# zyj0021200/simpleImageCaptionZoo

Measured on AMD Instinct MI355X. Metric: captions/sec (SCST step), BUTDDetection COCO14-size vocab, higher is better.
Workload: dtype f32

## Files before the change

### include/icz.h

```cpp
#ifndef ICZ_H_
#define ICZ_H_
#include <stddef.h>
#include <stdint.h>

#ifdef __cplusplus
extern "C" {
#endif

typedef enum {
    ICZ_OK = 0,
    ICZ_ERR_INVALID = -1,
    ICZ_ERR_HIP = -2,
    ICZ_ERR_STATE = -3,
    ICZ_ERR_NOMEM = -4
} icz_status;

const char* icz_last_error(void);
const char* icz_version(void);

typedef struct icz_butd icz_butd_t;

typedef struct {
    int32_t R;
    int32_t D;
    int32_t H;
    int32_t E;
    int32_t A;
    int32_t V;
    int32_t max_rows;
    int32_t max_len;
} icz_butd_dims;

typedef struct {
    float* embed_weight;
    float *td_w_ih, *td_w_hh, *td_b_ih, *td_b_hh;
    float *lm_w_ih, *lm_w_hh, *lm_b_ih, *lm_b_hh;
    float *enc_att_v, *enc_att_g, *enc_att_b;
    float *dec_att_v, *dec_att_g, *dec_att_b;
    float *affine_v, *affine_g, *affine_b;
    float *predict_v, *predict_g, *predict_b;
} icz_butd_params;

int icz_butd_create(const icz_butd_dims* dims, icz_butd_t** out);
int icz_butd_destroy(icz_butd_t* h);
int icz_butd_bind_params(icz_butd_t* h, const icz_butd_params* params);
int icz_butd_set_option(icz_butd_t* h, const char* name, int32_t value);
int icz_butd_set_mask_sum_global(icz_butd_t* h, const float* mask_sum_global_dev, void* stream);
typedef void (*icz_grad_ready_cb)(void* user, int32_t stage);
int icz_butd_set_grad_callback(icz_butd_t* h, icz_grad_ready_cb cb, void* user);
int icz_butd_refresh_weights(icz_butd_t* h, void* stream);

int icz_butd_greedy(icz_butd_t* h, const float* feats, int32_t B, int32_t max_len, int64_t* ids_out,
                    float* alphas_out, void* stream);

typedef struct {
    uint64_t seed;
    const float* uniforms;
    const uint8_t* emb_mask;
    const uint8_t* att_mask;
    const uint8_t* out_mask;
} icz_rng;

int icz_butd_sample(icz_butd_t* h, const float* feats, int32_t B, int32_t max_len, const icz_rng* rng,
                    int64_t* seq_out, float* logprobs_out, void* stream);

int icz_butd_scst_rollouts(icz_butd_t* h, const float* feats, int32_t B, int32_t max_len, const icz_rng* rng,
                           int64_t* greedy_ids_out, int64_t* seq_out, float* logprobs_out, void* stream);
int icz_butd_sample_n(icz_butd_t* h, const float* feats, int32_t B, int32_t K, int32_t max_len, const icz_rng* rng,
                      int64_t* seq_out, float* logprobs_out, void* stream);

int icz_butd_sample_backward(icz_butd_t* h, const float* reward, const icz_butd_params* grads, float* loss_out,
                             float* mask_sum_out, float mask_sum_global, void* stream);
int icz_butd_sample_backward_dlogp(icz_butd_t* h, const float* dlogp, const icz_butd_params* grads, void* stream);
int icz_butd_sample_mask_sum(icz_butd_t* h, float* mask_sum_out, void* stream);

int icz_butd_xe_forward(icz_butd_t* h, const float* feats, const int64_t* captions, int32_t B, int32_t L,
                        const int32_t* lengths_host, const icz_rng* rng, int32_t train,
                        float* packed_logits_out, void* stream);
int icz_butd_xe_backward(icz_butd_t* h, float smoothing, const icz_butd_params* grads, float* loss_out,
                         float n_tokens_global, void* stream);

int icz_butd_set_scheduled_sampling(icz_butd_t* h, float ss_prob, const float* gate_uniforms, const float* draw_uniforms);

int icz_butd_saved_alphas(icz_butd_t* h, float* alphas_out, void* stream);

int icz_butd_xe_backward_dlogits(icz_butd_t* h, const float* dpacked, const icz_butd_params* grads, void* stream);

int icz_butd_beam_search(icz_butd_t* h, const float* feats, int32_t n_img, int32_t beam, int32_t max_steps,
                         float* seqs_out, int32_t* lens_out, void* stream);

typedef struct {
    int32_t n_best;
    int32_t block_ngram;
    int32_t lp_kind;
    float lp_alpha;
} icz_beam_opts;

int icz_butd_beam_search_opts(icz_butd_t* h, const float* feats, int32_t n_img, int32_t beam, int32_t max_steps,
                              const icz_beam_opts* opts, float* seqs_out, int32_t* lens_out, float* scores_out, void* stream);

typedef struct {
    int32_t groups;
    float diversity;
} icz_beam_diversity;

int icz_butd_beam_search_diverse(icz_butd_t* h, const float* feats, int32_t n_img, int32_t beam, int32_t max_steps,
                                 const icz_beam_opts* opts, const icz_beam_diversity* div, float* seqs_out, int32_t* lens_out,
                                 float* scores_out, void* stream);

int icz_butd_step(icz_butd_t* h, const float* feats, int32_t B, const int64_t* it, float* h1, float* c1,
                  float* h2, float* c2, float* ctx_out, float* alpha_out, float* logits_out, void* stream);

typedef struct icz_nic icz_nic_t;
typedef struct { int32_t E, H, V, max_rows, max_len; } icz_nic_dims;
typedef struct {
    float* embed_weight;
    float *w_ih, *w_hh, *b_ih, *b_hh;
    float *predict_v, *predict_g, *predict_b;
} icz_nic_params;
int icz_nic_create(const icz_nic_dims* dims, icz_nic_t** out);
int icz_nic_destroy(icz_nic_t* h);
int icz_nic_bind_params(icz_nic_t* h, const icz_nic_params* params);
int icz_nic_refresh_weights(icz_nic_t* h, void* stream);
int icz_nic_greedy(icz_nic_t* h, const float* features, int32_t B, int32_t max_len, int64_t* ids_out, void* stream);
int icz_nic_sample(icz_nic_t* h, const float* features, int32_t B, int32_t max_len, const icz_rng* rng, int64_t* seq_out,
                   float* logprobs_out, void* stream);
int icz_nic_sample_backward(icz_nic_t* h, const float* reward, const icz_nic_params* grads, float* dfeatures_out, float* loss_out,
                            float* mask_sum_out, float mask_sum_global, void* stream);
int icz_nic_xe_forward(icz_nic_t* h, const float* features, const int64_t* captions, int32_t B, int32_t L, const int32_t* lengths_host,
                       const icz_rng* rng, int32_t train, float* packed_logits_out, void* stream);
int icz_nic_xe_backward(icz_nic_t* h, float smoothing, const icz_nic_params* grads, float* dfeatures_out, float* loss_out,
                        float n_tokens_global, void* stream);
int icz_nic_set_norm_global(icz_nic_t* h, const float* norm_dev, void* stream);
int icz_nic_set_option(icz_nic_t* h, const char* name, int32_t value);
int icz_nic_set_scheduled_sampling(icz_nic_t* h, float ss_prob, const float* gate_uniforms, const float* draw_uniforms);
int icz_nic_beam_search(icz_nic_t* h, const float* features, int32_t n_img, int32_t beam, int32_t max_steps, float* seqs_out,
                        int32_t* lens_out, void* stream);
int icz_nic_beam_search_opts(icz_nic_t* h, const float* features, int32_t n_img, int32_t beam, int32_t max_steps,
                             const icz_beam_opts* opts, float* seqs_out, int32_t* lens_out, float* scores_out, void* stream);
int icz_nic_beam_search_diverse(icz_nic_t* h, const float* features, int32_t n_img, int32_t beam, int32_t max_steps,
                                const icz_beam_opts* opts, const icz_beam_diversity* div, float* seqs_out, int32_t* lens_out,
                                float* scores_out, void* stream);

typedef struct icz_aoa icz_aoa_t;
typedef struct { int32_t R, D, Hd, E, V, NH, max_rows, max_len; } icz_aoa_dims;
typedef struct {
    float *q_w, *q_b, *k_w, *k_b, *v_w, *v_b, *aoa_w, *aoa_b, *ln_g, *ln_b;
} icz_aoa_block;
typedef struct {
    float *proj_w, *proj_b;
    icz_aoa_block layer[6];
    float *ref_ln_g, *ref_ln_b;
    float *lstm_w_ih, *lstm_w_hh, *lstm_b_ih, *lstm_b_hh;
    icz_aoa_block dec;
    float* embed_weight;
    float *predict_v, *predict_g, *predict_b;
} icz_aoa_params;
typedef struct {
    uint64_t seed;
    const float* uniforms;
    const uint8_t *proj_mask, *ref_att_mask, *ref_aoa_mask, *ref_sc_mask, *emb_mask, *ctx_mask, *att_mask, *out_mask;
} icz_aoa_rng;
int icz_aoa_create(const icz_aoa_dims* dims, icz_aoa_t** out);
int icz_aoa_destroy(icz_aoa_t* h);
int icz_aoa_bind_params(icz_aoa_t* h, const icz_aoa_params* params);
int icz_aoa_refresh_weights(icz_aoa_t* h, void* stream);
int icz_aoa_set_regions(icz_aoa_t* h, int32_t regions, const int32_t* counts_dev, const int32_t* counts_host, int32_t n_img);
int icz_aoa_set_option(icz_aoa_t* h, const char* name, int32_t value);
int icz_aoa_refine(icz_aoa_t* h, const float* feats, int32_t B, float* refined_out, void* stream);
int icz_aoa_greedy(icz_aoa_t* h, const float* feats, int32_t B, int32_t max_len, int64_t* ids_out, void* stream);
int icz_aoa_beam_search(icz_aoa_t* h, const float* feats, int32_t n_img, int32_t beam, int32_t max_steps, float* seqs_out,
                        int32_t* lens_out, void* stream);
int icz_aoa_beam_search_opts(icz_aoa_t* h, const float* feats, int32_t n_img, int32_t beam, int32_t max_steps,
                             const icz_beam_opts* opts, float* seqs_out, int32_t* lens_out, float* scores_out, void* stream);
int icz_aoa_beam_search_diverse(icz_aoa_t* h, const float* feats, int32_t n_img, int32_t beam, int32_t max_steps,
                                const icz_beam_opts* opts, const icz_beam_diversity* div, float* seqs_out, int32_t* lens_out,
                                float* scores_out, void* stream);
int icz_aoa_sample(icz_aoa_t* h, const float* feats, int32_t B, int32_t max_len, const icz_aoa_rng* rng, int64_t* seq_out,
                   float* logprobs_out, void* stream);
int icz_aoa_scst_rollouts(icz_aoa_t* h, const float* feats, int32_t B, int32_t max_len, const icz_aoa_rng* rng, int64_t* ids_out,
                          int64_t* seq_out, float* logprobs_out, void* stream);
int icz_aoa_sample_backward(icz_aoa_t* h, const float* reward, const icz_aoa_params* grads, float* loss_out, float* mask_sum_out,
                            float mask_sum_global, void* stream);
int icz_aoa_xe_forward(icz_aoa_t* h, const float* feats, const int64_t* captions, int32_t B, int32_t L, const int32_t* lengths_host,
                       const icz_aoa_rng* rng, int32_t train, float* packed_logits_out, void* stream);
int icz_aoa_xe_backward(icz_aoa_t* h, float smoothing, const icz_aoa_params* grads, float* loss_out, float n_tokens_global,
                        void* stream);
int icz_aoa_set_norm_global(icz_aoa_t* h, const float* norm_dev, void* stream);
int icz_aoa_set_grad_callback(icz_aoa_t* h, icz_grad_ready_cb cb, void* user);
int icz_aoa_saved_alphas(icz_aoa_t* h, float* alphas_out, void* stream);
int icz_aoa_set_scheduled_sampling(icz_aoa_t* h, float ss_prob, const float* gate_uniforms, const float* draw_uniforms);

typedef struct icz_ensemble icz_ensemble_t;
int icz_ensemble_create(const int32_t* kinds, void* const* members, const float* weights, int32_t M, icz_ensemble_t** out);
int icz_ensemble_destroy(icz_ensemble_t* h);
int icz_ensemble_greedy(icz_ensemble_t* h, const float* const* feats, int32_t B, int32_t max_len, int64_t* ids_out, void* stream);
int icz_ensemble_beam_search_diverse(icz_ensemble_t* h, const float* const* feats, int32_t n_img, int32_t beam, int32_t max_steps,
                                     const icz_beam_opts* opts, const icz_beam_diversity* div, float* seqs_out, int32_t* lens_out,
                                     float* scores_out, void* stream);
int icz_ensemble_logprob(int32_t M, const float* const* logits, const float* const* bias, const int32_t* nsplit, const int32_t* ld,
                         const float* weights, int32_t rows, int32_t V, float* lp_out, int32_t ldo, int64_t* argmax_out, void* stream);

typedef struct {
    float temperature;
    int32_t top_k;
    float top_p;
} icz_sample_opts;
int icz_sample_decode_check(const icz_sample_opts* opts, int32_t n_img, int32_t n, int32_t V, int32_t max_rows);
int icz_butd_sample_decode(icz_butd_t* h, const float* feats, int32_t n_img, int32_t n, int32_t max_len, const icz_sample_opts* opts,
                           uint64_t seed, const float* uniforms, int64_t* ids_out, float* logp_out, float* score_out, void* stream);
int icz_aoa_sample_decode(icz_aoa_t* h, const float* feats, int32_t n_img, int32_t n, int32_t max_len, const icz_sample_opts* opts,
                          uint64_t seed, const float* uniforms, int64_t* ids_out, float* logp_out, float* score_out, void* stream);
int icz_nic_sample_decode(icz_nic_t* h, const float* features, int32_t n_img, int32_t n, int32_t max_len, const icz_sample_opts* opts,
                          uint64_t seed, const float* uniforms, int64_t* ids_out, float* logp_out, float* score_out, void* stream);
int icz_sample_filter_draw(const float* logits, const float* bias, int32_t nsplit, int32_t ld, int32_t rows, int32_t V,
                           const icz_sample_opts* opts, const float* uniforms, int64_t* tok_out, float* logp_out, uint8_t* keep_out,
                           void* stream);

int icz_ensemble_sample_decode(icz_ensemble_t* h, const float* const* feats, int32_t n_img, int32_t n, int32_t max_len,
                               const icz_sample_opts* opts, uint64_t seed, const float* uniforms, int64_t* ids_out, float* logp_out,
                               float* score_out, void* stream);
int icz_ensemble_sample_filter_draw(int32_t M, const float* const* logits, const float* const* bias, const int32_t* nsplit,
                                    const int32_t* ld, const float* weights, int32_t rows, int32_t V, const icz_sample_opts* opts,
                                    const float* uniforms, int64_t* tok_out, float* logp_out, uint8_t* keep_out, void* stream);

int icz_adam_clamp_step(float* param, const float* grad, float* exp_avg, float* exp_avg_sq, int64_t n,
                        float lr, float clip, int32_t step, void* stream);
int icz_adam_clamp_multi(int32_t count, float* const* params, const float* const* grads, float* const* exp_avg,
                         float* const* exp_avg_sq, const int64_t* numel, float lr, float clip, int32_t step, void* stream);

typedef struct icz_ciderd icz_ciderd_t;

int icz_ciderd_create(const int32_t* df_keys, const double* df_idf, int64_t cap, double default_idf,
                      const double* penalty, icz_ciderd_t** out);
int icz_ciderd_destroy(icz_ciderd_t* h);

int icz_ciderd_reward(icz_ciderd_t* h, const int64_t* gen, const int64_t* greedy, int32_t B, int32_t T,
                      const int32_t* img_ref_ptr, const int32_t* ref_ent_ptr, const int32_t* ent_key,
                      const int32_t* ent_order, const double* ent_w, const double* ref_norm,
                      const int32_t* ref_len, float* reward_out, double* scores_out, void* stream);
int icz_ciderd_cook_host(const int32_t* df_keys_host, const double* df_idf_host, int64_t cap, double default_idf,
                         const int32_t* tokens, const int32_t* ref_tok_ptr, int32_t n_refs, int64_t max_ent,
                         int32_t* ent_key_out, int32_t* ent_order_out, double* ent_w_out, int32_t* ref_ent_ptr_out,
                         double* ref_norm_out, int32_t* ref_len_out, int64_t* n_ent_out);
typedef struct icz_ciderd_vocab icz_ciderd_vocab_t;
int icz_ciderd_vocab_create(const char* words, const int64_t* word_off, const int32_t* word_id, int32_t n_words, int32_t V,
                            icz_ciderd_vocab_t** out);
int icz_ciderd_vocab_destroy(icz_ciderd_vocab_t* v);
int icz_ciderd_vocab_oov_id(icz_ciderd_vocab_t* v, const char* word, int32_t len, int32_t* id_out);
int icz_ciderd_cook_text(icz_ciderd_vocab_t* vocab, const int32_t* df_keys_host, const double* df_idf_host, int64_t cap, double default_idf,
                         const char* text, int64_t text_len, int32_t n_refs, int64_t max_ent,
                         int32_t* ent_key_out, int32_t* ent_order_out, double* ent_w_out, int32_t* ref_ent_ptr_out,
                         double* ref_norm_out, int32_t* ref_len_out, int64_t* n_ent_out);
int icz_ciderd_reward_indexed(icz_ciderd_t* h, const int64_t* gen, const int64_t* greedy, int32_t B, int32_t T,
                              const int32_t* img_slot, const int32_t* img_ref_ptr, const int32_t* ref_ent_ptr,
                              const int32_t* ent_key, const int32_t* ent_order, const double* ent_w, const double* ref_norm,
                              const int32_t* ref_len, float* reward_out, double* scores_out, void* stream);
int icz_ciderd_reward_loo(icz_ciderd_t* h, const int64_t* gen, int32_t B, int32_t K, int32_t T, const int32_t* img_slot,
                          const int32_t* img_ref_ptr, const int32_t* ref_ent_ptr, const int32_t* ent_key, const int32_t* ent_order,
                          const double* ent_w, const double* ref_norm, const int32_t* ref_len, float* reward_out, double* scores_out,
                          void* stream);

int icz_ciderd_cook_device(icz_ciderd_t* h, const int32_t* tok, const int32_t* ptr, int32_t n_cand, int32_t* ent_key_out,
                           int32_t* ent_order_out, double* ent_w_out, int32_t* ent_ptr_out, double* norm_out, int32_t* len_out, void* stream);
size_t icz_ciderd_pairwise_workspace_bytes(int32_t n_img, int32_t K);
int icz_ciderd_pairwise(icz_ciderd_t* h, const int32_t* tok, const int32_t* ptr, int32_t n_img, int32_t K, double* pair_out,
                        double* consensus_out, int32_t* best_out, void* workspace, size_t workspace_bytes, void* stream);
int icz_ciderd_scores_csr(icz_ciderd_t* h, const int32_t* tok, const int32_t* ptr, int32_t n_img, int32_t K, const int32_t* img_slot,
                          const int32_t* img_ref_ptr, const int32_t* ref_ent_ptr, const int32_t* ent_key, const int32_t* ent_order,
                          const double* ent_w, const double* ref_norm, const int32_t* ref_len, double* scores_out, void* stream);
int icz_ngram_diversity(const int32_t* tok, const int32_t* ptr, int32_t n_img, int32_t K, int32_t* counts_out, void* stream);

int icz_bleu_stats(const int32_t* hyp_tok, const int32_t* hyp_ptr, const int32_t* ref_tok, const int32_t* ref_ptr,
                   const int32_t* img_ref_ptr, int32_t n_img, int32_t* stats_out, void* stream);
int icz_rouge_lcs(const int32_t* hyp_tok, const int32_t* hyp_ptr, const int32_t* ref_tok, const int32_t* ref_ptr,
                  const int32_t* img_ref_ptr, int32_t n_img, int32_t* lcs_out, void* stream);

int icz_gemm_f32(int32_t layout, const float* X, int32_t ldx, const float* W, int32_t ldw, const float* bias,
                 float* C, int32_t ldc, int32_t M, int32_t N, int32_t K, int32_t nsplit, float* workspace,
                 size_t workspace_floats, void* stream);
size_t icz_gemm_workspace_floats(int32_t M, int32_t N);
int icz_gemm_set_big_cfg(int32_t cfg);
int icz_gemm_big_cfg_for(int32_t layout, int32_t M, int32_t N, int32_t K, int32_t nsplit);
int icz_gemm_tn_grouped(const float* dY, int32_t ldy, int32_t M, int32_t K, int32_t ngroups, const float* const* X, const int32_t* ldx,
                        const int32_t* cols, float* const* out, const int32_t* ldo, const int32_t* rows_live, void* stream);
int icz_gemm_tn_split_pick(int32_t M, int32_t N, int32_t K);
int icz_gemm_tn_split(const float* dY, int32_t ldy, int32_t M, const float* X, int32_t ldx, int32_t N, int32_t K, float* out, int32_t ldo,
                      float* workspace, size_t workspace_floats, const int32_t* rows_live, void* stream);
int icz_gemm_route_for(int32_t layout, int32_t M, int32_t N, int32_t nseg, const int32_t* K, int32_t nsplit);
int icz_gemm_tn_grouped_fits(int32_t M, int32_t K, int32_t ngroups, const int32_t* cols);
int icz_prof_begin(void);
int icz_prof_select(int32_t which);
int icz_prof_pair_overhead(void* stream, int32_t n, double* avg_us);
int icz_prof_end(double* avg_us, double* bytes_per_launch, double* flops_per_launch, long long* launches);
int icz_kprof_begin(void);
int icz_kprof_end(int32_t group, double* avg_us, long long* pairs);
int icz_prof_stream_rate(const void* buf, size_t bytes, int32_t reps, void* stream, double* gbs);

#ifdef __cplusplus
}
#endif
#endif
```

### simpleimagecaptionzoo_amd/_lib.py

```python
import ctypes as C
import os

_HERE = os.path.dirname(os.path.abspath(__file__))
LIB_PATH = os.path.join(_HERE, "libicz.so")


class IczError(RuntimeError):
    pass


GRAD_READY_CB = C.CFUNCTYPE(None, C.c_void_p, C.c_int32)


class ButdDims(C.Structure):
    _fields_ = [(n, C.c_int32) for n in ("R", "D", "H", "E", "A", "V", "max_rows", "max_len")]


BUTD_PARAM_FIELDS = (
    "embed_weight",
    "td_w_ih", "td_w_hh", "td_b_ih", "td_b_hh",
    "lm_w_ih", "lm_w_hh", "lm_b_ih", "lm_b_hh",
    "enc_att_v", "enc_att_g", "enc_att_b",
    "dec_att_v", "dec_att_g", "dec_att_b",
    "affine_v", "affine_g", "affine_b",
# ... 45 lines not shown
class AoaRng(C.Structure):
    _fields_ = [("seed", C.c_uint64), ("uniforms", C.c_void_p)] + [(n, C.c_void_p) for n in (
        "proj_mask", "ref_att_mask", "ref_aoa_mask", "ref_sc_mask", "emb_mask", "ctx_mask", "att_mask", "out_mask")]


class NicParams(C.Structure):
    _fields_ = [(n, C.c_void_p) for n in NIC_PARAM_FIELDS]


class ButdParams(C.Structure):
    _fields_ = [(n, C.c_void_p) for n in BUTD_PARAM_FIELDS]


class Rng(C.Structure):
    _fields_ = [("seed", C.c_uint64), ("uniforms", C.c_void_p), ("emb_mask", C.c_void_p),
                ("att_mask", C.c_void_p), ("out_mask", C.c_void_p)]


class BeamOpts(C.Structure):
    _fields_ = [("n_best", C.c_int32), ("block_ngram", C.c_int32), ("lp_kind", C.c_int32), ("lp_alpha", C.c_float)]


class BeamDiversity(C.Structure):
    _fields_ = [("groups", C.c_int32), ("diversity", C.c_float)]


class SampleOpts(C.Structure):
    _fields_ = [("temperature", C.c_float), ("top_k", C.c_int32), ("top_p", C.c_float)]


_lib = None


def lib():
    global _lib
    if _lib is not None:
        return _lib
    if not os.path.exists(LIB_PATH):
        raise IczError("libicz.so not found at %s -- the HIP extension is required (no fallback); run "
                       "__graft_entry__.build()" % LIB_PATH)
    import torch
    L = C.CDLL(LIB_PATH)
    vp, i32, i64, f32 = C.c_void_p, C.c_int32, C.c_int64, C.c_float
    sig = {
        "icz_last_error": (C.c_char_p, []),
        "icz_version": (C.c_char_p, []),
        "icz_butd_create": (C.c_int, [C.POINTER(ButdDims), C.POINTER(vp)]),
        "icz_butd_destroy": (C.c_int, [vp]),
        "icz_butd_bind_params": (C.c_int, [vp, C.POINTER(ButdParams)]),
        "icz_butd_set_option": (C.c_int, [vp, C.c_char_p, i32]),
        "icz_butd_set_grad_callback": (C.c_int, [vp, GRAD_READY_CB, vp]),
        "icz_aoa_set_grad_callback": (C.c_int, [vp, GRAD_READY_CB, vp]),
        "icz_butd_set_mask_sum_global": (C.c_int, [vp, vp, vp]),
        "icz_butd_refresh_weights": (C.c_int, [vp, vp]),
        "icz_butd_greedy": (C.c_int, [vp, vp, i32, i32, vp, vp, vp]),
        "icz_butd_step": (C.c_int, [vp, vp, i32, vp, vp, vp, vp, vp, vp, vp, vp, vp]),
        "icz_butd_sample": (C.c_int, [vp, vp, i32, i32, C.POINTER(Rng), vp, vp, vp]),
        "icz_butd_scst_rollouts": (C.c_int, [vp, vp, i32, i32, C.POINTER(Rng), vp, vp, vp, vp]),
        "icz_butd_sample_n": (C.c_int, [vp, vp, i32, i32, i32, C.POINTER(Rng), vp, vp, vp]),
        "icz_butd_sample_backward": (C.c_int, [vp, vp, C.POINTER(ButdParams), vp, vp, f32, vp]),
        "icz_butd_sample_backward_dlogp": (C.c_int, [vp, vp, C.POINTER(ButdParams), vp]),
        "icz_butd_xe_backward_dlogits": (C.c_int, [vp, vp, C.POINTER(ButdParams), vp]),
        "icz_butd_beam_search": (C.c_int, [vp, vp, i32, i32, i32, vp, vp, vp]),
        "icz_butd_beam_search_opts": (C.c_int, [vp, vp, i32, i32, i32, C.POINTER(BeamOpts), vp, vp, vp, vp]),
        "icz_butd_beam_search_diverse": (C.c_int, [vp, vp, i32, i32, i32, C.POINTER(BeamOpts), C.POINTER(BeamDiversity), vp, vp, vp, vp]),
        "icz_butd_sample_mask_sum": (C.c_int, [vp, vp, vp]),
        "icz_butd_xe_forward": (C.c_int, [vp, vp, vp, i32, i32, C.POINTER(i32), C.POINTER(Rng), i32, vp, vp]),
        "icz_butd_xe_backward": (C.c_int, [vp, f32, C.POINTER(ButdParams), vp, f32, vp]),
        "icz_butd_set_scheduled_sampling": (C.c_int, [vp, f32, vp, vp]),
        "icz_nic_set_scheduled_sampling": (C.c_int, [vp, f32, vp, vp]),
        "icz_aoa_set_scheduled_sampling": (C.c_int, [vp, f32, vp, vp]),
        "icz_adam_clamp_step": (C.c_int, [vp, vp, vp, vp, i64, f32, f32, i32, vp]),
        "icz_nic_create": (C.c_int, [C.POINTER(NicDims), C.POINTER(vp)]),
        "icz_nic_destroy": (C.c_int, [vp]),
        "icz_nic_bind_params": (C.c_int, [vp, C.POINTER(NicParams)]),
        "icz_nic_refresh_weights": (C.c_int, [vp, vp]),
        "icz_nic_greedy": (C.c_int, [vp, vp, i32, i32, vp, vp]),
        "icz_nic_sample": (C.c_int, [vp, vp, i32, i32, C.POINTER(Rng), vp, vp, vp]),
        "icz_nic_sample_backward": (C.c_int, [vp, vp, C.POINTER(NicParams), vp, vp, vp, f32, vp]),
        "icz_nic_xe_forward": (C.c_int, [vp, vp, vp, i32, i32, C.POINTER(i32), C.POINTER(Rng), i32, vp, vp]),
        "icz_nic_xe_backward": (C.c_int, [vp, f32, C.POINTER(NicParams), vp, vp, f32, vp]),
        "icz_butd_saved_alphas": (C.c_int, [vp, vp, vp]),
        "icz_aoa_saved_alphas": (C.c_int, [vp, vp, vp]),
        "icz_nic_set_norm_global": (C.c_int, [vp, vp, vp]),
        "icz_aoa_set_norm_global": (C.c_int, [vp, vp, vp]),
        "icz_nic_beam_search": (C.c_int, [vp, vp, i32, i32, i32, vp, vp, vp]),
        "icz_nic_beam_search_opts": (C.c_int, [vp, vp, i32, i32, i32, C.POINTER(BeamOpts), vp, vp, vp, vp]),
        "icz_nic_beam_search_diverse": (C.c_int, [vp, vp, i32, i32, i32, C.POINTER(BeamOpts), C.POINTER(BeamDiversity), vp, vp, vp, vp]),
        "icz_aoa_create": (C.c_int, [C.POINTER(AoaDims), C.POINTER(vp)]),
        "icz_aoa_destroy": (C.c_int, [vp]),
        "icz_aoa_bind_params": (C.c_int, [vp, C.POINTER(AoaParams)]),
        "icz_aoa_refresh_weights": (C.c_int, [vp, vp]),
        "icz_aoa_set_regions": (C.c_int, [vp, i32, vp, vp, i32]),
        "icz_aoa_set_option": (C.c_int, [vp, C.c_char_p, i32]),
        "icz_nic_set_option": (C.c_int, [vp, C.c_char_p, i32]),
        "icz_aoa_refine": (C.c_int, [vp, vp, i32, vp, vp]),
        "icz_aoa_greedy": (C.c_int, [vp, vp, i32, i32, vp, vp]),
        "icz_aoa_beam_search": (C.c_int, [vp, vp, i32, i32, i32, vp, vp, vp]),
        "icz_aoa_beam_search_opts": (C.c_int, [vp, vp, i32, i32, i32, C.POINTER(BeamOpts), vp, vp, vp, vp]),
        "icz_aoa_beam_search_diverse": (C.c_int, [vp, vp, i32, i32, i32, C.POINTER(BeamOpts), C.POINTER(BeamDiversity), vp, vp, vp, vp]),
        "icz_ensemble_create": (C.c_int, [C.POINTER(i32), C.POINTER(vp), C.POINTER(f32), i32, C.POINTER(vp)]),
        "icz_ensemble_destroy": (C.c_int, [vp]),
        "icz_ensemble_greedy": (C.c_int, [vp, C.POINTER(vp), i32, i32, vp, vp]),
        "icz_ensemble_beam_search_diverse": (C.c_int, [vp, C.POINTER(vp), i32, i32, i32, C.POINTER(BeamOpts), C.POINTER(BeamDiversity), vp, vp,
                                                       vp, vp]),
        "icz_ensemble_logprob": (C.c_int, [i32, C.POINTER(vp), C.POINTER(vp), C.POINTER(i32), C.POINTER(i32), C.POINTER(f32), i32, i32, vp, i32,
                                           vp, vp]),
        "icz_ensemble_sample_decode": (C.c_int, [vp, C.POINTER(vp), i32, i32, i32, C.POINTER(SampleOpts), C.c_uint64, vp, vp, vp, vp, vp]),
        "icz_ensemble_sample_filter_draw": (C.c_int, [i32, C.POINTER(vp), C.POINTER(vp), C.POINTER(i32), C.POINTER(i32), C.POINTER(f32), i32, i32,
                                                      C.POINTER(SampleOpts), vp, vp, vp, vp, vp]),
        "icz_sample_decode_check": (C.c_int, [C.POINTER(SampleOpts), i32, i32, i32, i32]),
        "icz_butd_sample_decode": (C.c_int, [vp, vp, i32, i32, i32, C.POINTER(SampleOpts), C.c_uint64, vp, vp, vp, vp, vp]),
        "icz_aoa_sample_decode": (C.c_int, [vp, vp, i32, i32, i32, C.POINTER(SampleOpts), C.c_uint64, vp, vp, vp, vp, vp]),
        "icz_nic_sample_decode": (C.c_int, [vp, vp, i32, i32, i32, C.POINTER(SampleOpts), C.c_uint64, vp, vp, vp, vp, vp]),
        "icz_sample_filter_draw": (C.c_int, [vp, vp, i32, i32, i32, i32, C.POINTER(SampleOpts), vp, vp, vp, vp, vp]),
        "icz_aoa_sample": (C.c_int, [vp, vp, i32, i32, C.POINTER(AoaRng), vp, vp, vp]),
        "icz_aoa_scst_rollouts": (C.c_int, [vp, vp, i32, i32, C.POINTER(AoaRng), vp, vp, vp, vp]),
        "icz_aoa_sample_backward": (C.c_int, [vp, vp, C.POINTER(AoaParams), vp, vp, f32, vp]),
        "icz_aoa_xe_forward": (C.c_int, [vp, vp, vp, i32, i32, C.POINTER(i32), C.POINTER(AoaRng), i32, vp, vp]),
        "icz_aoa_xe_backward": (C.c_int, [vp, f32, C.POINTER(AoaParams), vp, f32, vp]),
        "icz_ciderd_create": (C.c_int, [vp, vp, i64, C.c_double, vp, C.POINTER(vp)]),
        "icz_ciderd_destroy": (C.c_int, [vp]),
        "icz_ciderd_reward": (C.c_int, [vp, vp, vp, i32, i32, vp, vp, vp, vp, vp, vp, vp, vp, vp, vp]),
        "icz_ciderd_cook_host": (C.c_int, [vp, vp, i64, C.c_double, vp, vp, i32, i64, vp, vp, vp, vp, vp, vp, C.POINTER(i64)]),
        "icz_ciderd_vocab_create": (C.c_int, [C.c_char_p, vp, vp, i32, i32, C.POINTER(vp)]),
        "icz_ciderd_vocab_destroy": (C.c_int, [vp]),
        "icz_ciderd_vocab_oov_id": (C.c_int, [vp, C.c_char_p, i32, C.POINTER(i32)]),
        "icz_ciderd_cook_text": (C.c_int, [vp, vp, vp, i64, C.c_double, C.c_char_p, i64, i32, i64, vp, vp, vp, vp, vp, vp, C.POINTER(i64)]),
        "icz_ciderd_reward_indexed": (C.c_int, [vp, vp, vp, i32, i32, vp, vp, vp, vp, vp, vp, vp, vp, vp, vp, vp]),
        "icz_ciderd_reward_loo": (C.c_int, [vp, vp, i32, i32, i32, vp, vp, vp, vp, vp, vp, vp, vp, vp, vp, vp]),
        "icz_ciderd_cook_device": (C.c_int, [vp, vp, vp, i32, vp, vp, vp, vp, vp, vp, vp]),
        "icz_ciderd_pairwise_workspace_bytes": (C.c_size_t, [i32, i32]),
        "icz_ciderd_pairwise": (C.c_int, [vp, vp, vp, i32, i32, vp, vp, vp, vp, C.c_size_t, vp]),
        "icz_ciderd_scores_csr": (C.c_int, [vp, vp, vp, i32, i32, vp, vp, vp, vp, vp, vp, vp, vp, vp, vp]),
        "icz_ngram_diversity": (C.c_int, [vp, vp, i32, i32, vp, vp]),
        "icz_bleu_stats": (C.c_int, [vp, vp, vp, vp, vp, i32, vp, vp]),
        "icz_rouge_lcs": (C.c_int, [vp, vp, vp, vp, vp, i32, vp, vp]),
        "icz_prof_begin": (C.c_int, []),
        "icz_prof_select": (C.c_int, [i32]),
        "icz_prof_pair_overhead": (C.c_int, [vp, i32, C.POINTER(C.c_double)]),
        "icz_prof_end": (C.c_int, [C.POINTER(C.c_double), C.POINTER(C.c_double), C.POINTER(C.c_double), C.POINTER(C.c_longlong)]),
        "icz_kprof_begin": (C.c_int, []),
        "icz_kprof_end": (C.c_int, [i32, C.POINTER(C.c_double), C.POINTER(C.c_longlong)]),
        "icz_prof_stream_rate": (C.c_int, [vp, C.c_size_t, i32, vp, C.POINTER(C.c_double)]),
        "icz_adam_clamp_multi": (C.c_int, [i32, C.POINTER(vp), C.POINTER(vp), C.POINTER(vp), C.POINTER(vp), C.POINTER(i64), f32, f32, i32, vp]),
        "icz_gemm_f32": (C.c_int, [i32, vp, i32, vp, i32, vp, vp, i32, i32, i32, i32, i32, vp, C.c_size_t, vp]),
        "icz_gemm_workspace_floats": (C.c_size_t, [i32, i32]),
        "icz_gemm_set_big_cfg": (C.c_int, [i32]),
        "icz_gemm_big_cfg_for": (C.c_int, [i32, i32, i32, i32, i32]),
        "icz_gemm_tn_grouped": (C.c_int, [vp, i32, i32, i32, i32, vp, vp, vp, vp, vp, vp, vp]),
        "icz_gemm_tn_split_pick": (C.c_int, [i32, i32, i32]),
        "icz_gemm_tn_split": (C.c_int, [vp, i32, i32, vp, i32, i32, i32, vp, i32, vp, C.c_size_t, vp, vp]),
        "icz_gemm_route_for": (C.c_int, [i32, i32, i32, i32, vp, i32]),
        "icz_gemm_tn_grouped_fits": (C.c_int, [i32, i32, i32, vp]),
    }
    for name, (res, args) in sig.items():
        try:
            fn = getattr(L, name)
        except AttributeError as e:
            raise IczError("libicz.so lacks symbol %s (stale build?)" % name) from e
        fn.restype, fn.argtypes = res, args
    _lib = L
    return L


def check(status):
    if status != 0:
        raise IczError("libicz status %d: %s" % (status, lib().icz_last_error().decode()))


def ptr(t):
    return None if t is None else C.c_void_p(t.data_ptr())


def stream_ptr():
    import torch
    return C.c_void_p(torch.cuda.current_stream().cuda_stream)
```

### simpleimagecaptionzoo_amd/butd.py

```python
import ctypes as C

import torch

from . import _lib
from ._lib import BUTD_PARAM_KEYS, ButdDims, ButdParams, Rng, check, lib, ptr, stream_ptr
from .handle import GraphDecoderHandle


def make_rng(seed=0, uniforms=None, emb_mask=None, att_mask=None, out_mask=None):
    r = Rng()
    r.seed = int(seed) & 0xFFFFFFFFFFFFFFFF
    keep = []
    for name, t, dt in (("uniforms", uniforms, torch.float32), ("emb_mask", emb_mask, torch.uint8),
                        ("att_mask", att_mask, torch.uint8), ("out_mask", out_mask, torch.uint8)):
        if t is not None:
            if t.dtype != dt or not t.is_cuda or not t.is_contiguous():
                raise _lib.IczError("%s must be a contiguous %s CUDA tensor" % (name, dt))
            setattr(r, name, t.data_ptr())
            keep.append(t)
    r._keep = keep
    return r


class ButdHandle(GraphDecoderHandle):

    family, kind = "butd", 0
    _Params, _param_keys = ButdParams, BUTD_PARAM_KEYS
    _make_rng = staticmethod(make_rng)
    _own_entries = ("step", "sample_n", "sample_mask_sum", "saved_alphas", "sample_backward_dlogp", "xe_backward_dlogits")
    _entry_names = {"set_norm_global": "set_mask_sum_global"}
    _sample_bufs = True

    def __init__(self, R, D, H, E, A, V, max_rows, max_len=20, device="cuda:0"):
        self._create(ButdDims(R, D, H, E, A, V, max_rows, max_len), device)

    def enable_graphs(self, on=True):
        super().enable_graphs(on)

    def set_concurrent(self, on=True):
        self.set_option("concurrent", 1 if on else 0)

    def _feats(self, feats):
        if feats.dtype != torch.float32 or not feats.is_cuda:
            raise _lib.IczError("feats must be an fp32 CUDA tensor")
        if feats.dim() != 3 or feats.shape[1] != self.R or feats.shape[2] != self.D:
            raise _lib.IczError("feats must be (B,%d,%d), got %s" % (self.R, self.D, tuple(feats.shape)))
        return feats.contiguous()

    def greedy(self, feats, max_len=20, want_alphas=False):
        feats = self._feats(feats)
        B = feats.shape[0]
        ids = self._buf("greedy_ids", (B, max_len), torch.int64)
        alphas = self._buf("greedy_alphas", (B, max_len, self.R), torch.float32) if want_alphas else None
        check(self._e.greedy(self._h, ptr(feats), B, max_len, ptr(ids), ptr(alphas), stream_ptr()))
        return (ids, alphas) if want_alphas else ids

    def sample_n(self, feats, n, max_len=20, rng=None):
        feats = self._feats(feats)
        B, n = feats.shape[0], int(n)
        if not 2 <= n <= 8:
            raise _lib.IczError("sample_n: n=%d samples per image outside 2..8" % n)
        if B * n > self.max_rows:
            raise _lib.IczError("sample_n: %d images x %d samples exceed the handle's row capacity %d" % (B, n, self.max_rows))
        rng = rng or make_rng(0)
        seq = self._buf("sample_n_seq", (B * n, max_len), torch.int64)
        lp = self._buf("sample_n_lp", (B * n, max_len), torch.float32)
        check(self._e.sample_n(self._h, ptr(feats), B, n, max_len, C.byref(rng), ptr(seq), ptr(lp), stream_ptr()))
        self._live = (feats, rng, seq, lp)
        return seq, lp

    def sample_mask_sum(self):
        out = torch.zeros(1, device=self.device)
        check(self._e.sample_mask_sum(self._h, ptr(out), stream_ptr()))
        return out

    def sample_backward_dlogp(self, dlogp, grads):
        dlogp = dlogp.to(device=self.device, dtype=torch.float32).contiguous()
        gs = self._grad_struct(grads)
        check(self._e.sample_backward_dlogp(self._h, ptr(dlogp), C.byref(gs), stream_ptr()))

    def saved_alphas(self, B, T):
        out = torch.empty(B, T, self.R, device=self.device)
        check(self._e.saved_alphas(self._h, ptr(out), stream_ptr()))
        return out

    def xe_backward_dlogits(self, dpacked, grads):
        dpacked = dpacked.to(device=self.device, dtype=torch.float32).contiguous()
        gs = self._grad_struct(grads)
        check(self._e.xe_backward_dlogits(self._h, ptr(dpacked), C.byref(gs), stream_ptr()))

    def step(self, feats, it, h1, c1, h2, c2):
        feats = self._feats(feats)
        B = feats.shape[0]
        dev = feats.device
        ctx = torch.empty(B, self.D, device=dev)
        alpha = torch.empty(B, self.R, device=dev)
        logits = torch.empty(B, self.V, device=dev)
        check(self._e.step(self._h, ptr(feats), B, ptr(it), ptr(h1), ptr(c1), ptr(h2), ptr(c2), ptr(ctx), ptr(alpha), ptr(logits),
                           stream_ptr()))
        return ctx, alpha, logits


def gemm(layout, X, W, bias=None, nsplit=0):
    code = {"nt": 0, "nn": 1, "tn": 2}[layout]
    if layout == "nt":
        M, K = X.shape
        N = W.shape[0]
    elif layout == "nn":
        M, K = X.shape
        N = W.shape[1]
    else:
        K, M = X.shape
        N = W.shape[1]
    out = torch.empty(M, N, device=X.device, dtype=torch.float32)
    ws = torch.empty(max(lib().icz_gemm_workspace_floats(M, N), max(nsplit, 1) * M * N), device=X.device,
                     dtype=torch.float32)
    check(lib().icz_gemm_f32(code, ptr(X), X.stride(0), ptr(W), W.stride(0), ptr(bias), ptr(out), N, M, N, K,
                             nsplit, ptr(ws), ws.numel(), stream_ptr()))
    return out


def gemm_set_big_cfg(cfg):
    check(lib().icz_gemm_set_big_cfg(int(cfg)))


def gemm_tn_grouped(dY, Xs, outs=None, rows_live=None):
    K, M = dY.shape
    n = len(Xs)
    if outs is None:
        outs = [torch.empty(M, x.shape[1], device=dY.device, dtype=torch.float32) for x in Xs]
    xp = (C.c_void_p * n)(*[x.data_ptr() for x in Xs])
    op = (C.c_void_p * n)(*[o.data_ptr() for o in outs])
    ldx = (C.c_int32 * n)(*[x.stride(0) for x in Xs])
    cols = (C.c_int32 * n)(*[x.shape[1] for x in Xs])
    ldo = (C.c_int32 * n)(*[o.stride(0) for o in outs])
    check(lib().icz_gemm_tn_grouped(ptr(dY), dY.stride(0), M, K, n, xp, ldx, cols, op, ldo, ptr(rows_live), stream_ptr()))
    return outs


def gemm_tn_split_pick(M, N, K):
    return int(lib().icz_gemm_tn_split_pick(int(M), int(N), int(K)))


def gemm_tn_split(dY, X, out=None, workspace=None, rows_live=None):
    K, M = dY.shape
    N = X.shape[1]
    if out is None:
        out = torch.empty(M, N, device=dY.device, dtype=torch.float32)
    if workspace is None:
        workspace = torch.empty(max(gemm_tn_split_pick(M, N, K), 1) * M * N, device=dY.device, dtype=torch.float32)
    check(lib().icz_gemm_tn_split(ptr(dY), dY.stride(0), M, ptr(X), X.stride(0), N, K, ptr(out), out.stride(0), ptr(workspace),
                                  workspace.numel(), ptr(rows_live), stream_ptr()))
    return out


GEMM_ROUTES = ("nt_fp32_mt1", "nt_fp32_mt2", "nt_fp32_mt4", "resident_4stage", "resident_512deep", "resident_128row", "x3_128tile",
               "large_tile", "nn_fp32", "tn_fp32_64", "tn_fp32_128")


def gemm_route_for(layout, M, N, Ks, nsplit=0):
    Ks = [int(k) for k in (Ks if isinstance(Ks, (list, tuple)) else [Ks])]
    arr = (C.c_int32 * len(Ks))(*Ks)
    r = int(lib().icz_gemm_route_for({"nt": 0, "nn": 1, "tn": 2}[layout], int(M), int(N), len(Ks), arr, int(nsplit)))
    return GEMM_ROUTES[r] if r >= 0 else None


def gemm_tn_grouped_fits(M, K, cols):
    arr = (C.c_int32 * len(cols))(*[int(c) for c in cols])
    return int(lib().icz_gemm_tn_grouped_fits(int(M), int(K), len(cols), arr)) == 1
```

### simpleimagecaptionzoo_amd/csrc/butd.hip

```cpp
#include <vector>

#include "butd_impl.h"

namespace icz {

int Butd::init(const icz_butd_dims& d) {
    dims = d;
    ICZ_REQUIRE(d.R > 0 && d.R <= 64, "butd: R=%d must be in 1..64 (36 boxes / 49 grid cells)", d.R);
    ICZ_REQUIRE(d.D % 4 == 0 && d.H % 4 == 0 && d.E % 4 == 0 && d.A % 4 == 0, "butd: D,H,E,A must be multiples of 4");
    ICZ_REQUIRE(d.V > 3 && d.max_rows > 0 && d.max_len > 0, "butd: bad V/max_rows/max_len");
    const size_t rows = d.max_rows, H = d.H, D = d.D, E = d.E, A = d.A, V = d.V, R = d.R;
    ICZ_TRY(alloc((void**)&w_enc, sizeof(float) * A * D));
    ICZ_TRY(alloc((void**)&w_dec, sizeof(float) * A * H));
    ICZ_TRY(alloc((void**)&w_aff, sizeof(float) * A));
    const size_t Vp = pad_vocab(d.V);
    ICZ_TRY(alloc((void**)&w_pred, sizeof(float) * Vp * H));
    ICZ_TRY(alloc((void**)&n_enc, sizeof(float) * A));
    ICZ_TRY(alloc((void**)&n_dec, sizeof(float) * A));
    ICZ_TRY(alloc((void**)&n_aff, sizeof(float) * 4));
    ICZ_TRY(alloc((void**)&n_pred, sizeof(float) * V));
    ICZ_TRY(alloc((void**)&mean, sizeof(float) * rows * D));
    ICZ_TRY(alloc((void**)&premean, sizeof(float) * rows * 4 * H));
    ICZ_TRY(alloc((void**)&enc_ctx, sizeof(float) * rows * R * A));
    for (int i = 0; i < 2; ++i) {
        ICZ_TRY(alloc((void**)&h1[i], sizeof(float) * rows * H));
        ICZ_TRY(alloc((void**)&c1[i], sizeof(float) * rows * H));
        ICZ_TRY(alloc((void**)&h2[i], sizeof(float) * rows * H));
        ICZ_TRY(alloc((void**)&c2[i], sizeof(float) * rows * H));
    }
    ICZ_TRY(alloc((void**)&emb, sizeof(float) * rows * E));
    ICZ_TRY(alloc((void**)&ctx, sizeof(float) * rows * D));
    ICZ_TRY(alloc((void**)&scores, sizeof(float) * rows * R));
    ICZ_TRY(alloc((void**)&alpha, sizeof(float) * rows * R));
    ICZ_TRY(alloc((void**)&h2drop, sizeof(float) * rows * H));
    ICZ_TRY(alloc((void**)&logits, sizeof(float) * rows * Vp));
    ICZ_TRY(alloc((void**)&amax_val, sizeof(float) * rows * ARGMAX_PARTS));
    ICZ_TRY(alloc((void**)&amax_idx, sizeof(int) * rows * ARGMAX_PARTS));
    ICZ_TRY(alloc((void**)&it, sizeof(int64_t) * rows));
    ICZ_TRY(alloc_scalars(mem));
    size_t nmax = 4 * H;
    if (A > nmax) nmax = A;
    if (V > nmax) nmax = V;
    ws_floats = (size_t)TARGET_WGS * 4096 * 2 + rows * nmax;
    {
        const size_t kmax = 2 * H + (E > D ? E : D), r128 = rows < 128 ? rows : 128;
        const size_t need = (kmax / 256 + 1) * r128 * 4 * H;
        if (need > ws_floats) ws_floats = need;
    }
    ICZ_TRY(alloc((void**)&ws, sizeof(float) * ws_floats));
    ICZ_TRY(mem.synced());
    if (const char* e = getenv("ICZ_EARLY_OUT")) early_out = atoi(e) != 0;
    if (const char* e = getenv("ICZ_MERGE_SMALL")) { const int n = atoi(e); if (n >= 0 && n <= 32) merge_small = n; }
    return ICZ_OK;
}

int Butd::refresh(hipStream_t st) {
    ICZ_REQUIRE(bound, "butd: parameters not bound");
    const int A = dims.A, D = dims.D, H = dims.H, V = dims.V;
    WeightNormTable wt = {};
    int nb = 0;
    auto add = [&](const float* v, const float* g, float* w, float* norm, int rows, int cols) {
        wt.j[wt.count++] = {v, g, w, norm, rows, cols, nb};
        nb += cdiv(rows, 4);
    };
    add(P.enc_att_v, P.enc_att_g, w_enc, n_enc, A, D);
    add(P.dec_att_v, P.dec_att_g, w_dec, n_dec, A, H);
    add(P.affine_v, P.affine_g, w_aff, n_aff, 1, A);
    add(P.predict_v, P.predict_g, w_pred, n_pred, V, H);
    hipLaunchKernelGGL(weight_norm_multi_kernel, dim3(nb), dim3(256), 0, st, wt);
    ICZ_CHECK_HIP(hipGetLastError());
    fresh = true;
    wt_fresh = false;
    return ICZ_OK;
}

bool Butd::wt_possible() const {
    GemmArgs g = {};
    g.nseg = 1;
    g.seg[0] = {w_enc, w_enc, 4 * dims.H, 4 * dims.H, 4 * dims.H, nullptr};
    g.M = 64; g.N = dims.D + dims.H;
    GemmArgs p = g, q = g;
    p.N = q.N = dims.H;
    p.nseg = 2; p.seg[1] = p.seg[0];
    return dims.H % 64 == 0 && dims.D % 64 == 0 && gemm_resident_x3_fits(g) && gemm_resident_x3_pair_fits(p, q);
}

int Butd::refresh_transposes(hipStream_t st) {
    ICZ_REQUIRE(bound && wt_lm_ih, "butd: no transposed weight buffers");
    const int H = dims.H, D = dims.D, E = dims.E;
    TransposeTable tt = {};
    int nb = 0;
    auto add = [&](const float* src, int ld, int cols, float* dst) {
        tt.j[tt.count++] = {src, ld, 4 * H, cols, dst, nb};
        nb += (4 * H / 64) * (cols / 64);
    };
    add(P.lm_w_ih, D + H, D + H, wt_lm_ih);
    add(P.lm_w_hh, H, H, wt_lm_hh);
    add(P.td_w_ih, H + D + E, H, wt_td_ih_h2);
    add(P.td_w_hh, H, H, wt_td_hh);
    hipLaunchKernelGGL(transpose_multi_kernel, dim3(nb), dim3(256), 0, st, tt);
    ICZ_CHECK_HIP(hipGetLastError());
    wt_fresh = true;
    return ICZ_OK;
}

int Butd::gemm_nt(GemmArgs& g, int* nsplit_out, hipStream_t st) {
    g.nsplit = gemm_fit_split(GEMM_NT, g, gemm_pick_split(g, TARGET_WGS), ws_floats);
    if (g.nsplit > 1) {
        ICZ_REQUIRE(gemm_slab_floats(g.M, g.N, g.nsplit) <= ws_floats, "butd: workspace too small for %dx%dx%d slabs", g.nsplit, g.M, g.N);
        g.out = ws;
        g.bias = nullptr;
    }
    *nsplit_out = g.nsplit;
    return gemm_f32(GEMM_NT, g, st);
}

int Butd::prologue(const float* feats, int n_img, hipStream_t st) {
    const int R = dims.R, D = dims.D, H = dims.H, E = dims.E, A = dims.A;
    ICZ_REQUIRE(fresh, "butd: call icz_butd_refresh_weights after binding/updating parameters");
    ICZ_REQUIRE(n_img > 0 && n_img <= dims.max_rows, "butd: %d images exceed capacity %d", n_img, dims.max_rows);
    hipLaunchKernelGGL(mean_feats_kernel, dim3(cdiv(D, 1024), n_img), dim3(256), 0, st, feats, mean, R, D);
    {
        GemmArgs g = {};
        g.nseg = 1;
        g.seg[0] = {mean, P.td_w_ih + H, D, H + D + E, D, nullptr};
        g.M = n_img; g.N = 4 * H; g.out = premean; g.ldo = 4 * H;
        int ns;
        ICZ_TRY(gemm_nt(g, &ns, st));
        if (ns > 1) {
            size_t MN = (size_t)n_img * 4 * H;
            hipLaunchKernelGGL(slab_reduce_kernel, dim3(cdiv((int)(MN / 4), 256)), dim3(256), 0, st, ws, ns, MN, 4 * H, (const float*)nullptr, premean);
        }
    }
    {
        GemmArgs g = {};
        g.nseg = 1;
        g.seg[0] = {feats, w_enc, D, D, D, nullptr};
        g.M = n_img * R; g.N = A; g.out = enc_ctx; g.ldo = A; g.bias = P.enc_att_b;
        int ns;
        const float* bias = g.bias;
        ICZ_TRY(gemm_nt(g, &ns, st));
        if (ns > 1) {
            size_t MN = (size_t)n_img * R * A;
            hipLaunchKernelGGL(slab_reduce_kernel, dim3(cdiv((int)(MN / 4), 256)), dim3(256), 0, st, ws, ns, MN, A, bias, enc_ctx);
        }
    }
    ICZ_CHECK_HIP(hipGetLastError());
    return ICZ_OK;
}

int Butd::step(const StepIO& s, hipStream_t st) {
    const int R = dims.R, D = dims.D, H = dims.H, E = dims.E, A = dims.A, V = dims.V;
    const int Vp = pad_vocab(V);
    const int rows = s.rows;
    float* const ws = s.ws_alt ? s.ws_alt : this->ws;
    float* const scores = s.scores_alt ? s.scores_alt : this->scores;
    DropCfg off = {0, nullptr, nullptr, 0, 0};
    if (!s.emb_ready)
        hipLaunchKernelGGL(embed_kernel, dim3(cdiv(E, 1024), rows), dim3(256), 0, st, P.embed_weight, s.it, s.emb_out ? s.emb_out : emb, rows, E, s.drop_emb);
    const float* embp = s.emb_out ? s.emb_out : emb;
    int ns;
    {
        GemmArgs g = {};
        g.nseg = 3;
        g.seg[0] = {s.h2_in, P.td_w_ih, H, H + D + E, H, nullptr};
        g.seg[1] = {embp, P.td_w_ih + H + D, E, H + D + E, E, nullptr};
        g.seg[2] = {s.h1_in, P.td_w_hh, H, H, H, nullptr};
        g.M = rows; g.N = 4 * H; g.out = ws; g.ldo = 4 * H;
        g.live = s.live;
        const size_t ws_cap = s.ws_alt ? (tb.xfloats < ws_floats ? tb.xfloats : ws_floats) : ws_floats;
        g.nsplit = gemm_fit_split(GEMM_NT, g, gemm_pick_split(g, STEP_WGS), ws_cap);
        ns = g.nsplit;
        ICZ_REQUIRE(gemm_slab_floats(rows, 4 * H, ns) <= ws_cap && (size_t)rows * 4 * H <= ws_cap, "butd: workspace too small");
        if (ns == 1) { g.out = ws; }
        ICZ_TRY(gemm_f32(GEMM_NT, g, st));
        LstmPointArgs a = {ws, ns, premean, s.img_of_row, P.td_b_ih, P.td_b_hh, s.c1_in, s.h1_out, s.c1_out, s.gates_td_out, nullptr, rows, H, s.live};
        kprof_mark(KP_LSTM_POINT, true, st);
        launch_lstm_point(a, off, st);
        kprof_mark(KP_LSTM_POINT, false, st);
    }
    {
        kprof_mark(KP_ATTENTION, true, st);
        GemmArgs g = {};
        g.nseg = 1;
        g.seg[0] = {s.h1_out, w_dec, H, H, H, nullptr};
        g.M = rows; g.N = A; g.out = ws; g.ldo = A;
        g.live = s.live;
        g.nsplit = gemm_pick_split(g, STEP_WGS);
        ns = g.nsplit;
        ICZ_TRY(gemm_f32(GEMM_NT, g, st));
        AttScoreArgs a = {enc_ctx, s.img_of_row, ws, ns, P.dec_att_b, w_aff, P.affine_b, s.dec_ctx_out, scores, rows, R, A, s.live};
        const int G = s.rows_per_img;
        const bool grouped = G > 1 && G <= ATT_CTX_MAX_G && rows % G == 0 && sizeof(float) * A * G <= 60 * 1024;
        if (grouped && s.drop_att.mode == 0 && !s.live)
            hipLaunchKernelGGL(att_scores_group_kernel, dim3(rows / G, ATT_PARTS), dim3(256), sizeof(float) * A * G, st, a, G);
        else if (grouped)
            hipLaunchKernelGGL(att_scores_group_train_kernel, dim3(rows / G, ATT_PARTS), dim3(256), sizeof(float) * A * G, st, a, s.drop_att, G);
        else
            hipLaunchKernelGGL(att_scores_kernel, dim3(rows, ATT_PARTS), dim3(256), sizeof(float) * A, st, a, s.drop_att);
        if (G > 1 && G <= ATT_CTX_MAX_G && rows % G == 0 && !s.alpha_out2)
            hipLaunchKernelGGL(att_ctx_group_kernel, dim3(rows / G, cdiv(D, 512)), dim3(256), 0, st, s.feats, (const float*)scores,
                               s.alpha_out ? s.alpha_out : alpha, s.ctx_out ? s.ctx_out : ctx, R, D, G, s.live);
        else
            hipLaunchKernelGGL(att_ctx_kernel, dim3(rows, cdiv(D, 512)), dim3(256), 0, st, s.feats, s.img_of_row, (const float*)scores,
                               s.alpha_out ? s.alpha_out : alpha, s.alpha_out2, s.alpha2_stride, s.ctx_out ? s.ctx_out : ctx, R, D, s.live);
        kprof_mark(KP_ATTENTION, false, st);
    }
    const float* ctxp = s.ctx_out ? s.ctx_out : ctx;
    {
        GemmArgs g = {};
        g.nseg = 3;
        g.seg[0] = {ctxp, P.lm_w_ih, D, D + H, D, nullptr};
        g.seg[1] = {s.h1_out, P.lm_w_ih + D, H, D + H, H, nullptr};
        g.seg[2] = {s.h2_in, P.lm_w_hh, H, H, H, nullptr};
        g.M = rows; g.N = 4 * H; g.out = ws; g.ldo = 4 * H;
        g.live = s.live;
        const size_t ws_cap = s.ws_alt ? (tb.xfloats < ws_floats ? tb.xfloats : ws_floats) : ws_floats;
        g.nsplit = gemm_fit_split(GEMM_NT, g, gemm_pick_split(g, STEP_WGS), ws_cap);
        ns = g.nsplit;
        ICZ_REQUIRE(gemm_slab_floats(rows, 4 * H, ns) <= ws_cap && (size_t)rows * 4 * H <= ws_cap, "butd: workspace too small");
        ICZ_TRY(gemm_f32(GEMM_NT, g, st));
        LstmPointArgs a = {ws, ns, nullptr, nullptr, P.lm_b_ih, P.lm_b_hh, s.c2_in, s.h2_out, s.c2_out, s.gates_lm_out,
                           s.h2drop_out ? s.h2drop_out : h2drop, rows, H, s.live};
        launch_lstm_point(a, s.drop_out, st);
    }
    if (!s.skip_predict) {
        const size_t ws_cap = s.ws_alt ? (tb.xfloats < ws_floats ? tb.xfloats : ws_floats) : ws_floats;
        ICZ_TRY(gemm_predict(s.h2drop_out ? s.h2drop_out : h2drop, H, w_pred, P.predict_b, rows, V, Vp, s.logits_out ? s.logits_out : logits,
                             s.logits_ld ? s.logits_ld : Vp, ws, ws_cap, s.pred_nsplit, st, s.live));
    }
    ICZ_CHECK_HIP(hipGetLastError());
    return ICZ_OK;
}

int Butd::zero_state(int rows, int which, hipStream_t st) {
    ZeroList z = {{h1[which], c1[which], h2[which], c2[which]}, 4};
    const size_t n = (size_t)rows * dims.H;
    hipLaunchKernelGGL(zero_bufs_kernel, dim3(cdiv((int)(n / 4), 256)), dim3(256), 0, st, z, n);
    return ICZ_OK;
}

int Butd::greedy(const float* feats, int B, int max_len, int64_t* ids_out, float* alphas_out, hipStream_t st) {
    ICZ_REQUIRE(feats && ids_out && B > 0 && B <= dims.max_rows && max_len > 0, "butd greedy: bad arguments");
    ICZ_REQUIRE(fresh, "butd: call icz_butd_refresh_weights after binding/updating parameters");
    if (!use_graphs) return greedy_impl(feats, B, max_len, ids_out, alphas_out, st);
    const std::vector<uintptr_t> key = {1, (uintptr_t)feats, (uintptr_t)B, (uintptr_t)max_len, (uintptr_t)ids_out, (uintptr_t)alphas_out, opt_bits()};
    return gc.run(key, st, [&](hipStream_t s) { return greedy_impl(feats, B, max_len, ids_out, alphas_out, s); });
}

int Butd::greedy_impl(const float* feats, int B, int max_len, int64_t* ids_out, float* alphas_out, hipStream_t st) {
    ICZ_TRY(prologue(feats, B, st));
    return greedy_chain(feats, B, max_len, ids_out, alphas_out, st);
}

int Butd::greedy_chain(const float* feats, int B, int max_len, int64_t* ids_out, float* alphas_out, hipStream_t st, bool scst) {
    ICZ_TRY(zero_state(B, 0, st));
    int* const gn = (scst && early_out && gnunf && tb.T >= max_len && tb.B >= B) ? gnunf : nullptr;
    hipLaunchKernelGGL(greedy_init_kernel, dim3(cdiv(B > max_len ? B : max_len, 256)), dim3(256), 0, st, it, B, gn, max_len);
    int cur = 0;
    const int Vp = pad_vocab(dims.V);
    bool track = false;
    for (int t = 0; t < max_len; ++t) {
        StepIO s = {};
        s.rows = B; s.feats = feats; s.it = it;
        s.emb_ready = t > 0;
        s.h1_in = h1[cur]; s.c1_in = c1[cur]; s.h2_in = h2[cur]; s.c2_in = c2[cur];
        s.h1_out = h1[cur ^ 1]; s.c1_out = c1[cur ^ 1]; s.h2_out = h2[cur ^ 1]; s.c2_out = c2[cur ^ 1];
        if (alphas_out) { s.alpha_out2 = alphas_out + (size_t)t * dims.R; s.alpha2_stride = max_len * dims.R; }
        int pns = 1;
        s.pred_nsplit = &pns;
        if (track && t > 0) s.live = gn + (t - 1);
        ICZ_TRY(step(s, st));
        if (t == 0) track = gn && pns > 1;
        kprof_mark(KP_GREEDY_SELECT, true, st);
        launch_greedy_select(logits_view(ws, P.predict_b, logits, B, Vp, pns), emb_slot(), B, dims.V, amax_val, amax_idx, it, ids_out, max_len, t,
                             track ? gunf : nullptr, track ? gn : nullptr, st);
        kprof_mark(KP_GREEDY_SELECT, false, st);
        cur ^= 1;
    }
    ICZ_CHECK_HIP(hipGetLastError());
    return ICZ_OK;
}

int Butd::prologue(const float* feats, int n_img, int k, const int32_t*, hipStream_t st) {
    ICZ_TRY(prologue(feats, n_img, st));
    seam_feats = feats;
    return zero_state(n_img * k, 0, st);
}

int Butd::step(int rows, const int64_t* it_, const int32_t* img_of_row, int rows_per_img, int cur, bool slabs, LogitsView* out,
               hipStream_t st) {
    StepIO s = {};
    s.rows = rows; s.feats = seam_feats; s.img_of_row = img_of_row; s.it = it_;
    s.rows_per_img = rows_per_img;
    s.emb_ready = seam_emb_ready; s.live = seam_live;
    s.h1_in = h1[cur]; s.c1_in = c1[cur]; s.h2_in = h2[cur]; s.c2_in = c2[cur];
    s.h1_out = h1[cur ^ 1]; s.c1_out = c1[cur ^ 1]; s.h2_out = h2[cur ^ 1]; s.c2_out = c2[cur ^ 1];
    int pns = 1;
    if (slabs) s.pred_nsplit = &pns;
    ICZ_TRY(step(s, st));
    if (out) *out = logits_view(ws, P.predict_b, logits, rows, pad_vocab(dims.V), pns);
    return ICZ_OK;
}

void Butd::gather(const int32_t* src_row, int rows, int fan, hipStream_t st) {
    hipLaunchKernelGGL(beam_gather_kernel, dim3(cdiv(dims.H, 1024), rows), dim3(256), 0, st, src_row, dims.H, h1[1], c1[1], h2[1], c2[1],
                       h1[0], c1[0], h2[0], c2[0], fan);
}

DecodeMember* butd_member(void* handle) { return static_cast<DecodeMember*>(reinterpret_cast<Butd*>(handle)); }

}

using namespace icz;

extern "C" {

int icz_butd_create(const icz_butd_dims* dims, icz_butd_t** out) { return abi_create<Butd>("icz_butd_create", dims, out); }

int icz_butd_destroy(icz_butd_t* h) {
    delete reinterpret_cast<Butd*>(h);
    return ICZ_OK;
}

int icz_butd_bind_params(icz_butd_t* h, const icz_butd_params* p) {
    ICZ_REQUIRE(h && p, "icz_butd_bind_params: null argument");
    ICZ_TRY(check_param_table("icz_butd_bind_params", p, sizeof(*p), (1u << 16) | (1u << 17)));
    Butd* b = reinterpret_cast<Butd*>(h);
    if (b->bound && memcmp(&b->P, p, sizeof(*p)) != 0) {
        ICZ_CHECK_HIP(hipDeviceSynchronize());
        b->gc.clear();
    }
    b->P = *p;
    b->bound = true;
    b->fresh = false;
    return ICZ_OK;
}

int icz_butd_set_option(icz_butd_t* h, const char* name, int32_t value) {
    ICZ_REQUIRE(h && name, "icz_butd_set_option: null argument");
    Butd* b = reinterpret_cast<Butd*>(h);
    if (strcmp(name, "graphs") == 0) { b->use_graphs = value != 0; return ICZ_OK; }
    if (strcmp(name, "concurrent") == 0) { b->concurrent = value != 0; return ICZ_OK; }
    if (strcmp(name, "early_out") == 0) { b->early_out = value != 0; return ICZ_OK; }
    if (strcmp(name, "small_nt") == 0) { b->small_nt = value != 0; return ICZ_OK; }
    if (strcmp(name, "group_att") == 0) { b->group_att = value != 0; return ICZ_OK; }
    if (strcmp(name, "merge_small") == 0) {
        ICZ_REQUIRE(value >= 0 && value <= 32, "icz_butd_set_option: merge_small %d outside 0..32", value);
        b->merge_small = value;
        return ICZ_OK;
    }
    set_error("icz_butd_set_option: unknown option '%s'", name);
    return ICZ_ERR_INVALID;
}

int icz_butd_set_mask_sum_global(icz_butd_t* h, const float* mask_sum_global_dev, void* stream) {
    return set_norm_global("icz_butd_set_mask_sum_global", reinterpret_cast<Butd*>(h), mask_sum_global_dev, stream);
}

int icz_butd_set_grad_callback(icz_butd_t* h, icz_grad_ready_cb cb, void* user) {
    ICZ_REQUIRE(h, "null handle");
    Butd* b = reinterpret_cast<Butd*>(h);
    b->grad_cb = cb; b->grad_cb_user = user;
    return ICZ_OK;
}

int icz_butd_refresh_weights(icz_butd_t* h, void* stream) {
    ICZ_REQUIRE(h, "null handle");
    return reinterpret_cast<Butd*>(h)->refresh((hipStream_t)stream);
}

int icz_butd_greedy(icz_butd_t* h, const float* feats, int32_t B, int32_t max_len, int64_t* ids_out,
                    float* alphas_out, void* stream) {
    ICZ_REQUIRE(h, "null handle");
    return reinterpret_cast<Butd*>(h)->greedy(feats, B, max_len, ids_out, alphas_out, (hipStream_t)stream);
}

int icz_butd_step(icz_butd_t* h, const float* feats, int32_t B, const int64_t* it, float* h1, float* c1,
                  float* h2, float* c2, float* ctx_out, float* alpha_out, float* logits_out, void* stream) {
    ICZ_REQUIRE(h && feats && it && h1 && c1 && h2 && c2 && logits_out, "icz_butd_step: null argument");
    Butd* b = reinterpret_cast<Butd*>(h);
    hipStream_t st = (hipStream_t)stream;
    ICZ_REQUIRE(B > 0 && B <= b->dims.max_rows, "icz_butd_step: B out of range");
    ICZ_TRY(b->prologue(feats, B, st));
    StepIO s = {};
    s.rows = B; s.feats = feats; s.it = it;
    s.h1_in = h1; s.c1_in = c1; s.h2_in = h2; s.c2_in = c2;
    s.h1_out = b->h1[0]; s.c1_out = b->c1[0]; s.h2_out = b->h2[0]; s.c2_out = b->c2[0];
    s.ctx_out = ctx_out; s.alpha_out = alpha_out; s.logits_out = logits_out; s.logits_ld = b->dims.V;
    ICZ_TRY(b->step(s, st));
    const size_t n = sizeof(float) * B * b->dims.H;
    ICZ_CHECK_HIP(hipMemcpyAsync(h1, b->h1[0], n, hipMemcpyDeviceToDevice, st));
    ICZ_CHECK_HIP(hipMemcpyAsync(c1, b->c1[0], n, hipMemcpyDeviceToDevice, st));
    ICZ_CHECK_HIP(hipMemcpyAsync(h2, b->h2[0], n, hipMemcpyDeviceToDevice, st));
    ICZ_CHECK_HIP(hipMemcpyAsync(c2, b->c2[0], n, hipMemcpyDeviceToDevice, st));
    return ICZ_OK;
}

}
```

### simpleimagecaptionzoo_amd/csrc/butd_impl.h

```cpp
#pragma once
#include <vector>
#include <stdint.h>

#include "decoder_core.h"

namespace icz {

struct StepIO {
    int rows;
    const float* feats;
    const int32_t* img_of_row;
    int rows_per_img;
    const int64_t* it;
    bool emb_ready;
    const float *h1_in, *c1_in, *h2_in, *c2_in;
    float *h1_out, *c1_out, *h2_out, *c2_out;
    float* emb_out;
    float* gates_td_out;
    float* gates_lm_out;
    float* dec_ctx_out;
    float* alpha_out;
    float* alpha_out2; int alpha2_stride;
    float* ctx_out;
    float* h2drop_out;
    float* logits_out;
    int logits_ld;
    int* pred_nsplit;
    float* ws_alt;
    float* scores_alt;
    DropCfg drop_emb, drop_att, drop_out;
    bool skip_predict;
    const int* live;
};

struct TrainBuf {
    int B = 0, T = 0;
    int64_t* tok = nullptr;
    float *emb = nullptr, *h1 = nullptr, *c1 = nullptr, *h2 = nullptr, *c2 = nullptr;
    float *gtd = nullptr, *glm = nullptr, *dec = nullptr, *alpha = nullptr, *ctx = nullptr, *h2d = nullptr, *logit = nullptr;
    int* nany = nullptr;
    int32_t* img2 = nullptr;
    int32_t* imgk = nullptr;
    float* dEncImg = nullptr;
    float *dGtd = nullptr, *dGlm = nullptr, *dDec = nullptr, *dEmb = nullptr, *dH2d = nullptr, *dEnc = nullptr;
    float *dwaff = nullptr, *dalpha = nullptr, *dS = nullptr, *dGsum = nullptr;
    float *dc1[2] = {nullptr, nullptr}, *dc2[2] = {nullptr, nullptr};
    float* X[4] = {nullptr, nullptr, nullptr, nullptr}; size_t xfloats = 0;
    float *dWp = nullptr, *dWenc = nullptr, *dWdec = nullptr, *dWaff = nullptr, *scalars = nullptr;
    float* wslab[2] = {nullptr, nullptr}; size_t wslab_floats[2] = {0, 0};
};

struct Butd : CaptionHead, DecodeMember {
    static constexpr int TARGET_WGS = 512;
    static constexpr int ATT_PARTS = 4;
    static constexpr int STEP_WGS = 256;
    icz_butd_dims dims;
    icz_butd_params P;
    bool bound = false, fresh = false;
    DeviceBuffers mem;

    float *w_enc = nullptr, *w_dec = nullptr, *w_aff = nullptr, *w_pred = nullptr;
    float *n_enc = nullptr, *n_dec = nullptr, *n_aff = nullptr, *n_pred = nullptr;
    float *mean = nullptr, *premean = nullptr, *enc_ctx = nullptr;
    float *h1[2], *c1[2], *h2[2], *c2[2];
    float *emb = nullptr, *ctx = nullptr, *scores = nullptr, *alpha = nullptr, *h2drop = nullptr, *logits = nullptr;
    int64_t* it = nullptr;
    float* amax_val = nullptr; int* amax_idx = nullptr;
    float* ws = nullptr;
    size_t ws_floats = 0;
    float *wt_lm_ih = nullptr, *wt_lm_hh = nullptr, *wt_td_ih_h2 = nullptr, *wt_td_hh = nullptr;
    bool wt_fresh = false;
    bool wt_possible() const;
    int refresh_transposes(hipStream_t st);

    int alloc(void** p, size_t bytes) { return mem.alloc(p, bytes); }
    int init(const icz_butd_dims& d);
    int refresh(hipStream_t st);
    int gemm_nt(GemmArgs& g, int* nsplit_out, hipStream_t st);
    int prologue(const float* feats, int n_img, hipStream_t st);
    int step(const StepIO& s, hipStream_t st);
    int zero_state(int rows, int which, hipStream_t st);
    int greedy(const float* feats, int B, int max_len, int64_t* ids_out, float* alphas_out, hipStream_t st);

    GraphCache gc{24};
    bool use_graphs = false;
    bool concurrent = true;
    uintptr_t opt_bits() const {
        return (concurrent ? 1 : 0) + (early_out ? 2 : 0) + 4 * merge_small + (small_nt ? 256 : 0) + (group_att ? 512 : 0);
    }
    int greedy_impl(const float* feats, int B, int max_len, int64_t* ids_out, float* alphas_out, hipStream_t st);
    int sample_impl(const float* feats, int B, int T, int64_t* seq_out, float* logp_out, hipStream_t st);
    int greedy_chain(const float* feats, int B, int max_len, int64_t* ids_out, float* alphas_out, hipStream_t st, bool scst = false);
    int sample_chain(const float* feats, int B, int T, int64_t* seq_out, float* logp_out, hipStream_t st, int row0 = 0, int64_t* ids_out = nullptr);
    int rollouts(const float* feats, int B, int T, const icz_rng* r, int64_t* ids_out, int64_t* seq_out, float* logp_out, hipStream_t st);
    int rollouts_impl(const float* feats, int B, int T, int64_t* ids_out, int64_t* seq_out, float* logp_out, hipStream_t st);
    SideStream side;
    SideStream low;
    icz_grad_ready_cb grad_cb = nullptr; void* grad_cb_user = nullptr;
    int sample_backward_impl(const float* reward, const icz_butd_params& G, float* loss_out, float* mask_sum_out, hipStream_t st,
                             int phases = 0xF, bool fire_cb = true);
    bool bptt_joined = false;
    int merge_small = 8;
    int cur_rows = 0, cur_row0 = 0;
    bool early_out = true;
    bool bptt_early_out = false;
    bool small_nt = true;
    int cur_K = 1, cur_nimg = 0;
    bool group_att = false;

    const float* seam_feats = nullptr;
    int vocab() const override { return dims.V; }
    int row_capacity() const override { return dims.max_rows; }
    bool refreshed() const override { return fresh; }
    bool compact_step() const override { return true; }
    EmbSlot emb_slot() const override { return {P.embed_weight, emb, dims.E, 1}; }
    DeviceBuffers& buffers() override { return mem; }
    int prologue(const float* feats, int n_img, int k, const int32_t* img_of_row, hipStream_t st) override;
    int step(int rows, const int64_t* it, const int32_t* img_of_row, int rows_per_img, int cur, bool slabs, LogitsView* out,
             hipStream_t st) override;
    void gather(const int32_t* src_row, int rows, int fan, hipStream_t st) override;

    TrainBuf tb;
    icz_rng rng = {};
    const float* cur_feats = nullptr;
    int ensure_train(int B, int T);
    int train_step(const float* feats, int rows, int Bs, int t, bool train, hipStream_t st, bool emb_ready = false, int* pred_nsplit = nullptr,
                   bool skip_predict = false, const int* live = nullptr, int row0 = 0);
    int sample(const float* feats, int B, int T, const icz_rng* r, int64_t* seq_out, float* logp_out, hipStream_t st);
    int sample_n(const float* feats, int B, int K, int T, const icz_rng* r, int64_t* seq_out, float* logp_out, hipStream_t st);
    int sample_n_impl(const float* feats, int B, int K, int T, int64_t* seq_out, float* logp_out, hipStream_t st);
    int sample_mask_sum(float* out, hipStream_t st);
    int sample_backward(const float* reward, const icz_butd_params* G, float* loss_out, float* mask_sum_out,
                        float mask_sum_global, hipStream_t st);
    int xe_forward(const float* feats, const int64_t* captions, int B, int L, const int32_t* lengths, const icz_rng* r,
                   int train, float* packed_out, hipStream_t st);
    int sample_backward_dlogp(const float* dlogp, const icz_butd_params* G, hipStream_t st);
    int xe_backward_dlogits(const float* dpacked, const icz_butd_params* G, hipStream_t st);
    int xe_backward(float smoothing, const icz_butd_params* G, float* loss_out, float n_tokens_global, hipStream_t st);
    int gemm_auto(GemmLayout layout, GemmArgs& g, float* slab, size_t slab_floats, int* ns_out, hipStream_t st);
    int wgrad(const float* dY, int ldy, int M, const float* X, int ldx, int N, int K, float* out, int ldo, hipStream_t st, const int* rows_live = nullptr);
    int bptt_prelude(hipStream_t st);
    int colsum(const float* X, int K, int N, int ldx, float* out, hipStream_t st);
    int bptt(const icz_butd_params& G, hipStream_t st, int phases = 0xF, bool fire_cb = true);
};

}
```

### simpleimagecaptionzoo_amd/csrc/butd_kernels.h

```cpp
#pragma once
#include <stdlib.h>

#include "icz_common.h"
#include "rng.h"

namespace icz {
namespace {

__global__ __launch_bounds__(256) void weight_norm_kernel(const float* __restrict__ v, const float* __restrict__ g,
                                                          float* __restrict__ w, float* __restrict__ norm,
                                                          int rows, int cols) {
    const int lane = threadIdx.x & 63;
    const int row = blockIdx.x * 4 + (threadIdx.x >> 6);
    if (row >= rows) return;
    const float* vr = v + (size_t)row * cols;
    float ss = 0.f;
    for (int c = lane * 4; c < cols; c += 256) {
        f32x4 x = *reinterpret_cast<const f32x4*>(vr + c);
        ss += x[0] * x[0] + x[1] * x[1] + x[2] * x[2] + x[3] * x[3];
    }
    ss = wave_sum(ss);
    const float nrm = sqrtf(ss);
    const float s = g[row] / nrm;
    float* wr = w + (size_t)row * cols;
// ... 1043 lines not shown
        if (w < wave) wave_off += t;
        total += t;
    }
    const double target = (double)u * total;
    int cand = 0x7fffffff;
    {
        const double prev = __shfl_up(inc, 1, 64);
        double run = wave_off + (lane ? prev : 0.0);
        if (run <= target && wave_off + inc > target) {
            cand = v1 - 1;
            for (int v = v0; v < v1 - 1; ++v) {
                run += (double)expf((srow[v] - mx) - lse);
                if (run > target) { cand = v; break; }
            }
        }
    }
#pragma unroll
    for (int o = 32; o > 0; o >>= 1) cand = min(cand, __shfl_xor(cand, o, 64));
    if (lane == 0) smi[wave] = cand;
    __syncthreads();
    int tok = 0;
    {
        int d = smi[0];
#pragma unroll
        for (int w = 1; w < NW; ++w) d = min(d, smi[w]);
        if (d > a.V - 1) d = a.V - 1;
        const bool unf = was_unf && (d != 2);
        tok = unf ? d : 0;
        if (tid == 0) {
            a.unfinished[sr] = unf ? 1 : 0;
            a.seq_out[(size_t)sr * a.T + a.t] = tok;
            a.logp_out[(size_t)sr * a.T + a.t] = (srow[d] - mx) - lse;
            a.it_next[row] = tok;
            a.draw_out[row] = d;
            a.lse_out[row] = mx + lse;
            if (unf) {
                atomicAdd(&a.n_unfinished[a.t], 1);
                if (MG) atomicAdd(&a.n_any[a.t], 1);
            }
        }
    }
    if (a.emb_next)
        for (int e = tid * 4; e < a.E; e += 4 * SEL_THREADS) {
            f32x4 x = *reinterpret_cast<const f32x4*>(a.emb_table + (size_t)tok * a.E + e);
            const uint32_t k = a.emb_drop.mode ? a.emb_drop.keep4((uint64_t)sr * a.E + e) : 0xFu;
#pragma unroll
            for (int j = 0; j < 4; ++j) x[j] = ((k >> j) & 1u) ? fmaxf(x[j], 0.f) * sc : 0.f;
            *reinterpret_cast<f32x4*>(a.emb_next + (size_t)row * a.E + e) = x;
        }
}
inline void launch_sample_select(hipStream_t st, int rows, const SampleSelArgs& a) {
    if (a.row0 > 0) hipLaunchKernelGGL(sample_select_kernel<true>, dim3(rows), dim3(SEL_THREADS), sizeof(float) * a.V, st, a);
    else hipLaunchKernelGGL(sample_select_kernel<false>, dim3(rows), dim3(SEL_THREADS), sizeof(float) * a.V, st, a);
}

__global__ __launch_bounds__(256) void reinforce_loss_kernel(const float* __restrict__ logp, const int64_t* __restrict__ seq,
                                                             const float* __restrict__ reward, int B, int T,
                                                             const float* __restrict__ mask_sum_global_p, float* __restrict__ coef,
                                                             float* __restrict__ loss_out, float* __restrict__ mask_sum_out) {
    __shared__ float smf[4];
    const int tid = threadIdx.x;
    float ms = 0.f, ls = 0.f;
    for (int i = tid; i < B * T; i += 256) {
        const int t = i % T;
        const float m = (t == 0) ? 1.f : (seq[i - 1] > 0 ? 1.f : 0.f);
        ms += m;
        ls += -logp[i] * reward[i] * m;
    }
    ms = block_sum_256(ms, smf);
    ls = block_sum_256(ls, smf);
    const float msg = mask_sum_global_p ? mask_sum_global_p[0] : 0.f;
    const float denom = msg > 0.f ? msg : ms;
    for (int i = tid; i < B * T; i += 256) {
        const int t = i % T;
        const float m = (t == 0) ? 1.f : (seq[i - 1] > 0 ? 1.f : 0.f);
        coef[i] = -reward[i] * m / denom;
    }
    if (tid == 0) {
        if (loss_out) loss_out[0] = ls / denom;
        if (mask_sum_out) mask_sum_out[0] = ms;
    }
}

__global__ __launch_bounds__(256) void reinforce_dlogits_kernel(float* __restrict__ logits, int V, int ldl,
                                                                const int32_t* __restrict__ draw, const float* __restrict__ lse,
                                                                const float* __restrict__ coef, int B, int T, int Bs = 0, int row0 = 0) {
    const int row = blockIdx.y;
    const int v = blockIdx.x * 256 + threadIdx.x;
    if (v >= ldl) return;
    const int stride = Bs > 0 ? Bs : B;
    const int t = row / stride, b = row % stride - row0;
    float* l = logits + (size_t)row * ldl;
    const float c = b >= 0 ? coef[(size_t)b * T + t] : 0.f;
    const int d = draw[row];
    float g = 0.f;
    if (v < V && d >= 0 && c != 0.f) g = c * ((v == d ? 1.f : 0.f) - expf(l[v] - lse[row]));
    l[v] = g;
}

constexpr int XE_MAX_T = 128;
struct XeRows { int n[XE_MAX_T]; };
__global__ __launch_bounds__(256) void xe_loss_dlogits_kernel(float* __restrict__ logits, int V, int ldl,
                                                              const int64_t* __restrict__ captions, int L, int B, XeRows rows,
                                                              float smoothing, float inv_n_host, const float* __restrict__ n_dev,
                                                              float* __restrict__ loss_rows) {
    __shared__ float smf[4];
    const int b = blockIdx.x, t = blockIdx.y, tid = threadIdx.x;
    if (b >= rows.n[t]) {
        float* z = logits + (size_t)(t * B + b) * ldl;
        for (int v = tid; v < ldl; v += 256) z[v] = 0.f;
        return;
    }
    const float inv_n = (n_dev && n_dev[0] > 0.f) ? 1.0f / n_dev[0] : inv_n_host;
    const int row = t * B + b;
    float* l = logits + (size_t)row * ldl;
    float mx = -INFINITY;
    for (int v = tid; v < V; v += 256) mx = fmaxf(mx, l[v]);
    mx = block_max_256(mx, smf);
    float se = 0.f;
    for (int v = tid; v < V; v += 256) se += expf(l[v] - mx);
    se = block_sum_256(se, smf);
    const float lse = mx + logf(se);
    const int tg = (int)captions[(size_t)b * L + t + 1];
    const float conf = 1.f - smoothing, low = smoothing / (float)(V - 1);
    const float lconf = conf > 0.f ? logf(conf) : 0.f, llow = low > 0.f ? logf(low) : 0.f;
    float ls = 0.f;
    for (int v = tid; v < ldl; v += 256) {
        float g = 0.f;
        if (v < V) {
            const float lp = l[v] - lse;
            const float tr = (v == tg) ? conf : low;
            if (tr > 0.f) ls += tr * (((v == tg) ? lconf : llow) - lp);
            g = (expf(lp) - tr) * inv_n;
        }
        l[v] = g;
    }
    ls = block_sum_256(ls, smf);
    if (tid == 0) loss_rows[row] = ls;
}

__global__ __launch_bounds__(256) void sum_scale_kernel(const float* __restrict__ x, int n, float scale_host, const float* __restrict__ n_dev,
                                                        float* __restrict__ out) {
    __shared__ float smf[4];
    const float scale = (n_dev && n_dev[0] > 0.f) ? 1.0f / n_dev[0] : scale_host;
    float s = 0.f;
    for (int i = threadIdx.x; i < n; i += 256) s += x[i];
    s = block_sum_256(s, smf);
    if (threadIdx.x == 0) out[0] = s * scale;
}

struct LstmBwdArgs {
    const float* dh_a; int ns_a;
    int lda_a;
    const float* dh_b; int ns_b; int lda_b;
    const float* dh_c; int ns_c; int lda_c;
    const float* dhdrop;
    const float* dc_in;
    const float* gates;
    const float* c_prev;
    const float* c_cur;
    float* dgates;
    float* dc_prev;
    int rows, H;
    int rows_a, rows_b, rows_c;
    int dc_in_rows;
    const int* live;
    const int* carry_live;
};
__global__ __launch_bounds__(256) void lstm_bwd_point_kernel(LstmBwdArgs a, DropCfg dc) {
    const int row = blockIdx.y;
    const int j = blockIdx.x * 256 + threadIdx.x;
    if (j >= a.H) return;
    const int H = a.H, G = 4 * H;
    const int lflag = live_flag(a.live), cflag = live_flag(a.carry_live);
    const float* g = a.gates + (size_t)row * G + j;
    const float gi = g[0], gf = g[H], gg = g[2 * H], go = g[3 * H];
    const float cc = a.c_cur[(size_t)row * H + j];
    const float cp = a.c_prev ? a.c_prev[(size_t)row * H + j] : 0.f;
    float dhd = 0.f;
    if (a.dhdrop) dhd = a.dhdrop[(size_t)row * H + j];
    if (flag_dead(lflag)) {
        float* o = a.dgates + (size_t)row * G + j;
        o[0] = 0.f; o[H] = 0.f; o[2 * H] = 0.f; o[3 * H] = 0.f;
        return;
    }
    const bool carry = cflag != 0;
    float dh = 0.f;
    if (a.dh_a && carry && row < a.rows_a) dh += sum_slabs1(a.dh_a, a.ns_a, (size_t)a.rows_a * a.lda_a, (size_t)row * a.lda_a + j);
    if (a.dh_b && row < a.rows_b) dh += sum_slabs1(a.dh_b, a.ns_b, (size_t)a.rows_b * a.lda_b, (size_t)row * a.lda_b + j);
    if (a.dh_c && row < a.rows_c) dh += sum_slabs1(a.dh_c, a.ns_c, (size_t)a.rows_c * a.lda_c, (size_t)row * a.lda_c + j);
    if (a.dhdrop) {
        float d = dhd;
        if (dc.mode) d = dc.keep((uint64_t)row * H + j) ? d * 2.0f : 0.f;
        dh += d;
    }
    const float dcin = (a.dc_in && carry && row < a.dc_in_rows) ? a.dc_in[(size_t)row * H + j] : 0.f;
    const float tc = tanhf(cc);
    const float dcv = dcin + dh * go * (1.f - tc * tc);
    float* o = a.dgates + (size_t)row * G + j;
    o[0] = dcv * gg * gi * (1.f - gi);
    o[H] = dcv * cp * gf * (1.f - gf);
    o[2 * H] = dcv * gi * (1.f - gg * gg);
    o[3 * H] = dh * tc * go * (1.f - go);
    a.dc_prev[(size_t)row * H + j] = dcv * gf;
}


constexpr int DALPHA_COLS = 512;
__global__ __launch_bounds__(256) void att_bwd_dalpha_kernel(const float* __restrict__ dctx, int ns, int ldc, int rows,
                                                             const float* __restrict__ feats, int R, int D,
                                                             float* __restrict__ dalpha_part, const int* __restrict__ live,
                                                             const int32_t* __restrict__ img_of_row) {
    __shared__ __attribute__((aligned(16))) float sd[DALPHA_COLS];
    const int lflag = live_flag(live);
    const int row = blockIdx.x, part = blockIdx.y, nparts = gridDim.y;
    const int tid = threadIdx.x, lane = tid & 63, wave = tid >> 6;
    const int c0 = part * DALPHA_COLS;
    const size_t ss = (size_t)rows * ldc;
    constexpr int NR = 5;
    const int ca = c0 + 4 * lane, cb = ca + 256;
    const bool va = ca < D, vb = cb < D;
    const float* frow = feats + (size_t)(img_of_row ? img_of_row[row] : row) * R * D;
    f32x4 xa[NR], xb[NR];
    auto load_pass = [&](int r0) {
#pragma unroll
        for (int u = 0; u < NR; ++u) {
            const int r = min(r0 + 4 * u, R - 1);
            xa[u] = *reinterpret_cast<const f32x4*>(frow + (size_t)r * D + (va ? ca : 0));
            xb[u] = *reinterpret_cast<const f32x4*>(frow + (size_t)r * D + (vb ? cb : 0));
        }
    };
    load_pass(wave);
    if (flag_dead(lflag)) return;
    if (tid < DALPHA_COLS / 4) {
        const int c = c0 + 4 * tid;
        f32x4 v = {0.f, 0.f, 0.f, 0.f};
        if (c < D) v = sum_slabs4(dctx, ns, ss, (size_t)row * ldc + c);
        *reinterpret_cast<f32x4*>(sd + 4 * tid) = v;
    }
    __syncthreads();
    const f32x4 ga = *reinterpret_cast<const f32x4*>(sd + 4 * lane), gb = *reinterpret_cast<const f32x4*>(sd + 256 + 4 * lane);
    for (int r0 = wave; r0 < R; r0 += 4 * NR) {
        if (r0 != wave) load_pass(r0);
#pragma unroll
        for (int u = 0; u < NR; ++u) {
            float acc = 0.f;
            if (va) acc += xa[u][0] * ga[0] + xa[u][1] * ga[1] + xa[u][2] * ga[2] + xa[u][3] * ga[3];
            if (vb) acc += xb[u][0] * gb[0] + xb[u][1] * gb[1] + xb[u][2] * gb[2] + xb[u][3] * gb[3];
            acc = wave_sum(acc);
            const int r = r0 + 4 * u;
            if (lane == 0 && r < R) dalpha_part[((size_t)row * nparts + part) * R + r] = acc;
        }
    }
}

struct AttBwdDdecArgs {
    const float* enc_ctx; const float* dec_ctx; const float* w_aff; const float* alpha; const float* dalpha;
    float* ddec; float* ds_out;
    int R, A, nparts;
    const int* live;
    const int32_t* img_of_row;
};
__global__ __launch_bounds__(256) void att_bwd_ddec_kernel(AttBwdDdecArgs a, DropCfg dc) {
    __shared__ float sds[64];
    __shared__ __attribute__((aligned(16))) float spart[3 * 64 * 4];
    const int row = blockIdx.x, tid = threadIdx.x, lane = tid & 63, wq = tid >> 6;
    const int lflag = live_flag(a.live);
    const int img = a.img_of_row ? a.img_of_row[row] : row;
    const float al = lane < a.R ? a.alpha[(size_t)row * a.R + lane] : 0.f;
    const float da0 = lane < a.R ? a.dalpha[(size_t)row * a.nparts * a.R + lane] : 0.f;
    if (flag_dead(lflag)) {
        if (blockIdx.y == 0 && tid < a.R) a.ds_out[(size_t)row * a.R + tid] = 0.f;
        const int c = blockIdx.y * 256 + tid;
        if (c < a.A) a.ddec[(size_t)row * a.A + c] = 0.f;
        return;
    }
    float da = da0;
    if (lane < a.R)
        for (int p = 1; p < a.nparts; ++p) da += a.dalpha[((size_t)row * a.nparts + p) * a.R + lane];
    const float dot = wave_sum(al * da);
    const float ds_l = al * (da - dot);
    if (tid < 64) {
        sds[tid] = ds_l;
        if (blockIdx.y == 0 && tid < a.R) a.ds_out[(size_t)row * a.R + tid] = ds_l;
    }
    __syncthreads();
    const int c = blockIdx.y * 256 + lane * 4;
    const bool valid = c < a.A;
    f32x4 acc = {0.f, 0.f, 0.f, 0.f};
    if (valid) {
        const f32x4 d = *reinterpret_cast<const f32x4*>(a.dec_ctx + (size_t)row * a.A + c);
        const f32x4 w = *reinterpret_cast<const f32x4*>(a.w_aff + c);
        const float sc = dc.mode ? 2.0f : 1.0f;
        constexpr int RB = 9;
        const bool shared_bits = dc.mode == 2 && (a.A & 255) == 0;
        for (int r0 = wq; r0 < a.R; r0 += 4 * RB) {
            f32x4 x[RB];
#pragma unroll
            for (int u = 0; u < RB; ++u) {
                const int r = min(r0 + 4 * u, a.R - 1);
                x[u] = *reinterpret_cast<const f32x4*>(a.enc_ctx + ((size_t)img * a.R + r) * a.A + c);
            }
            uint32_t kq[RB];
            if (shared_bits) {
                const int pu = min(lane >> 1, RB - 1), ph = lane & 1;
                const int pr = min(r0 + 4 * pu, a.R - 1);
                const uint64_t g = (((uint64_t)row * a.R + pr) * a.A + blockIdx.y * 256 + 128 * ph) >> 7;
                const uint64_t seed = *dc.seed_p;
                uint4_ ctr = {(uint32_t)g, (uint32_t)(g >> 32), dc.step, dc.stream};
                const uint4_ pw = philox4x32_10(ctr, (uint32_t)seed, (uint32_t)(seed >> 32));
#pragma unroll
                for (int u = 0; u < RB; ++u) {
                    const int src = 2 * u + (lane >> 5);
                    const uint32_t w0 = __shfl(pw.x, src), w1 = __shfl(pw.y, src), w2 = __shfl(pw.z, src), w3 = __shfl(pw.w, src);
                    const int wi = (lane >> 3) & 3;
                    const uint32_t ww = wi == 0 ? w0 : (wi == 1 ? w1 : (wi == 2 ? w2 : w3));
                    kq[u] = (ww >> ((4 * lane) & 31)) & 0xFu;
                }
            }
#pragma unroll
            for (int u = 0; u < RB; ++u) {
                const int r = r0 + 4 * u;
                if (r < a.R) {
                    const float ds = sds[r];
                    const uint32_t k = shared_bits ? kq[u] : (dc.mode ? dc.keep4(((uint64_t)row * a.R + r) * a.A + c) : 0xFu);
#pragma unroll
                    for (int j = 0; j < 4; ++j) {
                        const bool on = (x[u][j] + d[j] > 0.f) && ((k >> j) & 1u);
                        acc[j] += on ? ds * w[j] * sc : 0.f;
                    }
                }
            }
        }
    }
    if (wq > 0) *reinterpret_cast<f32x4*>(spart + ((wq - 1) * 64 + lane) * 4) = acc;
    __syncthreads();
    if (wq == 0 && valid) {
#pragma unroll
        for (int w = 0; w < 3; ++w) acc += *reinterpret_cast<const f32x4*>(spart + (w * 64 + lane) * 4);
        *reinterpret_cast<f32x4*>(a.ddec + (size_t)row * a.A + c) = acc;
    }
// ... 509 lines not shown
```

### simpleimagecaptionzoo_amd/csrc/butd_train.hip

```cpp
#include <math.h>

#include "butd_impl.h"

namespace icz {

static inline int round4(int x) { return pad_vocab(x); }

__global__ void sample_init_kernel(uint8_t* unf, int* nunf, int64_t* tok, int B, int T) {
    const int i = blockIdx.x * blockDim.x + threadIdx.x;
    if (i < B) { unf[i] = 1; tok[i] = 1; }
    if (i < T) nunf[i] = 0;
}

int Butd::ensure_train(int B, int T) {
    if (tb.B >= B && tb.T >= T) return ICZ_OK;
    ICZ_REQUIRE(B <= 2 * dims.max_rows, "butd: batch %d exceeds capacity %d", B, dims.max_rows);
    ICZ_REQUIRE(T <= XE_MAX_T, "butd: %d steps exceed the limit of %d", T, XE_MAX_T);
    if (tb.B > B) B = tb.B;
    if (tb.T > T) T = tb.T;
    if (dims.max_len > T) T = dims.max_len;
    if (!mem.training.empty()) {
        ICZ_TRY(mem.release_training(&gc));
        tb = TrainBuf();
        drop_loss_buffers();
    }
    if (!wt_lm_ih && wt_possible()) {
        const size_t G4 = 4 * (size_t)dims.H;
        ICZ_TRY(alloc((void**)&wt_lm_ih, sizeof(float) * G4 * (dims.D + dims.H)));
        ICZ_TRY(alloc((void**)&wt_lm_hh, sizeof(float) * G4 * dims.H));
        ICZ_TRY(alloc((void**)&wt_td_ih_h2, sizeof(float) * G4 * dims.H));
        ICZ_TRY(alloc((void**)&wt_td_hh, sizeof(float) * G4 * dims.H));
        wt_fresh = false;
    }
    DeviceBuffers::TrainingScope scope(mem);
    const size_t H = dims.H, D = dims.D, E = dims.E, A = dims.A, R = dims.R, V = dims.V;
    const size_t Vp = round4(dims.V);
    const size_t TB = (size_t)T * B;
    ICZ_TRY(alloc((void**)&tb.tok, sizeof(int64_t) * (TB + B)));
    ICZ_TRY(alloc((void**)&tb.emb, sizeof(float) * TB * E));
    ICZ_TRY(alloc((void**)&tb.h1, sizeof(float) * (TB + B) * H));
    ICZ_TRY(alloc((void**)&tb.c1, sizeof(float) * (TB + B) * H));
    ICZ_TRY(alloc((void**)&tb.h2, sizeof(float) * (TB + B) * H));
    ICZ_TRY(alloc((void**)&tb.c2, sizeof(float) * (TB + B) * H));
    ICZ_TRY(alloc((void**)&tb.gtd, sizeof(float) * TB * 4 * H));
    ICZ_TRY(alloc((void**)&tb.glm, sizeof(float) * TB * 4 * H));
    ICZ_TRY(alloc((void**)&tb.dec, sizeof(float) * TB * A));
    ICZ_TRY(alloc((void**)&tb.alpha, sizeof(float) * TB * R));
    ICZ_TRY(alloc((void**)&tb.ctx, sizeof(float) * TB * D));
    ICZ_TRY(alloc((void**)&tb.h2d, sizeof(float) * TB * H));
    ICZ_TRY(alloc((void**)&tb.logit, sizeof(float) * TB * Vp));
    ICZ_TRY(alloc_loss_buffers(mem, TB, B, T));
    ICZ_TRY(alloc((void**)&tb.nany, sizeof(int) * T));
    ICZ_TRY(alloc((void**)&tb.img2, sizeof(int32_t) * B));
    ICZ_TRY(alloc((void**)&tb.imgk, sizeof(int32_t) * B));
    ICZ_TRY(alloc((void**)&tb.dGtd, sizeof(float) * TB * 4 * H));
    ICZ_TRY(alloc((void**)&tb.dGlm, sizeof(float) * TB * 4 * H));
    ICZ_TRY(alloc((void**)&tb.dDec, sizeof(float) * TB * A));
    ICZ_TRY(alloc((void**)&tb.dEmb, sizeof(float) * TB * E));
    ICZ_TRY(alloc((void**)&tb.dH2d, sizeof(float) * TB * H));
    ICZ_TRY(alloc((void**)&tb.dEnc, sizeof(float) * (size_t)B * R * A));
    ICZ_TRY(alloc((void**)&tb.dEncImg, sizeof(float) * (size_t)(B / 2) * R * A));
    ICZ_TRY(alloc((void**)&tb.dwaff, sizeof(float) * (size_t)B * ATT_PARTS * A));
    ICZ_TRY(alloc((void**)&tb.dalpha, sizeof(float) * (size_t)B * R * cdiv((int)D, DALPHA_COLS)));
    ICZ_TRY(alloc((void**)&tb.dS, sizeof(float) * TB * R));
    ICZ_TRY(alloc((void**)&tb.dGsum, sizeof(float) * (size_t)(B + B / 2) * 4 * H));
    for (int i = 0; i < 2; ++i) {
        ICZ_TRY(alloc((void**)&tb.dc1[i], sizeof(float) * (size_t)B * H));
        ICZ_TRY(alloc((void**)&tb.dc2[i], sizeof(float) * (size_t)B * H));
    }
    tb.xfloats = (size_t)TARGET_WGS * 4096 * 2 + (size_t)B * (D + H);
    {
        const size_t kmax = 2 * H + (E > D ? E : D), r128 = B < 128 ? B : 128;
        const size_t need = (kmax / 256 + 1) * r128 * 4 * H;
        if (need > tb.xfloats) tb.xfloats = need;
    }
    for (int i = 0; i < 4; ++i) ICZ_TRY(alloc((void**)&tb.X[i], sizeof(float) * tb.xfloats));
    ICZ_TRY(alloc((void**)&tb.dWp, sizeof(float) * Vp * H));
    ICZ_TRY(alloc((void**)&tb.dWenc, sizeof(float) * A * D));
    ICZ_TRY(alloc((void**)&tb.dWdec, sizeof(float) * A * H));
    {
        auto slabs = [](size_t M, size_t N, size_t K) { return (size_t)gemm_tn_split_pick((int)M, (int)N, (int)K) * M * N; };
        const size_t side[3] = {slabs(A, H, TB), slabs(A, D, B * R), slabs(Vp, H, TB)}, own = slabs(4 * H, H, TB);
        const size_t direct[3] = {A * H, A * D, Vp * H};
        for (int i = 0; i < 3; ++i)
            if (side[i] > direct[i] && side[i] > tb.wslab_floats[1]) tb.wslab_floats[1] = side[i];
        tb.wslab_floats[0] = tb.wslab_floats[1];
        if (own > 4 * H * H && own > tb.wslab_floats[0]) tb.wslab_floats[0] = own;
        for (int i = 0; i < 2; ++i)
            if (tb.wslab_floats[i]) ICZ_TRY(alloc((void**)&tb.wslab[i], sizeof(float) * tb.wslab_floats[i]));
    }
    ICZ_TRY(alloc((void**)&tb.dWaff, sizeof(float) * A));
    ICZ_TRY(alloc((void**)&tb.scalars, sizeof(float) * 16));
    (void)V;
    ICZ_TRY(mem.synced());
    tb.B = B;
    tb.T = T;
    return ICZ_OK;
}

static DropCfg make_drop(const uint64_t* seed_p, bool train, const uint8_t* base, size_t per_step, uint32_t stream, int t, int row0 = 0) {
    DropCfg d = {0, nullptr, seed_p, stream, (uint32_t)t, row0};
    if (!train) return d;
    if (base) { d.mode = 1; d.mask = base + per_step * t; }
    else d.mode = 2;
    return d;
}

int Butd::train_step(const float* feats, int rows, int Bs, int t, bool train, hipStream_t st, bool emb_ready, int* pred_nsplit, bool skip_predict,
                     const int* live, int row0) {
    const size_t H = dims.H, D = dims.D, E = dims.E, A = dims.A, R = dims.R;
    const size_t Vp = round4(dims.V);
    const size_t slot = (size_t)t * Bs;
    StepIO s = {};
    s.emb_ready = emb_ready;
    s.rows = rows; s.feats = feats; s.it = tb.tok + slot;
    s.h1_in = tb.h1 + slot * H; s.c1_in = tb.c1 + slot * H; s.h2_in = tb.h2 + slot * H; s.c2_in = tb.c2 + slot * H;
    s.h1_out = tb.h1 + (slot + Bs) * H; s.c1_out = tb.c1 + (slot + Bs) * H;
    s.h2_out = tb.h2 + (slot + Bs) * H; s.c2_out = tb.c2 + (slot + Bs) * H;
    s.emb_out = tb.emb + slot * E;
    s.gates_td_out = tb.gtd + slot * 4 * H; s.gates_lm_out = tb.glm + slot * 4 * H;
    s.dec_ctx_out = tb.dec + slot * A; s.alpha_out = tb.alpha + slot * R; s.ctx_out = tb.ctx + slot * D;
    s.h2drop_out = tb.h2d + slot * H; s.logits_out = tb.logit + slot * Vp; s.logits_ld = (int)Vp;
    s.ws_alt = tb.X[0]; s.scores_alt = tb.dalpha;
    const size_t Bd = (size_t)(Bs - row0);
    s.drop_emb = make_drop(d_seed, train, rng.emb_mask, Bd * E, RNG_EMB, t, row0);
    s.drop_att = make_drop(d_seed, train, rng.att_mask, Bd * R * A, RNG_ATT, t, row0);
    s.drop_out = make_drop(d_seed, train, rng.out_mask, Bd * H, RNG_OUT, t, row0);
    if (row0 > 0) s.img_of_row = tb.img2;
    else if (cur_K > 1) {
        s.img_of_row = tb.imgk;
        s.rows_per_img = group_att ? cur_K : 1;
    }
    s.pred_nsplit = pred_nsplit;
    s.skip_predict = skip_predict;
    s.live = live;
    return step(s, st);
}

int Butd::sample(const float* feats, int B, int T, const icz_rng* r, int64_t* seq_out, float* logp_out, hipStream_t st) {
    ICZ_REQUIRE(feats && seq_out && logp_out && r, "butd sample: null argument");
    ICZ_REQUIRE(B > 0 && T > 0, "butd sample: bad B/T");
    ICZ_REQUIRE(fresh, "butd: call icz_butd_refresh_weights after binding/updating parameters");
    ICZ_TRY(ensure_train(B, T));
    rng = *r;
    hipLaunchKernelGGL(set_scalars_kernel, dim3(1), dim3(1), 0, st, d_seed, rng.seed, (float*)nullptr, 0.f);
    mode = 1; cur_B = B; cur_T = T; cur_train = true; cur_feats = feats;
    cur_rows = B; cur_row0 = 0; cur_K = 1; cur_nimg = B;
    rows_t.assign(T, B);
    cur_seq = seq_out; cur_logp = logp_out;
    const bool explicit_rng = rng.uniforms || rng.emb_mask || rng.att_mask || rng.out_mask;
    if (explicit_rng || !use_graphs) return sample_impl(feats, B, T, seq_out, logp_out, st);
    const std::vector<uintptr_t> key = {2, (uintptr_t)feats, (uintptr_t)B, (uintptr_t)T, (uintptr_t)seq_out, (uintptr_t)logp_out, opt_bits()};
    return gc.run(key, st, [&](hipStream_t s) { return sample_impl(feats, B, T, seq_out, logp_out, s); });
}

int Butd::sample_impl(const float* feats, int B, int T, int64_t* seq_out, float* logp_out, hipStream_t st) {
    ICZ_TRY(prologue(feats, B, st));
    return sample_chain(feats, B, T, seq_out, logp_out, st);
}

__global__ void imgk_init_kernel(int32_t* imgk, int rows, int K) {
    const int i = blockIdx.x * blockDim.x + threadIdx.x;
    if (i < rows) imgk[i] = i / K;
}

int Butd::sample_n(const float* feats, int B, int K, int T, const icz_rng* r, int64_t* seq_out, float* logp_out, hipStream_t st) {
    ICZ_REQUIRE(feats && seq_out && logp_out && r, "butd sample_n: null argument");
    ICZ_REQUIRE(K >= 2 && K <= ATT_CTX_MAX_G, "butd sample_n: K=%d samples per image outside 2..%d", K, ATT_CTX_MAX_G);
    ICZ_REQUIRE(B > 0 && T > 0, "butd sample_n: bad B/T");
    ICZ_REQUIRE((int64_t)B * K <= dims.max_rows, "butd sample_n: %d images x %d samples exceed the row capacity %d", B, K, dims.max_rows);
    ICZ_REQUIRE(fresh, "butd: call icz_butd_refresh_weights after binding/updating parameters");
    const int rows = B * K;
    ICZ_TRY(ensure_train(rows, T));
    rng = *r;
    hipLaunchKernelGGL(set_scalars_kernel, dim3(1), dim3(1), 0, st, d_seed, rng.seed, (float*)nullptr, 0.f);
    mode = 1; cur_B = rows; cur_T = T; cur_train = true; cur_feats = feats;
    cur_rows = rows; cur_row0 = 0; cur_K = K; cur_nimg = B;
    rows_t.assign(T, rows);
    cur_seq = seq_out; cur_logp = logp_out;
    const bool explicit_rng = rng.uniforms || rng.emb_mask || rng.att_mask || rng.out_mask;
    if (explicit_rng || !use_graphs) return sample_n_impl(feats, B, K, T, seq_out, logp_out, st);
    const std::vector<uintptr_t> key = {5, (uintptr_t)feats, (uintptr_t)B, (uintptr_t)K, (uintptr_t)T, (uintptr_t)seq_out, (uintptr_t)logp_out, opt_bits()};
    return gc.run(key, st, [&](hipStream_t s) { return sample_n_impl(feats, B, K, T, seq_out, logp_out, s); });
}

int Butd::sample_n_impl(const float* feats, int B, int K, int T, int64_t* seq_out, float* logp_out, hipStream_t st) {
    ICZ_TRY(prologue(feats, B, st));
    hipLaunchKernelGGL(imgk_init_kernel, dim3(cdiv(B * K, 256)), dim3(256), 0, st, tb.imgk, B * K, K);
    return sample_chain(feats, B * K, T, seq_out, logp_out, st);
}

int Butd::rollouts(const float* feats, int B, int T, const icz_rng* r, int64_t* ids_out, int64_t* seq_out, float* logp_out,
                   hipStream_t st) {
    ICZ_REQUIRE(feats && ids_out && seq_out && logp_out && r, "butd rollouts: null argument");
    ICZ_REQUIRE(B > 0 && T > 0 && B <= dims.max_rows, "butd rollouts: bad B/T");
    ICZ_REQUIRE(fresh, "butd: call icz_butd_refresh_weights after binding/updating parameters");
    const bool merged = B <= merge_small;
    ICZ_TRY(ensure_train(merged ? 2 * B : B, T));
    ICZ_TRY(side.ensure());
    rng = *r;
    hipLaunchKernelGGL(set_scalars_kernel, dim3(1), dim3(1), 0, st, d_seed, rng.seed, (float*)nullptr, 0.f);
    mode = 1; cur_B = B; cur_T = T; cur_train = true; cur_feats = feats;
    cur_rows = merged ? 2 * B : B; cur_row0 = merged ? B : 0; cur_K = 1; cur_nimg = B;
    rows_t.assign(T, B);
    cur_seq = seq_out; cur_logp = logp_out;
    const bool explicit_rng = rng.uniforms || rng.emb_mask || rng.att_mask || rng.out_mask;
    if (explicit_rng || !use_graphs) return rollouts_impl(feats, B, T, ids_out, seq_out, logp_out, st);
    const std::vector<uintptr_t> key = {4, (uintptr_t)feats, (uintptr_t)B, (uintptr_t)T, (uintptr_t)ids_out, (uintptr_t)seq_out, (uintptr_t)logp_out, opt_bits()};
    return gc.run(key, st, [&](hipStream_t s) { return rollouts_impl(feats, B, T, ids_out, seq_out, logp_out, s); });
}

int Butd::rollouts_impl(const float* feats, int B, int T, int64_t* ids_out, int64_t* seq_out, float* logp_out, hipStream_t st) {
    ICZ_TRY(prologue(feats, B, st));
    if (cur_row0 > 0) return sample_chain(feats, B, T, seq_out, logp_out, st, cur_row0, ids_out);
    if (!concurrent) {
        ICZ_TRY(greedy_chain(feats, B, T, ids_out, nullptr, st, true));
        return sample_chain(feats, B, T, seq_out, logp_out, st);
    }
    ICZ_CHECK_HIP(hipEventRecord(side.fork[0], st));
    ICZ_CHECK_HIP(hipStreamWaitEvent(side.st, side.fork[0], 0));
    const int ss = sample_chain(feats, B, T, seq_out, logp_out, st);
    const int sg = greedy_chain(feats, B, T, ids_out, nullptr, side.st, true);
    ICZ_CHECK_HIP(hipEventRecord(side.join[0], side.st));
    ICZ_CHECK_HIP(hipStreamWaitEvent(st, side.join[0], 0));
    return sg != ICZ_OK ? sg : ss;
}

__global__ void merged_init_kernel(int32_t* img2, int B, int* nany, int T, int64_t* tok_greedy) {
    const int i = blockIdx.x * blockDim.x + threadIdx.x;
// ... 62 lines not shown
    bptt_early_out = true;
    ICZ_TRY(bptt_prelude(st));
    const bool explicit_rng = rng.uniforms || rng.emb_mask || rng.att_mask || rng.out_mask;
    if (explicit_rng || !use_graphs) return sample_backward_impl(reward, *G, loss_out, mask_sum_out, st);
    std::vector<uintptr_t> key = {3, (uintptr_t)reward, (uintptr_t)loss_out, (uintptr_t)mask_sum_out, (uintptr_t)cur_B, (uintptr_t)cur_T,
                                  (uintptr_t)cur_feats, (uintptr_t)cur_seq, (uintptr_t)cur_logp,
                                  (uintptr_t)cur_rows, (uintptr_t)cur_row0,
                                  (uintptr_t)cur_K};
    const float* const* gp = reinterpret_cast<const float* const*>(G);
    for (size_t i = 0; i < sizeof(icz_butd_params) / sizeof(float*); ++i) key.push_back((uintptr_t)gp[i]);
    const icz_butd_params Gc = *G;
    if (!grad_cb) {
        key.push_back(opt_bits());
        return gc.run(key, st, [&](hipStream_t s) { return sample_backward_impl(reward, Gc, loss_out, mask_sum_out, s); });
    }
    for (int ph = 0; ph < 4; ++ph) {
        std::vector<uintptr_t> k2 = key;
        k2.push_back(0x100 + ph);
        k2.push_back(opt_bits());
        ICZ_TRY(gc.run(k2, st, [&](hipStream_t s) { return sample_backward_impl(reward, Gc, loss_out, mask_sum_out, s, 1 << ph, false); }));
        if (ph < 3) grad_cb(grad_cb_user, ph);
    }
    return ICZ_OK;
}

int Butd::sample_backward_impl(const float* reward, const icz_butd_params& G, float* loss_out, float* mask_sum_out, hipStream_t st,
                               int phases, bool fire_cb) {
    if (phases & 1) ICZ_TRY(reinforce(reward, tb.logit, dims.V, round4(dims.V), loss_out, mask_sum_out, st, cur_rows, cur_row0));
    return bptt(G, st, phases, fire_cb);
}

int Butd::xe_forward(const float* feats, const int64_t* captions, int B, int L, const int32_t* lengths, const icz_rng* r,
                     int train, float* packed_out, hipStream_t st) {
    ICZ_REQUIRE(feats && captions && lengths && B > 0 && L > 1, "butd xe_forward: bad arguments");
    int T = 0;
    ICZ_TRY(xe_steps("butd", lengths, B, L, &T));
    ICZ_TRY(ensure_train(B, T));
    if (r) rng = *r; else { rng = {}; }
    ICZ_REQUIRE(!train || r, "butd xe_forward: training mode needs an icz_rng");
    begin_xe(lengths, B, T, L, captions, train != 0, rng.seed, st);
    cur_feats = feats;
    cur_rows = B; cur_row0 = 0; cur_K = 1; cur_nimg = B;
    const size_t H = dims.H;
    const size_t Vp = round4(dims.V);
    ICZ_TRY(prologue(feats, B, st));
    ICZ_CHECK_HIP(hipMemsetAsync(tb.h1, 0, sizeof(float) * B * H, st));
    ICZ_CHECK_HIP(hipMemsetAsync(tb.c1, 0, sizeof(float) * B * H, st));
    ICZ_CHECK_HIP(hipMemsetAsync(tb.h2, 0, sizeof(float) * B * H, st));
    ICZ_CHECK_HIP(hipMemsetAsync(tb.c2, 0, sizeof(float) * B * H, st));
    ICZ_CHECK_HIP(hipMemsetAsync(tb.logit, 0, sizeof(float) * (size_t)T * B * Vp, st));
    captions_to_tok(tb.tok, st);
    const bool batched_predict = ss_prob <= 0.f && T * B >= 128;
    const bool batched_embed = ss_prob <= 0.f && T <= EMB_MAX_T && dims.E % 4 == 0;
    if (batched_embed) {
        EmbRows er = {};
        for (int t = 0; t < T; ++t) er.n[t] = rows_t[t];
        hipLaunchKernelGGL(embed_steps_kernel, dim3(cdiv(dims.E, 1024), T * B), dim3(256), 0, st, P.embed_weight, tb.tok, tb.emb, B, dims.E, er,
                           make_drop(d_seed, train != 0, rng.emb_mask, (size_t)B * dims.E, RNG_EMB, 0));
    }
    for (int t = 0; t < T; ++t) {
        if (t >= 2 && ss_prob > 0.f)
            ICZ_TRY(ss_select_launch(st, rows_t[t], tb.logit + (size_t)(t - 1) * B * Vp, (int)Vp, dims.V, t, B, ss_prob, ss_gate, ss_draw,
                                     d_seed, tb.tok + (size_t)t * B));
        ICZ_TRY(train_step(feats, rows_t[t], B, t, train != 0, st, batched_embed, nullptr, batched_predict));
    }
    if (batched_predict) {
        GemmArgs g = {};
        g.nseg = 1;
        g.seg[0] = {tb.h2d, w_pred, (int)H, (int)H, (int)H, nullptr};
        g.M = T * B; g.N = dims.V; g.out = tb.logit; g.ldo = (int)Vp; g.bias = P.predict_b; g.nsplit = 1;
        ICZ_TRY(gemm_f32(GEMM_NT, g, st));
    }
    if (packed_out) ICZ_TRY(gather_packed(tb.logit, dims.V, (int)Vp, packed_out, st));
    ICZ_CHECK_HIP(hipGetLastError());
    return ICZ_OK;
}

int Butd::xe_backward_dlogits(const float* dpacked, const icz_butd_params* G, hipStream_t st) {
    ICZ_TRY(require_mode(2, "butd"));
    ICZ_REQUIRE(dpacked && G, "butd xe_backward_dlogits: null argument");
    ICZ_TRY(scatter_packed(dpacked, dims.V, round4(dims.V), tb.logit, st));
    mode = 0;
    bptt_early_out = false;
    ICZ_TRY(bptt_prelude(st));
    return bptt(*G, st);
}

__global__ void transpose_coef_kernel(const float* __restrict__ dlogp, int n, float* __restrict__ coef) {
    int i = blockIdx.x * blockDim.x + threadIdx.x;
    if (i < n) coef[i] = dlogp[i];
}

int Butd::sample_backward_dlogp(const float* dlogp, const icz_butd_params* G, hipStream_t st) {
    ICZ_TRY(require_mode(1, "butd"));
    ICZ_REQUIRE(dlogp && G, "butd sample_backward_dlogp: null argument");
    const int B = cur_B, T = cur_T;
    const int Vp = round4(dims.V);
    ICZ_CHECK_HIP(hipMemcpyAsync(coef, dlogp, sizeof(float) * B * T, hipMemcpyDeviceToDevice, st));
    hipLaunchKernelGGL(reinforce_dlogits_kernel, dim3(cdiv(Vp, 256), T * cur_rows), dim3(256), 0, st, tb.logit, dims.V, Vp,
                       draw, lse, coef, B, T, cur_rows, cur_row0);
    ICZ_CHECK_HIP(hipGetLastError());
    mode = 0;
    bptt_early_out = true;
    ICZ_TRY(bptt_prelude(st));
    return bptt(*G, st);
}

int Butd::xe_backward(float smoothing, const icz_butd_params* G, float* loss_out, float n_tokens_global, hipStream_t st) {
    ICZ_TRY(require_mode(2, "butd"));
    ICZ_REQUIRE(G, "butd xe_backward: null grads");
    ICZ_TRY(xe_loss(smoothing, n_tokens_global, tb.logit, dims.V, round4(dims.V), loss_out, st));
    bptt_early_out = false;
    ICZ_TRY(bptt_prelude(st));
    return bptt(*G, st);
}

int Butd::gemm_auto(GemmLayout layout, GemmArgs& g, float* slab, size_t slab_floats, int* ns_out, hipStream_t st) {
    g.nsplit = g.M <= 64 ? gemm_pick_split(g, STEP_WGS, layout) : gemm_pick_split_balanced(g, layout, slab ? slab_floats : 0);
    if (g.nsplit > 1) {
        ICZ_REQUIRE(slab && gemm_slab_floats(g.M, g.N, g.nsplit) <= slab_floats, "butd: slab buffer too small (%d x %d x %d)", g.nsplit, g.M, g.N);
        g.out = slab; g.ldo = g.N; g.bias = nullptr; g.accumulate = 0;
    }
    if (ns_out) *ns_out = g.nsplit;
    return gemm_f32(layout, g, st);
}

int Butd::wgrad(const float* dY, int ldy, int M, const float* X, int ldx, int N, int K, float* out, int ldo, hipStream_t st, const int* rows_live) {
    float* const slab = tb.wslab[st == low.st ? 1 : 0];
    const size_t slab_floats = tb.wslab_floats[st == low.st ? 1 : 0];
    if (slab && ldo == N) {
        const int ns = gemm_tn_split_pick(M, N, K);
        if (ns > 1 && (size_t)ns * M * N <= slab_floats && ((size_t)M * N) % 4 == 0) {
            ICZ_TRY(gemm_tn_split(dY, ldy, M, X, ldx, N, K, ns, slab, rows_live, st));
            const size_t MN = (size_t)M * N;
            hipLaunchKernelGGL(slab_reduce_kernel, dim3(cdiv((int)(MN / 4), 256)), dim3(256), 0, st, (const float*)slab, ns, MN, N, (const float*)nullptr, out);
            ICZ_CHECK_HIP(hipGetLastError());
            return ICZ_OK;
        }
    }
    GemmArgs g = {};
    g.nseg = 1;
    g.rows_live = rows_live;
    g.seg[0] = {dY, X, ldy, ldx, K, nullptr};
    g.M = M; g.N = N; g.out = out; g.ldo = ldo; g.nsplit = 1;
    return gemm_f32(GEMM_TN, g, st);
}

int Butd::colsum(const float* X, int K, int N, int ldx, float* out, hipStream_t st) {
    hipLaunchKernelGGL(colsum_kernel, dim3(cdiv(N, 32)), dim3(256), 0, st, X, K, N, ldx, out);
    return ICZ_OK;
}

int Butd::bptt_prelude(hipStream_t st) {
    if (wt_lm_ih && !wt_fresh) ICZ_TRY(refresh_transposes(st));
    return ICZ_OK;
}

int Butd::bptt(const icz_butd_params& G, hipStream_t st, int phases, bool fire_cb) {
    const int B = cur_B, T = cur_T, Bs = cur_rows, roff = cur_row0;
    const int H = dims.H, D = dims.D, E = dims.E, A = dims.A, R = dims.R, V = dims.V;
    const int Vp = round4(V);
    const int TB = T * Bs;
    const float* feats = cur_feats;
    const size_t sH = (size_t)Bs * H;
    const int* const rl = (bptt_early_out && early_out) ? live_rows : nullptr;
    const int K = cur_K, n_img = K > 1 ? cur_nimg : B;
    const int32_t* const imgk = K > 1 ? tb.imgk : nullptr;

    ICZ_TRY(low.ensure(true));
    hipEvent_t ev_fork = low.fork[0], ev_join = low.join[0];
    if (phases & 1) {
    bptt_joined = false;
    auto side_branch = [&]() -> int {
        ICZ_CHECK_HIP(hipStreamWaitEvent(low.st, ev_fork, 0));
        hipStream_t sb = concurrent ? low.st : st;
        int s1 = wgrad(tb.logit, Vp, Vp, tb.h2d, H, H, TB, tb.dWp, H, sb, rl);
        hipLaunchKernelGGL(colsum_kernel, dim3(cdiv(V, 32)), dim3(256), 0, sb, tb.logit, TB, V, (int)Vp, G.predict_b);
        hipLaunchKernelGGL(weight_norm_bwd_kernel, dim3(cdiv(V, 4)), dim3(256), 0, sb, tb.dWp, H, P.predict_v, P.predict_g, n_pred,
                           G.predict_v, G.predict_g, V, H);
        ICZ_CHECK_HIP(hipEventRecord(ev_join, sb));
        if (s1 != ICZ_OK) { (void)hipStreamWaitEvent(st, ev_join, 0); return s1; }
        return ICZ_OK;
    };
    ICZ_CHECK_HIP(hipEventRecord(ev_fork, st));
    {
        GemmArgs g = {};
        g.nseg = 1;
        g.seg[0] = {tb.logit, w_pred, Vp, H, Vp, nullptr};
        g.M = TB; g.N = H; g.out = tb.dH2d; g.ldo = H; g.rows_live = rl;
        int ns;
        const int sg = gemm_auto(GEMM_NN, g, ws, ws_floats, &ns, st);
        if (sg != ICZ_OK) return sg;
        if (ns > 1) {
            size_t MN = (size_t)TB * H;
            hipLaunchKernelGGL(slab_reduce_kernel, dim3(cdiv((int)(MN / 4), 256)), dim3(256), 0, st, ws, ns, MN, H, (const float*)nullptr, tb.dH2d);
        }
    }
    ICZ_TRY(side_branch());
    const bool ragged = rows_t[T - 1] < B || roff > 0;
    if (ragged) {
        ICZ_CHECK_HIP(hipMemsetAsync(tb.dGtd, 0, sizeof(float) * (size_t)TB * 4 * H, st));
        ICZ_CHECK_HIP(hipMemsetAsync(tb.dGlm, 0, sizeof(float) * (size_t)TB * 4 * H, st));
        ICZ_CHECK_HIP(hipMemsetAsync(tb.dDec, 0, sizeof(float) * (size_t)TB * A, st));
        ICZ_CHECK_HIP(hipMemsetAsync(tb.dS, 0, sizeof(float) * (size_t)TB * R, st));
    }

    auto loop = [&]() -> int {
    int cur = 0;
    int ns1 = 1, ns2 = 1, ns3 = 1, ns4 = 1;
    int bnext = 0;
    for (int t = T - 1; t >= 0; --t) {
        const int bt = rows_t[t];
        const size_t slot = (size_t)t * Bs + roff;
        const int* const live = (bptt_early_out && early_out && t > 0) ? nunf + (t - 1) : nullptr;
        const int* const carry_live = (bptt_early_out && early_out && t + 1 < T) ? nunf + t : nullptr;
        DropCfg d_out = make_drop(d_seed, cur_train, rng.out_mask, (size_t)B * H, RNG_OUT, t);
        DropCfg d_att = make_drop(d_seed, cur_train, rng.att_mask, (size_t)B * R * A, RNG_ATT, t);
        DropCfg d_off = {0, nullptr, nullptr, 0, 0};
        {
            LstmBwdArgs a = {};
            a.dh_a = bnext ? tb.X[2] : nullptr; a.ns_a = ns3; a.lda_a = H; a.rows_a = bnext;
            a.dhdrop = tb.dH2d + slot * H;
            a.dc_in = bnext ? tb.dc2[cur] : nullptr; a.dc_in_rows = bnext;
            a.gates = tb.glm + slot * 4 * H;
            a.c_prev = tb.c2 + slot * H; a.c_cur = tb.c2 + slot * H + sH;
            a.dgates = tb.dGlm + slot * 4 * H; a.dc_prev = tb.dc2[cur ^ 1];
            a.rows = bt; a.H = H; a.live = live; a.carry_live = carry_live;
            hipLaunchKernelGGL(lstm_bwd_point_kernel, dim3(cdiv(H, 256), bt), dim3(256), 0, st, a, d_out);
        }
        const bool rdg = wt_lm_ih && wt_fresh && bt > 32 && bt <= 64 && gemm_slab_floats(bt, D + H, 4 * H / 256) <= tb.xfloats &&
                         gemm_slab_floats(bt, H, 2 * (4 * H / 256)) <= tb.xfloats;
        const bool tdg = small_nt && wt_lm_ih && wt_fresh && bt <= 32;
        if (rdg) {
            GemmArgs g = {};
            g.nseg = 1;
            g.seg[0] = {tb.dGlm + slot * 4 * H, wt_lm_ih, 4 * H, 4 * H, 4 * H, nullptr};
            g.M = bt; g.N = D + H; g.out = tb.X[0]; g.ldo = D + H; g.live = live;
            g.nsplit = ns1 = gemm_resident_x3_nsplit(g);
            ICZ_REQUIRE(gemm_slab_floats(bt, D + H, ns1) <= tb.xfloats, "butd: slab buffer too small for the dgrad slabs");
            ICZ_TRY(gemm_f32(GEMM_NT, g, st));
        } else if (tdg) {
            GemmArgs g = {};
            g.nseg = 1;
            g.seg[0] = {tb.dGlm + slot * 4 * H, wt_lm_ih, 4 * H, 4 * H, 4 * H, nullptr};
            g.M = bt; g.N = D + H; g.out = tb.X[0]; g.ldo = D + H; g.live = live;
            ICZ_TRY(gemm_auto(GEMM_NT, g, tb.X[0], tb.xfloats, &ns1, st));
        } else {
            GemmArgs g = {};
            g.nseg = 1;
            g.seg[0] = {tb.dGlm + slot * 4 * H, P.lm_w_ih, 4 * H, D + H, 4 * H, nullptr};
            g.M = bt; g.N = D + H; g.out = tb.X[0]; g.ldo = D + H; g.live = live;
            ICZ_TRY(gemm_auto(GEMM_NN, g, tb.X[0], tb.xfloats, &ns1, st));
        }
        {
            const int dparts = cdiv(D, DALPHA_COLS);
            hipLaunchKernelGGL(att_bwd_dalpha_kernel, dim3(bt, dparts), dim3(256), 0, st, tb.X[0], ns1, D + H, bt, feats, R, D, tb.dalpha, live, imgk);
            AttBwdDdecArgs da = {enc_ctx, tb.dec + slot * A, w_aff, tb.alpha + slot * R, tb.dalpha, tb.dDec + slot * A, tb.dS + slot * R, R, A, dparts, live, imgk};
            hipLaunchKernelGGL(att_bwd_ddec_kernel, dim3(bt, cdiv(A, 256)), dim3(256), 0, st, da, d_att);
            GemmArgs g = {};
            g.nseg = 1;
            g.seg[0] = {tb.dDec + slot * A, w_dec, A, H, A, nullptr};
            g.M = bt; g.N = H; g.out = tb.X[1]; g.ldo = H; g.live = live;
            ICZ_TRY(gemm_auto(GEMM_NN, g, tb.X[1], tb.xfloats, &ns2, st));
        }
        {
            LstmBwdArgs a = {};
            a.dh_a = bnext ? tb.X[3] : nullptr; a.ns_a = ns4; a.lda_a = H; a.rows_a = bnext;
            a.dh_b = tb.X[0] + D; a.ns_b = ns1; a.lda_b = D + H; a.rows_b = bt;
            a.dh_c = tb.X[1]; a.ns_c = ns2; a.lda_c = H; a.rows_c = bt;
            a.dc_in = bnext ? tb.dc1[cur] : nullptr; a.dc_in_rows = bnext;
            a.gates = tb.gtd + slot * 4 * H;
            a.c_prev = tb.c1 + slot * H; a.c_cur = tb.c1 + slot * H + sH;
            a.dgates = tb.dGtd + slot * 4 * H; a.dc_prev = tb.dc1[cur ^ 1];
            a.rows = bt; a.H = H; a.live = live; a.carry_live = carry_live;
            hipLaunchKernelGGL(lstm_bwd_point_kernel, dim3(cdiv(H, 256), bt), dim3(256), 0, st, a, d_off);
        }
        if (t > 0 && rdg) {
            GemmArgs g3 = {}, g4 = {};
            g3.nseg = 2;
            g3.seg[0] = {tb.dGlm + slot * 4 * H, wt_lm_hh, 4 * H, 4 * H, 4 * H, nullptr};
            g3.seg[1] = {tb.dGtd + slot * 4 * H, wt_td_ih_h2, 4 * H, 4 * H, 4 * H, nullptr};
            g3.M = bt; g3.N = H; g3.out = tb.X[2]; g3.ldo = H; g3.live = live;
            g4.nseg = 1; g4.live = live;
            g4.seg[0] = {tb.dGtd + slot * 4 * H, wt_td_hh, 4 * H, 4 * H, 4 * H, nullptr};
            g4.M = bt; g4.N = H; g4.out = tb.X[3]; g4.ldo = H;
            ns3 = gemm_resident_x3_nsplit(g3); ns4 = gemm_resident_x3_nsplit(g4);
            ICZ_REQUIRE(gemm_slab_floats(bt, H, ns3) <= tb.xfloats, "butd: slab buffer too small for the dgrad slabs");
            ICZ_TRY(gemm_resident_x3_pair(g3, g4, st));
        } else if (t > 0 && tdg) {
            {
                GemmArgs g = {};
                g.nseg = 2;
                g.seg[0] = {tb.dGlm + slot * 4 * H, wt_lm_hh, 4 * H, 4 * H, 4 * H, nullptr};
                g.seg[1] = {tb.dGtd + slot * 4 * H, wt_td_ih_h2, 4 * H, 4 * H, 4 * H, nullptr};
                g.M = bt; g.N = H; g.out = tb.X[2]; g.ldo = H; g.live = live;
                ICZ_TRY(gemm_auto(GEMM_NT, g, tb.X[2], tb.xfloats, &ns3, st));
            }
            {
                GemmArgs g = {};
                g.nseg = 1;
                g.seg[0] = {tb.dGtd + slot * 4 * H, wt_td_hh, 4 * H, 4 * H, 4 * H, nullptr};
                g.M = bt; g.N = H; g.out = tb.X[3]; g.ldo = H; g.live = live;
                ICZ_TRY(gemm_auto(GEMM_NT, g, tb.X[3], tb.xfloats, &ns4, st));
            }
        } else if (t > 0) {
            {
                GemmArgs g = {};
                g.nseg = 2;
                g.seg[0] = {tb.dGlm + slot * 4 * H, P.lm_w_hh, 4 * H, H, 4 * H, nullptr};
                g.seg[1] = {tb.dGtd + slot * 4 * H, P.td_w_ih, 4 * H, H + D + E, 4 * H, nullptr};
                g.M = bt; g.N = H; g.out = tb.X[2]; g.ldo = H; g.live = live;
                ICZ_TRY(gemm_auto(GEMM_NN, g, tb.X[2], tb.xfloats, &ns3, st));
            }
            {
                GemmArgs g = {};
                g.nseg = 1;
                g.seg[0] = {tb.dGtd + slot * 4 * H, P.td_w_hh, 4 * H, H, 4 * H, nullptr};
                g.M = bt; g.N = H; g.out = tb.X[3]; g.ldo = H; g.live = live;
                ICZ_TRY(gemm_auto(GEMM_NN, g, tb.X[3], tb.xfloats, &ns4, st));
            }
        }
        bnext = bt;
        cur ^= 1;
    }
    return ICZ_OK;
    };
    const int s_loop = loop();
    if (grad_cb || s_loop != ICZ_OK) {
        ICZ_CHECK_HIP(hipStreamWaitEvent(st, ev_join, 0));
        bptt_joined = true;
    }
    if (s_loop != ICZ_OK) return s_loop;
    }
    if ((phases & 1) && grad_cb && fire_cb) grad_cb(grad_cb_user, 0);
    const int ldtd = H + D + E, ldlm = D + H;
    const bool tail_side = phases == 0xF && !grad_cb && concurrent;
    if (tail_side) ICZ_CHECK_HIP(hipEventRecord(low.fork[1], st));
    bool tail_forked = false;
    hipStream_t const main_st = st;
    auto behind_loop = [&]() -> int {
    if (phases & 2) {
    {
        GemmArgs g = {};
        g.nseg = 1;
        g.seg[0] = {tb.dGtd, P.td_w_ih + H + D, 4 * H, H + D + E, 4 * H, nullptr};
        g.M = TB; g.N = E; g.out = tb.dEmb; g.ldo = E; g.rows_live = rl;
        int ns;
        ICZ_TRY(gemm_auto(GEMM_NN, g, ws, ws_floats, &ns, st));
        if (ns > 1) {
            size_t MN = (size_t)TB * E;
            hipLaunchKernelGGL(slab_reduce_kernel, dim3(cdiv((int)(MN / 4), 256)), dim3(256), 0, st, ws, ns, MN, E, (const float*)nullptr, tb.dEmb);
        }
        ICZ_CHECK_HIP(embed_grad_launch(st, tb.tok, TB, tb.dEmb, 1, (size_t)0, tb.emb, cur_train ? 2.0f : 1.0f, E, G.embed_weight, V, 1, rl));
    }
    const GemmColGroup td_groups[3] = {{tb.h2, H, H, G.td_w_ih, ldtd},
                                       {tb.emb, E, E, G.td_w_ih + H + D, ldtd},
                                       {tb.h1, H, H, G.td_w_hh, H}};
    const bool td_grouped = gemm_tn_grouped_fits(4 * H, TB, td_groups, 3);
    if (td_grouped) ICZ_TRY(gemm_tn_grouped(tb.dGtd, 4 * H, 4 * H, TB, td_groups, 3, rl, st));
    else ICZ_TRY(wgrad(tb.dGtd, 4 * H, 4 * H, tb.h2, H, H, TB, G.td_w_ih, ldtd, st, rl));
    hipLaunchKernelGGL(timesum_kernel, dim3(cdiv((int)((size_t)Bs * 4 * H / 4), 256)), dim3(256), 0, st, tb.dGtd, T, (size_t)Bs * 4 * H, tb.dGsum);
    if (K > 1) {
        float* const gimg = tb.dGsum + (size_t)Bs * 4 * H;
        const size_t N4 = (size_t)4 * H;
        hipLaunchKernelGGL(rowgroup_sum_kernel, dim3(cdiv((int)((size_t)n_img * N4 / 4), 256)), dim3(256), 0, st, (const float*)tb.dGsum, n_img, K, N4, gimg);
        ICZ_TRY(wgrad(gimg, 4 * H, 4 * H, mean, D, D, n_img, G.td_w_ih + H, ldtd, st));
    } else
        ICZ_TRY(wgrad(tb.dGsum + (size_t)roff * 4 * H, 4 * H, 4 * H, mean, D, D, B, G.td_w_ih + H, ldtd, st));
    if (!td_grouped) {
        ICZ_TRY(wgrad(tb.dGtd, 4 * H, 4 * H, tb.emb, E, E, TB, G.td_w_ih + H + D, ldtd, st, rl));
        ICZ_TRY(wgrad(tb.dGtd, 4 * H, 4 * H, tb.h1, H, H, TB, G.td_w_hh, H, st, rl));
    }
    }
    if ((phases & 2) && grad_cb && fire_cb) grad_cb(grad_cb_user, 1);
    if (phases & 4) {
    const GemmColGroup lm_groups[3] = {{tb.ctx, D, D, G.lm_w_ih, ldlm},
                                       {tb.h1 + sH, H, H, G.lm_w_ih + D, ldlm},
                                       {tb.h2, H, H, G.lm_w_hh, H}};
    if (gemm_tn_grouped_fits(4 * H, TB, lm_groups, 3)) {
        ICZ_TRY(gemm_tn_grouped(tb.dGlm, 4 * H, 4 * H, TB, lm_groups, 3, rl, st));
    } else {
        ICZ_TRY(wgrad(tb.dGlm, 4 * H, 4 * H, tb.ctx, D, D, TB, G.lm_w_ih, ldlm, st, rl));
        ICZ_TRY(wgrad(tb.dGlm, 4 * H, 4 * H, tb.h1 + sH, H, H, TB, G.lm_w_ih + D, ldlm, st, rl));
        ICZ_TRY(wgrad(tb.dGlm, 4 * H, 4 * H, tb.h2, H, H, TB, G.lm_w_hh, H, st, rl));
    }
    }
    if ((phases & 4) && grad_cb && fire_cb) grad_cb(grad_cb_user, 2);
    if (phases & 8) {
    if (tail_side) {
        ICZ_CHECK_HIP(hipStreamWaitEvent(low.st, low.fork[1], 0));
        tail_forked = true;
        st = low.st;
    }
    ICZ_TRY(wgrad(tb.dDec, A, A, tb.h1 + sH, H, H, TB, tb.dWdec, H, st));
    {
        AttBwdDencArgs ea = {enc_ctx, tb.dec + (size_t)roff * A, tb.dS + (size_t)roff * R, w_aff, tb.dEnc, tb.dwaff, B, R, A, T,
                             cur_train ? (rng.att_mask ? 1 : 2) : 0, rng.att_mask, (size_t)B * R * A, d_seed, (uint32_t)RNG_ATT, Bs, imgk};
        if (K > 1 && group_att) {
            ea.denc = tb.dEncImg;
            hipLaunchKernelGGL(att_bwd_denc_group_kernel<20>, dim3(n_img, ATT_PARTS), dim3(256), sizeof(float) * T * R, st, ea, K);
        } else {
            hipLaunchKernelGGL(att_bwd_denc_kernel<20>, dim3(B, ATT_PARTS), dim3(256), sizeof(float) * T * R, st, ea);
            if (K > 1) {
                const size_t N = (size_t)R * A;
                hipLaunchKernelGGL(rowgroup_sum_kernel, dim3(cdiv((int)((size_t)n_img * N / 4), 256)), dim3(256), 0, st, (const float*)tb.dEnc,
                                   n_img, K, N, tb.dEncImg);
            }
        }
    }
    const float* const denc = K > 1 ? tb.dEncImg : tb.dEnc;
    const int waff_rows = (K > 1 && group_att ? n_img : B) * ATT_PARTS;
    ICZ_TRY(wgrad(denc, A, A, feats, D, D, n_img * R, tb.dWenc, D, st));
    {
        ColsumTable ct = {};
        int nb = 0;
        auto add = [&](const float* X, int K, int N, int ldx, float* out, float* out2) {
            ct.j[ct.count++] = {X, K, N, ldx, out, out2, nb};
            nb += cdiv(N, 32);
        };
        add(tb.dGtd, TB, 4 * H, 4 * H, G.td_b_ih, G.td_b_hh);
        add(tb.dGlm, TB, 4 * H, 4 * H, G.lm_b_ih, G.lm_b_hh);
        add(tb.dDec, TB, A, A, G.dec_att_b, nullptr);
        add(denc, n_img * R, A, A, G.enc_att_b, nullptr);
        add(tb.dwaff, waff_rows, A, A, tb.dWaff, nullptr);
        add(tb.dwaff, 0, 1, 1, G.affine_b, nullptr);
        hipLaunchKernelGGL(colsum_multi_kernel, dim3(nb), dim3(256), 0, st, ct);
    }
    {
        WeightNormBwdTable wt = {};
        int nb = 0;
        auto add = [&](const float* dw, int lddw, const float* v, const float* g, const float* norm, float* dv, float* dg, int rows, int cols) {
            wt.j[wt.count++] = {dw, lddw, v, g, norm, dv, dg, rows, cols, nb};
            nb += cdiv(rows, 4);
        };
        add(tb.dWenc, D, P.enc_att_v, P.enc_att_g, n_enc, G.enc_att_v, G.enc_att_g, A, D);
        add(tb.dWdec, H, P.dec_att_v, P.dec_att_g, n_dec, G.dec_att_v, G.dec_att_g, A, H);
        add(tb.dWaff, A, P.affine_v, P.affine_g, n_aff, G.affine_v, G.affine_g, 1, A);
        hipLaunchKernelGGL(weight_norm_bwd_multi_kernel, dim3(nb), dim3(256), 0, st, wt);
    }
    }
    return ICZ_OK;
    };
    const int s_tail = behind_loop();
    st = main_st;
    if (tail_forked) {
        ICZ_CHECK_HIP(hipEventRecord(low.join[1], low.st));
        ICZ_CHECK_HIP(hipStreamWaitEvent(st, low.join[1], 0));
    }
    if (((phases & 8) || s_tail != ICZ_OK) && !bptt_joined) {
        ICZ_CHECK_HIP(hipStreamWaitEvent(st, ev_join, 0));
        bptt_joined = true;
    }
    if (s_tail != ICZ_OK) return s_tail;
    ICZ_CHECK_HIP(hipGetLastError());
    return ICZ_OK;
}

}

using namespace icz;
extern "C" {

int icz_butd_sample(icz_butd_t* h, const float* feats, int32_t B, int32_t max_len, const icz_rng* rng,
                    int64_t* seq_out, float* logprobs_out, void* stream) {
    ICZ_REQUIRE(h, "null handle");
    return reinterpret_cast<Butd*>(h)->sample(feats, B, max_len, rng, seq_out, logprobs_out, (hipStream_t)stream);
}
int icz_butd_sample_n(icz_butd_t* h, const float* feats, int32_t B, int32_t K, int32_t max_len, const icz_rng* rng,
                      int64_t* seq_out, float* logprobs_out, void* stream) {
    ICZ_REQUIRE(K >= 2 && K <= ATT_CTX_MAX_G, "icz_butd_sample_n: K=%d samples per image outside 2..%d", K, ATT_CTX_MAX_G);
    ICZ_REQUIRE(h, "icz_butd_sample_n: null handle");
    return reinterpret_cast<Butd*>(h)->sample_n(feats, B, K, max_len, rng, seq_out, logprobs_out, (hipStream_t)stream);
}
int icz_butd_scst_rollouts(icz_butd_t* h, const float* feats, int32_t B, int32_t max_len, const icz_rng* rng,
// ... 80 lines not shown
```

### simpleimagecaptionzoo_amd/csrc/gemm_f32.h

```cpp
#pragma once
#include "icz_common.h"

namespace icz {

constexpr int GEMM_MAX_SEG = 4;
constexpr int GEMM_BM = 64, GEMM_BN = 64, GEMM_BK = 64;

enum GemmLayout { GEMM_NT = 0, GEMM_NN = 1, GEMM_TN = 2 };

struct GemmSeg {
    const float* A;
    const float* B;
    int lda, ldb;
    int K;
    const int64_t* gather;
};

struct GemmArgs {
    GemmSeg seg[GEMM_MAX_SEG];
    int nseg;
    int M, N;
    float* out;
    int ldo;
    const float* bias;
    int nsplit;
    int chunks_per_split;
    int accumulate;
    int spread;
    const int* live;
    const int* rows_live;
};

int gemm_f32(GemmLayout layout, const GemmArgs& a, hipStream_t stream);
int gemm_route(GemmLayout layout, const GemmArgs& a);
int gemm_pick_split(const GemmArgs& a, int target_wgs, GemmLayout layout = GEMM_NT);
int gemm_pick_split_balanced(const GemmArgs& a, GemmLayout layout, size_t slab_capacity_floats);
size_t gemm_slab_floats(int M, int N, int nsplit);
int gemm_normalize_split(GemmLayout layout, const GemmArgs& a, int nsplit);
int gemm_fit_split(GemmLayout layout, const GemmArgs& a, int nsplit, size_t capacity_floats);

bool gemm_resident_x3_fits(const GemmArgs& a);
int gemm_resident_x3_stages(const GemmArgs& a);
int gemm_resident_x3_nsplit(const GemmArgs& a);
int gemm_resident_x3(const GemmArgs& a, hipStream_t stream);
bool gemm_resident_x3_pair_fits(const GemmArgs& a, const GemmArgs& b);
int gemm_resident_x3_pair(const GemmArgs& a, const GemmArgs& b, hipStream_t stream);
int gemm_predict(const float* x, int H, const float* w_pred, const float* bias, int rows, int V, int Vp, float* logits, int ldl,
                 float* ws, size_t ws_cap_floats, int* pred_nsplit, hipStream_t st, const int* live = nullptr);

int gemm_big_x3(GemmLayout layout, const GemmArgs& a, int cfg, hipStream_t stream);
int gemm_big_cfg(GemmLayout layout, const GemmArgs& a);
int gemm_big_switch();
void gemm_set_big_cfg(int cfg);
constexpr int GEMM_MAX_COLGROUPS = 4;
struct GemmColGroup { const float* B; int ldb; int cols; float* out; int ldo; };
bool gemm_tn_grouped_fits(int M, int K, const GemmColGroup* groups, int ngroups);
int gemm_tn_grouped(const float* dY, int ldy, int M, int K, const GemmColGroup* groups, int ngroups, const int* rows_live, hipStream_t stream);

int gemm_tn_split_pick(int M, int N, int K);
int gemm_tn_split(const float* dY, int ldy, int M, const float* X, int ldx, int N, int K, int nsplit, float* slabs, const int* rows_live, hipStream_t st);
struct GemmSwitches { bool tn_x3, nn_x3, nt_x3big, resident_x3, resident_m128, predict_slabs, resident_k512; unsigned prof_every; int big_cfg; };
const GemmSwitches& gemm_switches();

}
```

### simpleimagecaptionzoo_amd/csrc/gemm_f32.hip

```cpp
#include <stdlib.h>

#include <array>
#include <mutex>
#include <set>
#include <vector>

#include "gemm_f32.h"
#include "butd_kernels.h"

namespace icz {

static int total_chunks(const GemmArgs& a, int bk = GEMM_BK) {
    int t = 0;
    for (int s = 0; s < a.nseg; ++s) t += cdiv(a.seg[s].K, bk);
    return t;
}

template <int BK>
struct ChunkCursorT {
    int seg, k0;
    const float* A; const float* B;
    int lda, ldb, K;
    __device__ __forceinline__ void load_seg(const GemmArgs& a) {
        const GemmSeg& g = a.seg[seg];
// ... 1133 lines not shown
        for (int i = 0; i < 16; ++i) v[i] = __builtin_nontemporal_load(q + i * 256);
#pragma unroll
        for (int i = 0; i < 16; ++i) acc += v[i];
    }
    if (acc.x + acc.y + acc.z + acc.w == 1.2345e-30f) sink[0] = acc.x;
}

}

extern "C" {
int icz_prof_stream_rate(const void* buf, size_t bytes, int32_t reps, void* stream, double* gbs) {
    ICZ_REQUIRE(buf && gbs && reps > 0 && bytes >= (size_t)65536 * 1024 && bytes % 65536 == 0, "icz_prof_stream_rate: bad arguments");
    hipStream_t st = (hipStream_t)stream;
    float* sink = nullptr;
    ICZ_CHECK_HIP(hipMalloc((void**)&sink, 16));
    hipEvent_t e0, e1;
    ICZ_CHECK_HIP(hipEventCreate(&e0));
    ICZ_CHECK_HIP(hipEventCreate(&e1));
    const size_t nchunks = bytes / 65536;
    const int grid = 256 * 8;
    for (int i = 0; i < 2; ++i) hipLaunchKernelGGL(icz::stream_rate_kernel, dim3(grid), dim3(256), 0, st, (const icz::f32x4*)buf, nchunks, sink);
    ICZ_CHECK_HIP(hipEventRecord(e0, st));
    for (int i = 0; i < reps; ++i) hipLaunchKernelGGL(icz::stream_rate_kernel, dim3(grid), dim3(256), 0, st, (const icz::f32x4*)buf, nchunks, sink);
    ICZ_CHECK_HIP(hipEventRecord(e1, st));
    ICZ_CHECK_HIP(hipEventSynchronize(e1));
    float ms = 0.f;
    ICZ_CHECK_HIP(hipEventElapsedTime(&ms, e0, e1));
    (void)hipEventDestroy(e0); (void)hipEventDestroy(e1); (void)hipFree(sink);
    *gbs = (double)bytes * reps / (ms * 1e-3) / 1e9;
    return ICZ_OK;
}
int icz_prof_pair_overhead(void* stream, int32_t n, double* avg_us) { return icz::gemm_prof_pair_overhead((hipStream_t)stream, n, avg_us); }
int icz_prof_begin(void) { icz::gemm_prof_begin(); return ICZ_OK; }
int icz_kprof_begin(void) {
    icz::g_kprof.on = true;
    for (size_t& u : icz::g_kprof.used) u = 0;
    return ICZ_OK;
}
int icz_kprof_end(int32_t group, double* avg_us, long long* pairs) {
    ICZ_REQUIRE(group >= 0 && group < icz::KP_GROUPS && avg_us && pairs, "icz_kprof_end: bad arguments");
    icz::g_kprof.on = false;
    ICZ_CHECK_HIP(hipDeviceSynchronize());
    const size_t n = icz::g_kprof.used[group] / 2;
    double tot = 0.0;
    for (size_t i = 0; i < n; ++i) {
        float ms = 0.f;
        ICZ_CHECK_HIP(hipEventElapsedTime(&ms, icz::g_kprof.ev[group][2 * i], icz::g_kprof.ev[group][2 * i + 1]));
        tot += ms;
    }
    *avg_us = n ? tot * 1e3 / (double)n : 0.0;
    *pairs = (long long)n;
    return ICZ_OK;
}
int icz_prof_select(int32_t which) {
    if (which < 0 || which > 1) { icz::set_error("icz_prof_select: %d (0 = all skinny forward GEMMs, 1 = resident-activation kernel)", which); return ICZ_ERR_INVALID; }
    icz::gemm_prof_select(which);
    return ICZ_OK;
}
int icz_prof_end(double* avg_us, double* bytes_per_launch, double* flops_per_launch, long long* launches) {
    return icz::gemm_prof_end(avg_us, bytes_per_launch, flops_per_launch, launches);
}

using namespace icz;
static constexpr int ABI_TARGET_WGS = 512;

size_t icz_gemm_workspace_floats(int32_t M, int32_t N) {
    const size_t base = (size_t)ABI_TARGET_WGS * 4096 * 2 + (size_t)M * N;
    const size_t m128 = (M > 64 && M <= 128) ? (size_t)32 * M * N : 0;
    return base > m128 ? base : m128;
}

int icz_gemm_f32(int32_t layout, const float* X, int32_t ldx, const float* W, int32_t ldw, const float* bias,
                 float* C, int32_t ldc, int32_t M, int32_t N, int32_t K, int32_t nsplit, float* workspace,
                 size_t workspace_floats, void* stream) {
    ICZ_REQUIRE(layout >= 0 && layout <= 2, "icz_gemm_f32: layout %d", layout);
    GemmArgs g = {};
    g.nseg = 1;
    g.seg[0] = {X, W, ldx, ldw, K, nullptr};
    g.M = M; g.N = N; g.out = C; g.ldo = ldc; g.bias = bias;
    g.nsplit = nsplit > 0 ? nsplit : gemm_fit_split((GemmLayout)layout, g, gemm_pick_split(g, ABI_TARGET_WGS, (GemmLayout)layout), workspace_floats);
    g.nsplit = gemm_normalize_split((GemmLayout)layout, g, g.nsplit);
    hipStream_t st = (hipStream_t)stream;
    if (g.nsplit > 1) {
        ICZ_REQUIRE(workspace, "icz_gemm_f32: split-K needs a workspace");
        ICZ_REQUIRE(gemm_slab_floats(M, N, g.nsplit) <= workspace_floats, "icz_gemm_f32: workspace of %zu floats too small for %d slabs of %dx%d", workspace_floats, g.nsplit, M, N);
        ICZ_REQUIRE(ldc == N, "icz_gemm_f32: split-K path needs ldc == N");
        g.out = workspace; g.bias = nullptr;
        ICZ_TRY(gemm_f32((GemmLayout)layout, g, st));
        size_t MN = (size_t)M * N;
        ICZ_REQUIRE(MN % 4 == 0, "icz_gemm_f32: M*N must be a multiple of 4 for the split-K reduce");
        hipLaunchKernelGGL(slab_reduce_kernel, dim3(cdiv((int)(MN / 4), 256)), dim3(256), 0, st, workspace, g.nsplit, MN, N, bias, C);
        ICZ_CHECK_HIP(hipGetLastError());
        return ICZ_OK;
    }
    return gemm_f32((GemmLayout)layout, g, st);
}

int icz_gemm_set_big_cfg(int32_t cfg) {
    ICZ_REQUIRE(cfg >= -2 && cfg <= 5, "icz_gemm_set_big_cfg: %d", cfg);
    gemm_set_big_cfg(cfg);
    return ICZ_OK;
}

int icz_gemm_big_cfg_for(int32_t layout, int32_t M, int32_t N, int32_t K, int32_t nsplit) {
    if (layout < 0 || layout > 2 || M <= 0 || N <= 0 || K <= 0) return -1;
    GemmArgs g = {};
    g.nseg = 1;
    g.seg[0].K = K;
    g.M = M; g.N = N; g.nsplit = nsplit > 0 ? nsplit : 1;
    return gemm_big_cfg((GemmLayout)layout, g);
}

int icz_gemm_tn_grouped_fits(int32_t M, int32_t K, int32_t ngroups, const int32_t* cols) {
    if (M <= 0 || K <= 0 || ngroups < 1 || ngroups > GEMM_MAX_COLGROUPS || !cols) return -1;
    GemmColGroup g[GEMM_MAX_COLGROUPS] = {};
    for (int j = 0; j < ngroups; ++j) g[j].cols = cols[j];
    return gemm_tn_grouped_fits(M, K, g, ngroups) ? 1 : 0;
}

int icz_gemm_route_for(int32_t layout, int32_t M, int32_t N, int32_t nseg, const int32_t* K, int32_t nsplit) {
    if (layout < 0 || layout > 2 || M <= 0 || N <= 0 || nseg < 1 || nseg > GEMM_MAX_SEG || !K || nsplit < 0) return -1;
    GemmArgs g = {};
    g.nseg = nseg;
    for (int s = 0; s < nseg; ++s) {
        if (K[s] <= 0) return -1;
        g.seg[s].K = K[s];
    }
    g.M = M; g.N = N;
    g.nsplit = nsplit > 0 ? nsplit : gemm_pick_split(g, 256, (GemmLayout)layout);
    return gemm_route((GemmLayout)layout, g);
}

int icz_gemm_tn_split_pick(int32_t M, int32_t N, int32_t K) {
    if (M <= 0 || N <= 0 || K <= 0) return -1;
    return gemm_tn_split_pick(M, N, K);
}

int icz_gemm_tn_split(const float* dY, int32_t ldy, int32_t M, const float* X, int32_t ldx, int32_t N, int32_t K, float* out, int32_t ldo,
                      float* workspace, size_t workspace_floats, const int32_t* rows_live, void* stream) {
    ICZ_REQUIRE(dY && X && out && M > 0 && N > 0 && K > 0 && ldy >= M && ldx >= N, "icz_gemm_tn_split: bad arguments");
    ICZ_REQUIRE(ldo == N, "icz_gemm_tn_split: the slab sum writes a dense output (ldo %d, N %d)", ldo, N);
    const int ns = gemm_tn_split_pick(M, N, K);
    ICZ_REQUIRE(ns > 1, "icz_gemm_tn_split: shape not taken (M %d N %d K %d): issue it through icz_gemm_f32", M, N, K);
    const size_t MN = (size_t)M * N;
    ICZ_REQUIRE(workspace && (size_t)ns * MN <= workspace_floats, "icz_gemm_tn_split: workspace of %zu floats too small for %d slabs of %d x %d", workspace_floats, ns, M, N);
    ICZ_REQUIRE(((uintptr_t)out & 15) == 0, "icz_gemm_tn_split: output must be 16-byte aligned");
    hipStream_t st = (hipStream_t)stream;
    ICZ_TRY(gemm_tn_split(dY, ldy, M, X, ldx, N, K, ns, workspace, rows_live, st));
    hipLaunchKernelGGL(slab_reduce_kernel, dim3(cdiv((int)(MN / 4), 256)), dim3(256), 0, st, (const float*)workspace, ns, MN, N, (const float*)nullptr, out);
    ICZ_CHECK_HIP(hipGetLastError());
    return ICZ_OK;
}

int icz_gemm_tn_grouped(const float* dY, int32_t ldy, int32_t M, int32_t K, int32_t ngroups, const float* const* X, const int32_t* ldx,
                        const int32_t* cols, float* const* out, const int32_t* ldo, const int32_t* rows_live, void* stream) {
    ICZ_REQUIRE(ngroups >= 1 && ngroups <= GEMM_MAX_COLGROUPS && X && ldx && cols && out && ldo, "icz_gemm_tn_grouped: bad arguments");
    GemmColGroup g[GEMM_MAX_COLGROUPS];
    for (int j = 0; j < ngroups; ++j) g[j] = {X[j], ldx[j], cols[j], out[j], ldo[j]};
    ICZ_REQUIRE(gemm_tn_grouped_fits(M, K, g, ngroups), "icz_gemm_tn_grouped: shape not taken (M %d, K %d)", M, K);
    return gemm_tn_grouped(dY, ldy, M, K, g, ngroups, rows_live, (hipStream_t)stream);
}
}
```

### simpleimagecaptionzoo_amd/csrc/gemm_resident_x3.hip

```cpp
#include <stdlib.h>

#include <type_traits>

#include "gemm_f32.h"

namespace icz {

template <int I, int N, class F>
__device__ __forceinline__ void sk_static_for(F&& f) {
    if constexpr (I < N) {
        f(std::integral_constant<int, I>{});
        sk_static_for<I + 1, N>(f);
    }
}

typedef __attribute__((ext_vector_type(8))) __bf16 sk_bf16x8;
typedef __attribute__((ext_vector_type(4))) uint32_t sk_u32x4;
typedef __attribute__((ext_vector_type(2))) uint32_t sk_u32x2;

__device__ __forceinline__ uint32_t sk_cvt_pk_bf16(float lo, float hi) {
    uint32_t r;
    asm("v_cvt_pk_bf16_f32 %0, %1, %2" : "=v"(r) : "v"(lo), "v"(hi));
    return r;
}
// ... 428 lines not shown
        if constexpr (i == TPW * HS) {
            __builtin_amdgcn_sched_barrier(0);
            __syncthreads();
            split_x(xr2);
            __syncthreads();
            __builtin_amdgcn_sched_barrier(0);
            stamp(19);
        }
        if constexpr (HAS_LOAD) point_w(std::integral_constant<int, i + D - 1>{});
        const unsigned short* abase = planes + (size_t)li * RS_PB + 64 * hst + 8 * lq;
        sk_bf16x8 af[2][3];
        sk_static_for<0, 3>([&](auto pp) { af[0][decltype(pp)::value] = *reinterpret_cast<const sk_bf16x8*>(abase + decltype(pp)::value * PLANE); });
        sk_static_for<0, G>([&](auto gc) {
            constexpr int g = decltype(gc)::value, b = g / MT, t = g % MT;
            __builtin_amdgcn_sched_barrier(0);
            if constexpr (g + 1 < G) {
                constexpr int b1 = (g + 1) / MT, t1 = (g + 1) % MT;
                const unsigned short* ap = abase + (size_t)t1 * 16 * RS_PB + 32 * b1;
                sk_static_for<0, 3>([&](auto pp) { af[(g + 1) & 1][decltype(pp)::value] = *reinterpret_cast<const sk_bf16x8*>(ap + decltype(pp)::value * PLANE); });
            }
            constexpr bool X2_LOAD = i < 2 && g % 2 == 0;
            if constexpr (HAS_LOAD)
                sk_static_for<g * LW / G, (g + 1) * LW / G>([&](auto lc) { load_w1(std::integral_constant<int, (S + D - 1) % D>{}, lc); });
            if constexpr (X2_LOAD) load_x1(xr2, HS, std::integral_constant<int, i * (G / 2) + g / 2>{});
            if constexpr (b == 0 || HAS_NEXT) {
                sk_static_for<t * WP / MT, (t + 1) * WP / MT>([&](auto pc) {
                    if constexpr (b == 0) w_piece(std::integral_constant<int, S>{}, std::integral_constant<int, 1>{}, pc, std::integral_constant<int, 1>{});
                    else w_piece(std::integral_constant<int, (S + 1) % D>{}, std::integral_constant<int, 0>{}, pc, std::integral_constant<int, 1>{});
                });
            }
            sk_static_for<0, NCT>([&](auto cc) {
                constexpr int c = decltype(cc)::value;
                const sk_bf16x8 b0 = __builtin_bit_cast(sk_bf16x8, bq[0][c][0]), b1_ = __builtin_bit_cast(sk_bf16x8, bq[0][c][1]),
                                b2 = __builtin_bit_cast(sk_bf16x8, bq[0][c][2]);
                f32x4 v = acc[t][tile * NCT + c];
                v = __builtin_amdgcn_mfma_f32_16x16x32_bf16(b0, af[g & 1][2], v, 0, 0, 0);
                v = __builtin_amdgcn_mfma_f32_16x16x32_bf16(b2, af[g & 1][0], v, 0, 0, 0);
                v = __builtin_amdgcn_mfma_f32_16x16x32_bf16(b1_, af[g & 1][1], v, 0, 0, 0);
                v = __builtin_amdgcn_mfma_f32_16x16x32_bf16(b0, af[g & 1][1], v, 0, 0, 0);
                v = __builtin_amdgcn_mfma_f32_16x16x32_bf16(b1_, af[g & 1][0], v, 0, 0, 0);
                v = __builtin_amdgcn_mfma_f32_16x16x32_bf16(b0, af[g & 1][0], v, 0, 0, 0);
                acc[t][tile * NCT + c] = v;
            });
            __builtin_amdgcn_sched_group_barrier(0x100, 3, 0);
            if constexpr (HAS_LOAD || X2_LOAD)
                __builtin_amdgcn_sched_group_barrier(0x020, (HAS_LOAD ? (g + 1) * LW / G - g * LW / G : 0) + (X2_LOAD ? 1 : 0), 0);
#pragma unroll
            for (int k = 0; k < 6 * NCT; ++k) {
                __builtin_amdgcn_sched_group_barrier(0x008, 1, 0);
                __builtin_amdgcn_sched_group_barrier(0x002, 1, 0);
            }
            if constexpr (t == MT - 1) {
                __builtin_amdgcn_sched_barrier(0);
                sk_static_for<0, NCT * 3>([&](auto q) { bq[0][decltype(q)::value / 3][decltype(q)::value % 3] = bq[1][decltype(q)::value / 3][decltype(q)::value % 3]; });
            }
        });
        stamp(3 + i);
        if constexpr (i >= TPW * HS && i % HS == HS - 1) {
            store_tile(std::integral_constant<int, tile>{});
            stamp(12 + tile);
        }
    });
    stamp(31);
}

template <int D, bool STAMPS = false>
__global__ __launch_bounds__(256) void gemm_resident_x3_m128_kernel(GemmArgs a) {
    resident_x3_m128_body<D, STAMPS>(a, blockIdx.x);
}
constexpr size_t rs_m128_lds_bytes() { return (size_t)3 * 128 * rs_pb(2) * 2; }

static int rs_total_stages(const GemmArgs& a) {
    int tot = 0;
    for (int s = 0; s < a.nseg; ++s) tot += a.seg[s].K / SK_BK;
    return tot;
}
int gemm_resident_x3_stages(const GemmArgs& a) {
    const int tot = rs_total_stages(a);
    if (gemm_switches().resident_k512 && a.M <= 64 && tot % 8 == 0) return 8;
    return tot % 4 == 0 ? 4 : 0;
}
static bool rs_shape_ok(const GemmArgs& a) {
    if (!gemm_switches().resident_x3 || a.M <= 32 || a.M > (gemm_switches().resident_m128 ? 128 : 64) || a.N % 4 || a.accumulate) return false;
    for (int s = 0; s < a.nseg; ++s)
        if (a.seg[s].K % SK_BK || a.seg[s].gather) return false;
    return rs_total_stages(a) >= 8 && gemm_resident_x3_stages(a) > 0;
}
bool gemm_resident_x3_fits(const GemmArgs& a) { return a.N >= 2048 && rs_shape_ok(a); }
int gemm_resident_x3_nsplit(const GemmArgs& a) { return rs_total_stages(a) / gemm_resident_x3_stages(a); }

template <int NSR, bool STAMPS>
static int rs_launch(const GemmArgs& a, hipStream_t stream) {
    constexpr size_t lds = rs_lds_bytes<4, NSR>();
    static bool attr = false;
    if (!attr) {
        ICZ_CHECK_HIP(hipFuncSetAttribute(reinterpret_cast<const void*>(gemm_resident_x3_kernel<4, NSR, 2, 3, STAMPS>), hipFuncAttributeMaxDynamicSharedMemorySize, (int)lds));
        attr = true;
    }
    hipLaunchKernelGGL((gemm_resident_x3_kernel<4, NSR, 2, 3, STAMPS>), dim3(cdiv(a.N, 256) * a.nsplit), dim3(256), lds, stream, a);
    ICZ_CHECK_HIP(hipGetLastError());
    return ICZ_OK;
}

#ifndef RS_K512_D
#define RS_K512_D 3
#endif
template <bool STAMPS>
static int rs_launch_k512(const GemmArgs& a, hipStream_t stream) {
    constexpr size_t lds = rs_lds_bytes<4, 4>();
    static bool attr = false;
    if (!attr) {
        ICZ_CHECK_HIP(hipFuncSetAttribute(reinterpret_cast<const void*>(gemm_resident_x3_kernel<4, 8, 1, RS_K512_D, STAMPS, 4>), hipFuncAttributeMaxDynamicSharedMemorySize, (int)lds));
        attr = true;
    }
    hipLaunchKernelGGL((gemm_resident_x3_kernel<4, 8, 1, RS_K512_D, STAMPS, 4>), dim3(cdiv(a.N, 128) * a.nsplit), dim3(256), lds, stream, a);
    ICZ_CHECK_HIP(hipGetLastError());
    return ICZ_OK;
}

template <bool STAMPS>
static int rs_launch_m128(const GemmArgs& a, hipStream_t stream) {
    constexpr size_t lds = rs_m128_lds_bytes();
    static bool attr = false;
    if (!attr) {
        ICZ_CHECK_HIP(hipFuncSetAttribute(reinterpret_cast<const void*>(gemm_resident_x3_m128_kernel<3, STAMPS>), hipFuncAttributeMaxDynamicSharedMemorySize, (int)lds));
        attr = true;
    }
    hipLaunchKernelGGL((gemm_resident_x3_m128_kernel<3, STAMPS>), dim3(cdiv(a.N, 256) * a.nsplit), dim3(256), lds, stream, a);
    ICZ_CHECK_HIP(hipGetLastError());
    return ICZ_OK;
}

#ifdef ICZ_DEV
static unsigned long long* g_sk_stamps = nullptr;
static int rs_dev_env(const char* name) { const char* e = getenv(name); return e ? atoi(e) : 0; }
#endif

int gemm_resident_x3(const GemmArgs& a_in, hipStream_t stream) {
    GemmArgs a = a_in;
    const int nsr = gemm_resident_x3_stages(a);
    ICZ_REQUIRE(rs_shape_ok(a) && a.nsplit == gemm_resident_x3_nsplit(a) && a.chunks_per_split == nsr,
                "gemm_resident_x3: launch does not match the kernel's fixed decomposition (nsplit %d)", a.nsplit);
    ICZ_REQUIRE(a.nsplit > 1 || a.ldo >= a.N, "gemm_resident_x3: output row stride %d below N = %d", a.ldo, a.N);
#ifdef ICZ_DEV
    if (rs_dev_env("ICZ_DEV_STAMPS")) {
        if (!g_sk_stamps) ICZ_CHECK_HIP(hipMalloc((void**)&g_sk_stamps, sizeof(unsigned long long) * 32 * 4096));
        a.bias = reinterpret_cast<const float*>(g_sk_stamps);
        return a.M > 64 ? rs_launch_m128<true>(a, stream) : (nsr == 8 ? rs_launch_k512<true>(a, stream) : rs_launch<4, true>(a, stream));
    }
#endif
    return a.M > 64 ? rs_launch_m128<false>(a, stream) : (nsr == 8 ? rs_launch_k512<false>(a, stream) : rs_launch<4, false>(a, stream));
}

bool gemm_resident_x3_pair_fits(const GemmArgs& a, const GemmArgs& b) {
    return a.M <= 64 && b.M <= 64 && rs_shape_ok(a) && rs_shape_ok(b) && gemm_resident_x3_stages(a) == gemm_resident_x3_stages(b) && a.N >= 512 && b.N >= 512;
}
int gemm_resident_x3_pair(const GemmArgs& a_in, const GemmArgs& b_in, hipStream_t stream) {
    ICZ_REQUIRE(gemm_resident_x3_pair_fits(a_in, b_in), "gemm_resident_x3_pair: shapes outside the kernel's decomposition");
    GemmPair g;
    g.a = a_in; g.b = b_in;
    const int nsr = gemm_resident_x3_stages(g.a), tilew = nsr == 8 ? 128 : 256;
    for (GemmArgs* p : {&g.a, &g.b}) {
        p->nsplit = gemm_resident_x3_nsplit(*p);
        p->chunks_per_split = nsr;
        p->bias = nullptr;
        ICZ_REQUIRE(p->out && p->nsplit > 1, "gemm_resident_x3_pair: slab output expected");
    }
    g.first = cdiv(g.a.N, tilew) * g.a.nsplit;
    constexpr size_t lds = rs_lds_bytes<4, 4>();
    static bool attr = false;
    if (!attr) {
        ICZ_CHECK_HIP(hipFuncSetAttribute(reinterpret_cast<const void*>(gemm_resident_x3_pair_kernel<4, 4, 2, 3>), hipFuncAttributeMaxDynamicSharedMemorySize, (int)lds));
        ICZ_CHECK_HIP(hipFuncSetAttribute(reinterpret_cast<const void*>(gemm_resident_x3_pair_kernel<4, 8, 1, RS_K512_D, 4>), hipFuncAttributeMaxDynamicSharedMemorySize, (int)lds));
        attr = true;
    }
    const dim3 grid(g.first + cdiv(g.b.N, tilew) * g.b.nsplit);
    if (nsr == 8) hipLaunchKernelGGL((gemm_resident_x3_pair_kernel<4, 8, 1, RS_K512_D, 4>), grid, dim3(256), lds, stream, g);
    else hipLaunchKernelGGL((gemm_resident_x3_pair_kernel<4, 4, 2, 3>), grid, dim3(256), lds, stream, g);
    ICZ_CHECK_HIP(hipGetLastError());
    return ICZ_OK;
}

int gemm_predict(const float* x, int H, const float* w_pred, const float* bias, int rows, int V, int Vp, float* logits, int ldl,
                 float* ws, size_t ws_cap_floats, int* pred_nsplit, hipStream_t st, const int* live) {
    GemmArgs g = {};
    g.nseg = 1;
    g.live = live;
    g.seg[0] = {x, w_pred, H, H, H, nullptr};
    g.M = rows; g.N = Vp; g.out = ws; g.ldo = Vp;
    if (gemm_switches().predict_slabs && pred_nsplit && ws && gemm_resident_x3_fits(g) && gemm_resident_x3_nsplit(g) > 1 &&
        gemm_slab_floats(rows, Vp, gemm_resident_x3_nsplit(g)) <= ws_cap_floats) {
        g.nsplit = gemm_resident_x3_nsplit(g);
        *pred_nsplit = g.nsplit;
    } else {
        g.N = V; g.out = logits; g.ldo = ldl; g.bias = bias;
        g.nsplit = 1;
        if (pred_nsplit) *pred_nsplit = 1;
    }
    return gemm_f32(GEMM_NT, g, st);
}

}

#ifdef ICZ_DEV
extern "C" int icz_debug_skinny_stamps(unsigned long long* out_host, int n_workgroups) {
    if (!icz::g_sk_stamps || n_workgroups > 4096) return -1;
    return hipMemcpy(out_host, icz::g_sk_stamps, sizeof(unsigned long long) * 32 * n_workgroups, hipMemcpyDeviceToHost) == hipSuccess ? 0 : -2;
}
#endif
```

Before: 11950.

## Rebalance BPTT dgrad GEMMs: pair lm_hh with lm_ih, split td pair

In the LSTM backward loop, the recurrent dgrad for the language LSTM's hidden weights is moved into a paired resident launch with the input dgrad GEMM. The top-down LSTM dgrads are then run as a separate balanced pair with one tile per workgroup. The carry gradient becomes the sum of two slab sets, read by the pointwise kernel through a new second input. The aim is to even out per-step GEMM work and shorten the serial critical path, at the cost of an extra slab buffer and more slab summation in the pointwise kernel.

```diff
diff --git a/include/icz.h b/include/icz.h
--- a/include/icz.h
+++ b/include/icz.h
@@ -45,6 +45,8 @@
 int icz_butd_destroy(icz_butd_t* h);
 int icz_butd_bind_params(icz_butd_t* h, const icz_butd_params* params);
 int icz_butd_set_option(icz_butd_t* h, const char* name, int32_t value);
+int icz_butd_dgrad_route_counts(icz_butd_t* h, int32_t* out4);
+int icz_butd_transposed_dgrad_possible(int32_t D, int32_t H);
 int icz_butd_set_mask_sum_global(icz_butd_t* h, const float* mask_sum_global_dev, void* stream);
 typedef void (*icz_grad_ready_cb)(void* user, int32_t stage);
 int icz_butd_set_grad_callback(icz_butd_t* h, icz_grad_ready_cb cb, void* user);
@@ -287,6 +289,8 @@
 int icz_gemm_tn_split_pick(int32_t M, int32_t N, int32_t K);
 int icz_gemm_tn_split(const float* dY, int32_t ldy, int32_t M, const float* X, int32_t ldx, int32_t N, int32_t K, float* out, int32_t ldo,
                       float* workspace, size_t workspace_floats, const int32_t* rows_live, void* stream);
+int icz_gemm_resident_pair(const float* Xa, const float* Wa, float* Ca, const float* Xb, const float* Wb, float* Cb, int32_t M, int32_t N,
+                           int32_t K, int32_t stages, int32_t tiles, float* workspace, size_t workspace_floats, void* stream);
 int icz_gemm_route_for(int32_t layout, int32_t M, int32_t N, int32_t nseg, const int32_t* K, int32_t nsplit);
 int icz_gemm_tn_grouped_fits(int32_t M, int32_t K, int32_t ngroups, const int32_t* cols);
 int icz_prof_begin(void);
diff --git a/simpleimagecaptionzoo_amd/_lib.py b/simpleimagecaptionzoo_amd/_lib.py
--- a/simpleimagecaptionzoo_amd/_lib.py
+++ b/simpleimagecaptionzoo_amd/_lib.py
@@ -221,6 +221,9 @@
         "icz_gemm_tn_split_pick": (C.c_int, [i32, i32, i32]),
         "icz_gemm_tn_split": (C.c_int, [vp, i32, i32, vp, i32, i32, i32, vp, i32, vp, C.c_size_t, vp, vp]),
         "icz_gemm_route_for": (C.c_int, [i32, i32, i32, i32, vp, i32]),
+        "icz_gemm_resident_pair": (C.c_int, [vp, vp, vp, vp, vp, vp, i32, i32, i32, i32, i32, vp, C.c_size_t, vp]),
+        "icz_butd_dgrad_route_counts": (C.c_int, [vp, vp]),
+        "icz_butd_transposed_dgrad_possible": (C.c_int, [i32, i32]),
         "icz_gemm_tn_grouped_fits": (C.c_int, [i32, i32, i32, vp]),
     }
     for name, (res, args) in sig.items():
diff --git a/simpleimagecaptionzoo_amd/butd.py b/simpleimagecaptionzoo_amd/butd.py
--- a/simpleimagecaptionzoo_amd/butd.py
+++ b/simpleimagecaptionzoo_amd/butd.py
@@ -154,6 +154,30 @@
     return out
 
 
+def gemm_resident_pair(Xa, Wa, Xb, Wb, stages, tiles):
+    M, K = Xa.shape
+    N = Wa.shape[0]
+    assert Xb.shape == Xa.shape and Wb.shape == Wa.shape and all(t.is_contiguous() for t in (Xa, Wa, Xb, Wb))
+    Ca, Cb = (torch.empty(M, N, device=Xa.device, dtype=torch.float32) for _ in range(2))
+    ws = torch.empty(2 * max(K // (64 * stages), 1) * M * N, device=Xa.device, dtype=torch.float32)
+    check(lib().icz_gemm_resident_pair(ptr(Xa), ptr(Wa), ptr(Ca), ptr(Xb), ptr(Wb), ptr(Cb), M, N, K, int(stages), int(tiles), ptr(ws),
+                                       ws.numel(), stream_ptr()))
+    return Ca, Cb
+
+
+DGRAD_ROUTES = ("nn", "small_nt", "resident", "resident_balanced")
+
+
+def dgrad_route_counts(handle):
+    out = (C.c_int32 * 4)()
+    check(lib().icz_butd_dgrad_route_counts(handle._h, out))
+    return dict(zip(DGRAD_ROUTES, (int(v) for v in out)))
+
+
+def transposed_dgrad_possible(D, H):
+    return int(lib().icz_butd_transposed_dgrad_possible(int(D), int(H))) == 1
+
+
 GEMM_ROUTES = ("nt_fp32_mt1", "nt_fp32_mt2", "nt_fp32_mt4", "resident_4stage", "resident_512deep", "resident_128row", "x3_128tile",
                "large_tile", "nn_fp32", "tn_fp32_64", "tn_fp32_128")
 
diff --git a/simpleimagecaptionzoo_amd/csrc/butd.hip b/simpleimagecaptionzoo_amd/csrc/butd.hip
--- a/simpleimagecaptionzoo_amd/csrc/butd.hip
+++ b/simpleimagecaptionzoo_amd/csrc/butd.hip
@@ -51,6 +51,7 @@
     ICZ_TRY(mem.synced());
     if (const char* e = getenv("ICZ_EARLY_OUT")) early_out = atoi(e) != 0;
     if (const char* e = getenv("ICZ_MERGE_SMALL")) { const int n = atoi(e); if (n >= 0 && n <= 32) merge_small = n; }
+    if (const char* e = getenv("ICZ_BPTT_DGRAD_BALANCE")) dgrad_balance = atoi(e) != 0;
     return ICZ_OK;
 }
 
@@ -74,15 +75,26 @@
     return ICZ_OK;
 }
 
-bool Butd::wt_possible() const {
+static GemmArgs wt_shape(int K, int N, int nseg = 1) {
+    static const float placeholder = 0.f;
     GemmArgs g = {};
-    g.nseg = 1;
-    g.seg[0] = {w_enc, w_enc, 4 * dims.H, 4 * dims.H, 4 * dims.H, nullptr};
-    g.M = 64; g.N = dims.D + dims.H;
-    GemmArgs p = g, q = g;
-    p.N = q.N = dims.H;
-    p.nseg = 2; p.seg[1] = p.seg[0];
-    return dims.H % 64 == 0 && dims.D % 64 == 0 && gemm_resident_x3_fits(g) && gemm_resident_x3_pair_fits(p, q);
+    g.nseg = nseg;
+    for (int s = 0; s < nseg; ++s) g.seg[s] = {&placeholder, &placeholder, K, K, K, nullptr};
+    g.M = 64; g.N = N;
+    return g;
+}
+bool Butd::wt_possible_for(int D, int H) {
+    if (H <= 0 || D <= 0 || H % 64 || D % 64) return false;
+    const GemmArgs x1 = wt_shape(4 * H, D + H), xh = wt_shape(4 * H, H);
+    if (!gemm_resident_x3_fits(x1)) return false;
+    const int nsr = gemm_resident_x3_stages(x1);
+    return gemm_resident_x3_pair_fits(x1, xh, nsr, nsr == 8 ? 1 : 2) && gemm_resident_x3_pair_fits(xh, xh, 4, 1);
+}
+bool Butd::wt_possible() const { return wt_possible_for(dims.D, dims.H); }
+bool Butd::wt_legacy_pair() const {
+    const GemmArgs x3 = wt_shape(4 * dims.H, dims.H, 2), x4 = wt_shape(4 * dims.H, dims.H);
+    const int nsr = gemm_resident_x3_stages(x3);
+    return nsr > 0 && nsr == gemm_resident_x3_stages(x4) && gemm_resident_x3_pair_fits(x3, x4, nsr, nsr == 8 ? 1 : 2);
 }
 
 int Butd::refresh_transposes(hipStream_t st) {
@@ -345,6 +357,7 @@
     if (strcmp(name, "early_out") == 0) { b->early_out = value != 0; return ICZ_OK; }
     if (strcmp(name, "small_nt") == 0) { b->small_nt = value != 0; return ICZ_OK; }
     if (strcmp(name, "group_att") == 0) { b->group_att = value != 0; return ICZ_OK; }
+    if (strcmp(name, "dgrad_balance") == 0) { b->dgrad_balance = value != 0; return ICZ_OK; }
     if (strcmp(name, "merge_small") == 0) {
         ICZ_REQUIRE(value >= 0 && value <= 32, "icz_butd_set_option: merge_small %d outside 0..32", value);
         b->merge_small = value;
@@ -353,6 +366,15 @@
     set_error("icz_butd_set_option: unknown option '%s'", name);
     return ICZ_ERR_INVALID;
 }
+
+int icz_butd_dgrad_route_counts(icz_butd_t* h, int32_t* out4) {
+    ICZ_REQUIRE(h && out4, "icz_butd_dgrad_route_counts: null argument");
+    const Butd* b = reinterpret_cast<const Butd*>(h);
+    for (int i = 0; i < 4; ++i) out4[i] = b->dgrad_steps[i];
+    return ICZ_OK;
+}
+
+int icz_butd_transposed_dgrad_possible(int32_t D, int32_t H) { return Butd::wt_possible_for(D, H) ? 1 : 0; }
 
 int icz_butd_set_mask_sum_global(icz_butd_t* h, const float* mask_sum_global_dev, void* stream) {
     return set_norm_global("icz_butd_set_mask_sum_global", reinterpret_cast<Butd*>(h), mask_sum_global_dev, stream);
diff --git a/simpleimagecaptionzoo_amd/csrc/butd_impl.h b/simpleimagecaptionzoo_amd/csrc/butd_impl.h
--- a/simpleimagecaptionzoo_amd/csrc/butd_impl.h
+++ b/simpleimagecaptionzoo_amd/csrc/butd_impl.h
@@ -46,6 +46,7 @@
     float *dwaff = nullptr, *dalpha = nullptr, *dS = nullptr, *dGsum = nullptr;
     float *dc1[2] = {nullptr, nullptr}, *dc2[2] = {nullptr, nullptr};
     float* X[4] = {nullptr, nullptr, nullptr, nullptr}; size_t xfloats = 0;
+    float* X3a = nullptr; size_t x3a_floats = 0;
     float *dWp = nullptr, *dWenc = nullptr, *dWdec = nullptr, *dWaff = nullptr, *scalars = nullptr;
     float* wslab[2] = {nullptr, nullptr}; size_t wslab_floats[2] = {0, 0};
 };
@@ -71,6 +72,8 @@
     float *wt_lm_ih = nullptr, *wt_lm_hh = nullptr, *wt_td_ih_h2 = nullptr, *wt_td_hh = nullptr;
     bool wt_fresh = false;
     bool wt_possible() const;
+    bool wt_legacy_pair() const;
+    static bool wt_possible_for(int D, int H);
     int refresh_transposes(hipStream_t st);
 
     int alloc(void** p, size_t bytes) { return mem.alloc(p, bytes); }
@@ -86,7 +89,7 @@
     bool use_graphs = false;
     bool concurrent = true;
     uintptr_t opt_bits() const {
-        return (concurrent ? 1 : 0) + (early_out ? 2 : 0) + 4 * merge_small + (small_nt ? 256 : 0) + (group_att ? 512 : 0);
+        return (concurrent ? 1 : 0) + (early_out ? 2 : 0) + 4 * merge_small + (small_nt ? 256 : 0) + (group_att ? 512 : 0) + (dgrad_balance ? 1024 : 0);
     }
     int greedy_impl(const float* feats, int B, int max_len, int64_t* ids_out, float* alphas_out, hipStream_t st);
     int sample_impl(const float* feats, int B, int T, int64_t* seq_out, float* logp_out, hipStream_t st);
@@ -105,6 +108,8 @@
     bool early_out = true;
     bool bptt_early_out = false;
     bool small_nt = true;
+    bool dgrad_balance = true;
+    int dgrad_steps[4] = {0, 0, 0, 0};
     int cur_K = 1, cur_nimg = 0;
     bool group_att = false;
 
diff --git a/simpleimagecaptionzoo_amd/csrc/butd_kernels.h b/simpleimagecaptionzoo_amd/csrc/butd_kernels.h
--- a/simpleimagecaptionzoo_amd/csrc/butd_kernels.h
+++ b/simpleimagecaptionzoo_amd/csrc/butd_kernels.h
@@ -1219,6 +1219,7 @@
 struct LstmBwdArgs {
     const float* dh_a; int ns_a;
     int lda_a;
+    const float* dh_a2; int ns_a2;
     const float* dh_b; int ns_b; int lda_b;
     const float* dh_c; int ns_c; int lda_c;
     const float* dhdrop;
@@ -1253,7 +1254,10 @@
     }
     const bool carry = cflag != 0;
     float dh = 0.f;
-    if (a.dh_a && carry && row < a.rows_a) dh += sum_slabs1(a.dh_a, a.ns_a, (size_t)a.rows_a * a.lda_a, (size_t)row * a.lda_a + j);
+    if (a.dh_a && carry && row < a.rows_a) {
+        dh += sum_slabs1(a.dh_a, a.ns_a, (size_t)a.rows_a * a.lda_a, (size_t)row * a.lda_a + j);
+        if (a.dh_a2) dh += sum_slabs1(a.dh_a2, a.ns_a2, (size_t)a.rows_a * a.lda_a, (size_t)row * a.lda_a + j);
+    }
     if (a.dh_b && row < a.rows_b) dh += sum_slabs1(a.dh_b, a.ns_b, (size_t)a.rows_b * a.lda_b, (size_t)row * a.lda_b + j);
     if (a.dh_c && row < a.rows_c) dh += sum_slabs1(a.dh_c, a.ns_c, (size_t)a.rows_c * a.lda_c, (size_t)row * a.lda_c + j);
     if (a.dhdrop) {
diff --git a/simpleimagecaptionzoo_amd/csrc/butd_train.hip b/simpleimagecaptionzoo_amd/csrc/butd_train.hip
--- a/simpleimagecaptionzoo_amd/csrc/butd_train.hip
+++ b/simpleimagecaptionzoo_amd/csrc/butd_train.hip
@@ -32,6 +32,7 @@
         ICZ_TRY(alloc((void**)&wt_td_hh, sizeof(float) * G4 * dims.H));
         wt_fresh = false;
     }
+    const bool with_wt = wt_lm_ih != nullptr;
     DeviceBuffers::TrainingScope scope(mem);
     const size_t H = dims.H, D = dims.D, E = dims.E, A = dims.A, R = dims.R, V = dims.V;
     const size_t Vp = round4(dims.V);
@@ -75,6 +76,10 @@
         if (need > tb.xfloats) tb.xfloats = need;
     }
     for (int i = 0; i < 4; ++i) ICZ_TRY(alloc((void**)&tb.X[i], sizeof(float) * tb.xfloats));
+    if (with_wt) {
+        tb.x3a_floats = gemm_slab_floats(64, (int)H, (int)(4 * H / 256));
+        ICZ_TRY(alloc((void**)&tb.X3a, sizeof(float) * tb.x3a_floats));
+    }
     ICZ_TRY(alloc((void**)&tb.dWp, sizeof(float) * Vp * H));
     ICZ_TRY(alloc((void**)&tb.dWenc, sizeof(float) * A * D));
     ICZ_TRY(alloc((void**)&tb.dWdec, sizeof(float) * A * H));
@@ -443,7 +448,7 @@
 }
 
 int Butd::bptt_prelude(hipStream_t st) {
-    if (wt_lm_ih && !wt_fresh) ICZ_TRY(refresh_transposes(st));
+    if (wt_lm_ih && !wt_fresh && (dgrad_balance || wt_legacy_pair())) ICZ_TRY(refresh_transposes(st));
     return ICZ_OK;
 }
 
@@ -499,7 +504,12 @@
     auto loop = [&]() -> int {
     int cur = 0;
     int ns1 = 1, ns2 = 1, ns3 = 1, ns4 = 1;
+    const float* carry_a = tb.X[2];
+    const float* carry_b = nullptr;
+    int ns3b = 0;
     int bnext = 0;
+    for (int& c : dgrad_steps) c = 0;
+    const bool wt_ok = wt_lm_ih && wt_fresh && (dgrad_balance || wt_legacy_pair());
     for (int t = T - 1; t >= 0; --t) {
         const int bt = rows_t[t];
         const size_t slot = (size_t)t * Bs + roff;
@@ -510,7 +520,8 @@
         DropCfg d_off = {0, nullptr, nullptr, 0, 0};
         {
             LstmBwdArgs a = {};
-            a.dh_a = bnext ? tb.X[2] : nullptr; a.ns_a = ns3; a.lda_a = H; a.rows_a = bnext;
+            a.dh_a = bnext ? carry_a : nullptr; a.ns_a = ns3; a.lda_a = H; a.rows_a = bnext;
+            a.dh_a2 = bnext ? carry_b : nullptr; a.ns_a2 = ns3b;
             a.dhdrop = tb.dH2d + slot * H;
             a.dc_in = bnext ? tb.dc2[cur] : nullptr; a.dc_in_rows = bnext;
             a.gates = tb.glm + slot * 4 * H;
@@ -519,9 +530,13 @@
             a.rows = bt; a.H = H; a.live = live; a.carry_live = carry_live;
             hipLaunchKernelGGL(lstm_bwd_point_kernel, dim3(cdiv(H, 256), bt), dim3(256), 0, st, a, d_out);
         }
-        const bool rdg = wt_lm_ih && wt_fresh && bt > 32 && bt <= 64 && gemm_slab_floats(bt, D + H, 4 * H / 256) <= tb.xfloats &&
-                         gemm_slab_floats(bt, H, 2 * (4 * H / 256)) <= tb.xfloats;
-        const bool tdg = small_nt && wt_lm_ih && wt_fresh && bt <= 32;
+        const bool rdg = wt_ok && bt > 32 && bt <= 64 && gemm_slab_floats(bt, D + H, 4 * H / 256) <= tb.xfloats &&
+                         gemm_slab_floats(bt, H, 2 * (4 * H / 256)) <= tb.xfloats &&
+                         (!dgrad_balance || gemm_slab_floats(bt, H, 4 * H / 256) <= tb.x3a_floats);
+        const bool bal = rdg && dgrad_balance;
+        const bool tdg = small_nt && wt_ok && bt <= 32;
+        ++dgrad_steps[bal ? 3 : rdg ? 2 : tdg ? 1 : 0];
+        int ns3a = 0;
         if (rdg) {
             GemmArgs g = {};
             g.nseg = 1;
@@ -529,7 +544,17 @@
             g.M = bt; g.N = D + H; g.out = tb.X[0]; g.ldo = D + H; g.live = live;
             g.nsplit = ns1 = gemm_resident_x3_nsplit(g);
             ICZ_REQUIRE(gemm_slab_floats(bt, D + H, ns1) <= tb.xfloats, "butd: slab buffer too small for the dgrad slabs");
-            ICZ_TRY(gemm_f32(GEMM_NT, g, st));
+            if (bal && t > 0) {
+                GemmArgs g3 = {};
+                g3.nseg = 1;
+                g3.seg[0] = {tb.dGlm + slot * 4 * H, wt_lm_hh, 4 * H, 4 * H, 4 * H, nullptr};
+                g3.M = bt; g3.N = H; g3.out = tb.X3a; g3.ldo = H; g3.live = live;
+                const int nsr = gemm_resident_x3_stages(g);
+                ns3a = ns1;
+                ICZ_REQUIRE(gemm_slab_floats(bt, H, ns3a) <= tb.x3a_floats, "butd: slab buffer too small for the dgrad slabs");
+                ICZ_TRY(gemm_resident_x3_pair(g, g3, nsr, nsr == 8 ? 1 : 2, st));
+            } else
+                ICZ_TRY(gemm_f32(GEMM_NT, g, st));
         } else if (tdg) {
             GemmArgs g = {};
             g.nseg = 1;
@@ -566,7 +591,19 @@
             a.rows = bt; a.H = H; a.live = live; a.carry_live = carry_live;
             hipLaunchKernelGGL(lstm_bwd_point_kernel, dim3(cdiv(H, 256), bt), dim3(256), 0, st, a, d_off);
         }
-        if (t > 0 && rdg) {
+        if (t > 0 && bal) {
+            GemmArgs g3 = {}, g4 = {};
+            g3.nseg = 1; g3.live = live;
+            g3.seg[0] = {tb.dGtd + slot * 4 * H, wt_td_ih_h2, 4 * H, 4 * H, 4 * H, nullptr};
+            g3.M = bt; g3.N = H; g3.out = tb.X[2]; g3.ldo = H;
+            g4.nseg = 1; g4.live = live;
+            g4.seg[0] = {tb.dGtd + slot * 4 * H, wt_td_hh, 4 * H, 4 * H, 4 * H, nullptr};
+            g4.M = bt; g4.N = H; g4.out = tb.X[3]; g4.ldo = H;
+            ns3b = ns4 = 4 * H / 256;
+            ICZ_REQUIRE(gemm_slab_floats(bt, H, ns4) <= tb.xfloats, "butd: slab buffer too small for the dgrad slabs");
+            ICZ_TRY(gemm_resident_x3_pair(g3, g4, 4, 1, st));
+            ns3 = ns3a; carry_a = tb.X3a; carry_b = tb.X[2];
+        } else if (t > 0 && rdg) {
             GemmArgs g3 = {}, g4 = {};
             g3.nseg = 2;
             g3.seg[0] = {tb.dGlm + slot * 4 * H, wt_lm_hh, 4 * H, 4 * H, 4 * H, nullptr};
@@ -577,7 +614,8 @@
             g4.M = bt; g4.N = H; g4.out = tb.X[3]; g4.ldo = H;
             ns3 = gemm_resident_x3_nsplit(g3); ns4 = gemm_resident_x3_nsplit(g4);
             ICZ_REQUIRE(gemm_slab_floats(bt, H, ns3) <= tb.xfloats, "butd: slab buffer too small for the dgrad slabs");
-            ICZ_TRY(gemm_resident_x3_pair(g3, g4, st));
+            const int nsr = gemm_resident_x3_stages(g3);
+            ICZ_TRY(gemm_resident_x3_pair(g3, g4, nsr, nsr == 8 ? 1 : 2, st));
         } else if (t > 0 && tdg) {
             {
                 GemmArgs g = {};
@@ -611,6 +649,7 @@
                 ICZ_TRY(gemm_auto(GEMM_NN, g, tb.X[3], tb.xfloats, &ns4, st));
             }
         }
+        if (!(t > 0 && bal)) { carry_a = tb.X[2]; carry_b = nullptr; ns3b = 0; }
         bnext = bt;
         cur ^= 1;
     }
diff --git a/simpleimagecaptionzoo_amd/csrc/gemm_f32.h b/simpleimagecaptionzoo_amd/csrc/gemm_f32.h
--- a/simpleimagecaptionzoo_amd/csrc/gemm_f32.h
+++ b/simpleimagecaptionzoo_amd/csrc/gemm_f32.h
@@ -43,8 +43,8 @@
 int gemm_resident_x3_stages(const GemmArgs& a);
 int gemm_resident_x3_nsplit(const GemmArgs& a);
 int gemm_resident_x3(const GemmArgs& a, hipStream_t stream);
-bool gemm_resident_x3_pair_fits(const GemmArgs& a, const GemmArgs& b);
-int gemm_resident_x3_pair(const GemmArgs& a, const GemmArgs& b, hipStream_t stream);
+bool gemm_resident_x3_pair_fits(const GemmArgs& a, const GemmArgs& b, int nsr, int tpw);
+int gemm_resident_x3_pair(const GemmArgs& a, const GemmArgs& b, int nsr, int tpw, hipStream_t stream);
 int gemm_predict(const float* x, int H, const float* w_pred, const float* bias, int rows, int V, int Vp, float* logits, int ldl,
                  float* ws, size_t ws_cap_floats, int* pred_nsplit, hipStream_t st, const int* live = nullptr);
 
diff --git a/simpleimagecaptionzoo_amd/csrc/gemm_f32.hip b/simpleimagecaptionzoo_amd/csrc/gemm_f32.hip
--- a/simpleimagecaptionzoo_amd/csrc/gemm_f32.hip
+++ b/simpleimagecaptionzoo_amd/csrc/gemm_f32.hip
@@ -1309,6 +1309,27 @@
     return ICZ_OK;
 }
 
+int icz_gemm_resident_pair(const float* Xa, const float* Wa, float* Ca, const float* Xb, const float* Wb, float* Cb, int32_t M, int32_t N,
+                           int32_t K, int32_t stages, int32_t tiles, float* workspace, size_t workspace_floats, void* stream) {
+    ICZ_REQUIRE(Xa && Wa && Ca && Xb && Wb && Cb && M > 0 && N > 0 && K > 0, "icz_gemm_resident_pair: bad arguments");
+    GemmArgs a = {}, b = {};
+    a.nseg = b.nseg = 1;
+    a.seg[0] = {Xa, Wa, K, K, K, nullptr};
+    b.seg[0] = {Xb, Wb, K, K, K, nullptr};
+    a.M = b.M = M; a.N = b.N = N; a.ldo = b.ldo = N;
+    ICZ_REQUIRE(gemm_resident_x3_pair_fits(a, b, stages, tiles), "icz_gemm_resident_pair: shape not taken (M %d N %d K %d, %d stages x %d tiles)", M, N, K, stages, tiles);
+    const int ns = K / 64 / stages;
+    const size_t MN = (size_t)M * N;
+    ICZ_REQUIRE(workspace && 2 * (size_t)ns * MN <= workspace_floats, "icz_gemm_resident_pair: workspace of %zu floats too small for 2 x %d slabs of %d x %d", workspace_floats, ns, M, N);
+    a.out = workspace; b.out = workspace + (size_t)ns * MN;
+    hipStream_t st = (hipStream_t)stream;
+    ICZ_TRY(gemm_resident_x3_pair(a, b, stages, tiles, st));
+    hipLaunchKernelGGL(slab_reduce_kernel, dim3(cdiv((int)(MN / 4), 256)), dim3(256), 0, st, (const float*)a.out, ns, MN, N, (const float*)nullptr, Ca);
+    hipLaunchKernelGGL(slab_reduce_kernel, dim3(cdiv((int)(MN / 4), 256)), dim3(256), 0, st, (const float*)b.out, ns, MN, N, (const float*)nullptr, Cb);
+    ICZ_CHECK_HIP(hipGetLastError());
+    return ICZ_OK;
+}
+
 int icz_gemm_tn_grouped(const float* dY, int32_t ldy, int32_t M, int32_t K, int32_t ngroups, const float* const* X, const int32_t* ldx,
                         const int32_t* cols, float* const* out, const int32_t* ldo, const int32_t* rows_live, void* stream) {
     ICZ_REQUIRE(ngroups >= 1 && ngroups <= GEMM_MAX_COLGROUPS && X && ldx && cols && out && ldo, "icz_gemm_tn_grouped: bad arguments");
diff --git a/simpleimagecaptionzoo_amd/csrc/gemm_resident_x3.hip b/simpleimagecaptionzoo_amd/csrc/gemm_resident_x3.hip
--- a/simpleimagecaptionzoo_amd/csrc/gemm_resident_x3.hip
+++ b/simpleimagecaptionzoo_amd/csrc/gemm_resident_x3.hip
@@ -604,16 +604,25 @@
     return a.M > 64 ? rs_launch_m128<false>(a, stream) : (nsr == 8 ? rs_launch_k512<false>(a, stream) : rs_launch<4, false>(a, stream));
 }
 
-bool gemm_resident_x3_pair_fits(const GemmArgs& a, const GemmArgs& b) {
-    return a.M <= 64 && b.M <= 64 && rs_shape_ok(a) && rs_shape_ok(b) && gemm_resident_x3_stages(a) == gemm_resident_x3_stages(b) && a.N >= 512 && b.N >= 512;
-}
-int gemm_resident_x3_pair(const GemmArgs& a_in, const GemmArgs& b_in, hipStream_t stream) {
-    ICZ_REQUIRE(gemm_resident_x3_pair_fits(a_in, b_in), "gemm_resident_x3_pair: shapes outside the kernel's decomposition");
+static bool rs_pair_form_ok(int nsr, int tpw) {
+    return (nsr == 8 && tpw == 1 && gemm_switches().resident_k512) || (nsr == 4 && (tpw == 1 || tpw == 2));
+}
+bool gemm_resident_x3_pair_fits(const GemmArgs& a, const GemmArgs& b, int nsr, int tpw) {
+    if (!rs_pair_form_ok(nsr, tpw)) return false;
+    for (const GemmArgs* p : {&a, &b}) {
+        if (p->M > 64 || !rs_shape_ok(*p) || p->N < 512) return false;
+        const int tot = rs_total_stages(*p);
+        if (tot % nsr || tot / nsr < 2) return false;
+    }
+    return true;
+}
+int gemm_resident_x3_pair(const GemmArgs& a_in, const GemmArgs& b_in, int nsr, int tpw, hipStream_t stream) {
+    ICZ_REQUIRE(gemm_resident_x3_pair_fits(a_in, b_in, nsr, tpw), "gemm_resident_x3_pair: shapes outside the decomposition (%d stages, %d tiles)", nsr, tpw);
     GemmPair g;
     g.a = a_in; g.b = b_in;
-    const int nsr = gemm_resident_x3_stages(g.a), tilew = nsr == 8 ? 128 : 256;
+    const int tilew = 128 * tpw;
     for (GemmArgs* p : {&g.a, &g.b}) {
-        p->nsplit = gemm_resident_x3_nsplit(*p);
+        p->nsplit = rs_total_stages(*p) / nsr;
         p->chunks_per_split = nsr;
         p->bias = nullptr;
         ICZ_REQUIRE(p->out && p->nsplit > 1, "gemm_resident_x3_pair: slab output expected");
@@ -623,11 +632,13 @@
     static bool attr = false;
     if (!attr) {
         ICZ_CHECK_HIP(hipFuncSetAttribute(reinterpret_cast<const void*>(gemm_resident_x3_pair_kernel<4, 4, 2, 3>), hipFuncAttributeMaxDynamicSharedMemorySize, (int)lds));
+        ICZ_CHECK_HIP(hipFuncSetAttribute(reinterpret_cast<const void*>(gemm_resident_x3_pair_kernel<4, 4, 1, 3>), hipFuncAttributeMaxDynamicSharedMemorySize, (int)lds));
         ICZ_CHECK_HIP(hipFuncSetAttribute(reinterpret_cast<const void*>(gemm_resident_x3_pair_kernel<4, 8, 1, RS_K512_D, 4>), hipFuncAttributeMaxDynamicSharedMemorySize, (int)lds));
         attr = true;
     }
     const dim3 grid(g.first + cdiv(g.b.N, tilew) * g.b.nsplit);
     if (nsr == 8) hipLaunchKernelGGL((gemm_resident_x3_pair_kernel<4, 8, 1, RS_K512_D, 4>), grid, dim3(256), lds, stream, g);
+    else if (tpw == 1) hipLaunchKernelGGL((gemm_resident_x3_pair_kernel<4, 4, 1, 3>), grid, dim3(256), lds, stream, g);
     else hipLaunchKernelGGL((gemm_resident_x3_pair_kernel<4, 4, 2, 3>), grid, dim3(256), lds, stream, g);
     ICZ_CHECK_HIP(hipGetLastError());
     return ICZ_OK;
```

Result: no change. 12030, median of 5 (+0.7%).
